# Thiagodcv/gaussian-process-mpc

Hardware: AMD Instinct MI355X
Metric: GP-MPC rollouts/sec (N train pts x H horizon x d dims) (higher is better)
Workload: dtype f64; 1 GPU; C3: N=2048, d(state_dim)=4, action_dim=1, H=20, B=256 trajectories per GPU, gamma=-1.0, objective+gradient; N=2048, state_dim=4, action_dim=1, H=20, batch_per_gpu=256, parallelism=single GPU

## Files before the change

gaussian_process_mpc_amd/_lib.py:

```python
import ctypes
import os

import torch

_HERE = os.path.dirname(os.path.abspath(__file__))
LIB_PATH = os.environ.get("GPMPC_LIB_PATH") or os.path.join(_HERE, "csrc", "libgpmpc_hip.so")

MAX_D = 8
MAX_DS = 8
MAX_CONS = 16
MPPI_MAX_SAMPLES = 4096
LBFGS_MAX_STARTS = 256
LBFGS_MAX_HISTORY = 16
WANT_GRAD = 1
COV_BUG_COMPAT = 2
USE_GRAPH = 4
FP32_ACCUM = 8
FP32_ALL = 16

_ERR = {-1: "bad argument", -2: "device allocation failed", -3: "HIP call / kernel launch failed",
        -4: "workspace too small", -5: "pack not built",
        -6: "current HIP device differs from the device the pack was created on"}


class LibraryMissing(RuntimeError):
    pass


class GpmpcError(RuntimeError):
    pass


class CostParamsC(ctypes.Structure):
    _fields_ = [("gamma", ctypes.c_double),
                ("Q", ctypes.c_double * (MAX_DS * MAX_DS)),
                ("R", ctypes.c_double * (MAX_D * MAX_D)),
                ("R_delta", ctypes.c_double * (MAX_D * MAX_D)),
                ("x_ref", ctypes.c_double * MAX_DS),
                ("u_ref", ctypes.c_double * MAX_D),
                ("last_u", ctypes.c_double * MAX_D),
                ("has_R_delta", ctypes.c_int),
                ("schedule_id", ctypes.c_int)]


class StateConstraintsC(ctypes.Structure):
    _fields_ = [("n_rows", ctypes.c_int),
                ("reserved", ctypes.c_int),
                ("A", ctypes.c_double * (MAX_CONS * MAX_DS)),
                ("b", ctypes.c_double * MAX_CONS),
                ("kappa", ctypes.c_double * MAX_CONS)]


class MppiParamsC(ctypes.Structure):
    _fields_ = [("n_samples", ctypes.c_int),
                ("iterations", ctypes.c_int),
                ("sigma", ctypes.c_double * MAX_D),
                ("sigma_decay", ctypes.c_double),
                ("beta", ctypes.c_double),
                ("seed", ctypes.c_ulonglong),
                ("call_index", ctypes.c_uint),
                ("reserved", ctypes.c_uint),
                ("lb", ctypes.c_double * MAX_D),
                ("ub", ctypes.c_double * MAX_D)]


class LbfgsParamsC(ctypes.Structure):
    _fields_ = [("n_starts", ctypes.c_int),
                ("history", ctypes.c_int),
                ("gtol", ctypes.c_double),
                ("ftol", ctypes.c_double),
                ("c1", ctypes.c_double),
                ("min_step", ctypes.c_double),
                ("lb", ctypes.c_double * MAX_D),
                ("ub", ctypes.c_double * MAX_D)]


class AuglagParamsC(ctypes.Structure):
    _fields_ = [("inner", LbfgsParamsC),
                ("rho0", ctypes.c_double),
                ("growth", ctypes.c_double),
                ("shrink", ctypes.c_double),
                ("rho_max", ctypes.c_double),
                ("lam_max", ctypes.c_double),
                ("feas_tol", ctypes.c_double),
                ("inner_ticks", ctypes.c_int),
                ("reserved", ctypes.c_int)]


_vp, _i, _d, _sz, _u = ctypes.c_void_p, ctypes.c_int, ctypes.c_double, ctypes.c_size_t, ctypes.c_uint
_dp = ctypes.POINTER(ctypes.c_double)

SIGNATURES = {
    "gpmpc_device_count": (_i, []),
    "gpmpc_version": (ctypes.c_char_p, []),
    "gpmpc_last_error": (ctypes.c_char_p, []),
    "gpmpc_pack_create": (_i, [ctypes.POINTER(_vp), _i, _i, _i]),
    "gpmpc_pack_destroy": (_i, [_vp]),
    "gpmpc_pack_resize": (_i, [_vp, _i]),
    "gpmpc_pack_reload_tuning": (_i, [_vp]),
    "gpmpc_pack_graph_captures": (ctypes.c_longlong, [_vp]),
    "gpmpc_pack_callback_captures": (ctypes.c_longlong, [_vp]),
    "gpmpc_store_host": (_i, [_vp, _vp, _sz, _vp]),
    "gpmpc_build_ky": (_i, [_i, _i, _vp, _dp, _d, _d, _vp, _vp, _vp]),
    "gpmpc_pack_build": (_i, [_vp, _vp, _vp, _vp, _dp, _dp, _vp]),
    "gpmpc_pack_build_strided": (_i, [_vp, _vp, _vp, _vp, _sz, _sz, _dp, _dp, _vp]),
    "gpmpc_pack_build_beta": (_i, [_vp, _vp, _vp, _vp, _dp, _dp, _vp]),
    "gpmpc_pack_set_nominal": (_i, [_vp, _dp, _dp, _vp]),
    "gpmpc_pack_get_nominal": (_i, [_vp, _dp, _dp]),
    "gpmpc_pack_set_noise": (_i, [_vp, _dp, _dp, _dp, _vp]),
    "gpmpc_pack_get_noise": (_i, [_vp, _dp, _dp, _dp]),
    "gpmpc_pack_enable_fullcov": (_i, [_vp, _vp]),
    "gpmpc_pack_dims": (_i, [_vp] + [ctypes.POINTER(_i)] * 4),
    "gpmpc_pack_shared_lambda": (_i, [_vp]),
    "gpmpc_pack_export": (_i, [_vp, _vp, _vp, _vp]),
    "gpmpc_moment_match_workspace_bytes": (_sz, [_vp, _i]),
    "gpmpc_moment_match": (_i, [_vp, _i, _vp, _vp, _u] + [_vp] * 10 + [_vp, _sz, _vp]),
    "gpmpc_cost": (_i, [_i, _i, _i, _i, ctypes.POINTER(CostParamsC), _vp, _vp, _vp, _vp, _vp]),
    "gpmpc_cost_grad": (_i, [_i, _i, _i, _i, ctypes.POINTER(CostParamsC)] + [_vp] * 8),
    "gpmpc_cost_schedule_create": (_i, [_i, _i, _i, ctypes.POINTER(_i)]),
    "gpmpc_cost_schedule_destroy": (_i, [_i]),
    "gpmpc_cost_schedule_set": (_i, [_i, _i, _dp, _dp, _dp, _vp]),
    "gpmpc_cost_schedule_set_dev": (_i, [_i, _i, _vp, _vp, _vp, _vp]),
    "gpmpc_cost_schedule_get": (_i, [_i] + [ctypes.POINTER(_i)] * 5 + [ctypes.POINTER(_vp)]),
    "gpmpc_rollout_jac_workspace_bytes": (_sz, [_vp, _i, _i]),
    "gpmpc_rollout_jac": (_i, [_vp, _i, _i, _vp, _vp, _vp, _vp, _vp, _vp, _sz, _vp]),
    "gpmpc_rollout_vjp": (_i, [_i, _i, _i, _i, _vp, _vp, _vp, _vp, _vp, _vp]),
    "gpmpc_rollout_constraints": (_i, [_i, _i, _i, _i, ctypes.POINTER(StateConstraintsC), _vp, _vp, _vp, _vp, _vp, _vp]),
    "gpmpc_rollout_constrained_workspace_bytes": (_sz, [_vp, _i, _i, _u]),
    "gpmpc_rollout_constrained": (_i, [_vp, _i, _i, _vp, _vp, ctypes.POINTER(CostParamsC), ctypes.POINTER(StateConstraintsC), _u,
                                       _vp, _vp, _vp, _vp, _vp, _vp, _vp, _sz, _vp]),
    "gpmpc_mppi_sample": (_i, [_i, _i, _i, ctypes.POINTER(MppiParamsC), _i, _vp, _vp, _vp, _vp, _vp]),
    "gpmpc_mppi_update": (_i, [_i, _i, _i, _i, _d, _vp, _vp, _vp, _vp, _vp, _vp, _vp, _vp]),
    "gpmpc_mppi_solve_workspace_bytes": (_sz, [_vp, _i, ctypes.POINTER(MppiParamsC), ctypes.POINTER(StateConstraintsC)]),
    "gpmpc_mppi_solve": (_i, [_vp, _i, _vp, _vp, ctypes.POINTER(CostParamsC), ctypes.POINTER(StateConstraintsC),
                              ctypes.POINTER(MppiParamsC), _vp, _vp, _vp, _vp, _sz, _vp]),
    "gpmpc_lbfgs_state_bytes": (_sz, [_i, _i, _i, _i]),
    "gpmpc_lbfgs_start": (_i, [_i, _i, _i, ctypes.POINTER(LbfgsParamsC), _vp, _vp, _vp, _vp, _vp, _vp, _sz, _vp]),
    "gpmpc_lbfgs_tick": (_i, [_i, _i, ctypes.POINTER(LbfgsParamsC), _vp, _vp, _vp, _sz, _vp]),
    "gpmpc_lbfgs_solve_workspace_bytes": (_sz, [_vp, _i, ctypes.POINTER(LbfgsParamsC)]),
    "gpmpc_lbfgs_solve": (_i, [_vp, _i, _vp, _vp, ctypes.POINTER(CostParamsC), ctypes.POINTER(LbfgsParamsC), _i, _i, _vp, _sz, _vp]),
    "gpmpc_auglag_state_bytes": (_sz, [_i, _i, _i, _i]),
    "gpmpc_auglag_merit": (_i, [_i, _i, _i, _i] + [_vp] * 9),
    "gpmpc_auglag_outer": (_i, [_i, _i, _i, ctypes.POINTER(AuglagParamsC), _i, _vp, _vp, _vp, _vp, _vp, _vp, _sz, _vp]),
    "gpmpc_auglag_solve_workspace_bytes": (_sz, [_vp, _i, ctypes.POINTER(StateConstraintsC), ctypes.POINTER(AuglagParamsC)]),
    "gpmpc_auglag_solve": (_i, [_vp, _i, _vp, _vp, ctypes.POINTER(CostParamsC), ctypes.POINTER(StateConstraintsC),
                                ctypes.POINTER(AuglagParamsC), _i, _i, _vp, _sz, _vp]),
    "gpmpc_rollout_workspace_bytes": (_sz, [_vp, _i, _i, _u]),
    "gpmpc_plan_describe": (_i, [_vp, _i, _i, _u, ctypes.c_char_p, _sz]),
    "gpmpc_pack_autotune": (_i, [_vp, _i, _i, _u, ctypes.c_char_p, _sz]),
    "gpmpc_pack_autotune_clear": (_i, [_vp]),
    "gpmpc_rollout": (_i, [_vp, _i, _i, _vp, _vp, ctypes.POINTER(CostParamsC), _u, _vp, _vp, _vp, _vp, _vp, _sz, _vp]),
    "gpmpc_objective_gradient": (_i, [_vp, _i, _dp, _dp, ctypes.POINTER(CostParamsC), _u, _dp, _vp]),
    "gpmpc_rollout_fullcov_workspace_bytes": (_sz, [_vp, _i, _i, _u]),
    "gpmpc_rollout_fullcov_describe": (_i, [_vp, _i, _i, _u, ctypes.c_char_p, _sz]),
    "gpmpc_rollout_fullcov": (_i, [_vp, _i, _i, _vp, _vp, ctypes.POINTER(CostParamsC), _u, _vp, _vp, _vp, _vp, _vp, _sz, _vp]),
    "gpmpc_timing_enable": (_i, [_i]),
    "gpmpc_debug_run_list": (_i, [_i, _i, _i, ctypes.POINTER(_i), _i, ctypes.POINTER(_i)]),
    "gpmpc_debug_xcd_order": (_i, [_i, _i, _i, _i, ctypes.POINTER(_i), ctypes.POINTER(_i)]),
    "gpmpc_pair_kernel_time": (_i, [_dp, ctypes.POINTER(ctypes.c_longlong), _i]),
    "gpmpc_pair_kernel_time_class": (_i, [_i, _dp, ctypes.POINTER(ctypes.c_longlong)]),
    "gpmpc_matvec": (_i, [_i, _i, _vp, _vp, _vp, _vp]),
    "gpmpc_kinv_append_workspace_bytes": (_sz, [_i]),
    "gpmpc_kinv_append": (_i, [_i, _vp, _vp, _d, _vp, _vp, _sz, _vp]),
    "gpmpc_gp_append_workspace_bytes": (_sz, [_i, _i]),
    "gpmpc_gp_append": (_i, [_i, _i, _vp, _vp, _dp, _d, _d, _vp, _vp, _sz, _vp, _sz, _vp, _vp, _vp, _sz, _vp, _sz, _vp]),
    "gpmpc_kinv_remove": (_i, [_i, _vp, _sz, _i, _vp, _sz, _vp]),
    "gpmpc_gp_replace_workspace_bytes": (_sz, [_i, _i]),
    "gpmpc_gp_replace": (_i, [_i, _i, _i, _vp, _vp, _dp, _d, _d, _vp, _vp, _sz, _vp, _sz, _vp, _vp, _vp, _sz, _vp, _sz, _vp]),
    "gpmpc_predict_workspace_bytes": (_sz, [_i, _i, _i]),
    "gpmpc_predict": (_i, [_i, _i, _vp, _dp, _d, _vp, _vp, _d, _i, _vp, _vp, _vp, _vp, _vp, _sz, _vp]),
    "gpmpc_ml_grad_workspace_bytes": (_sz, [_i, _i]),
    "gpmpc_ml_grad": (_i, [_i, _i, _vp, _vp, _vp, _vp, _dp, _d, _d, _vp, _vp, _sz, _vp]),
}

_lib = None


def lib():
    global _lib
    if _lib is None:
        if not os.path.exists(LIB_PATH):
            raise LibraryMissing(
                f"{LIB_PATH} not found: build it with `python -c 'import __graft_entry__ as g; g.build()'` "
                "or `make -C gaussian_process_mpc_amd/csrc`. There is no CPU fallback.")
        h = ctypes.CDLL(LIB_PATH)
        tolerant = bool(os.environ.get("GPMPC_LIB_PATH")) and os.environ.get("GPMPC_LIB_ALLOW_MISSING") == "1"
        for name, (res, args) in SIGNATURES.items():
            try:
                fn = getattr(h, name)
            except AttributeError:
                if tolerant:
                    continue
                raise
            fn.restype, fn.argtypes = res, args
        _lib = h
    return _lib


def check(rc, what):
    if rc != 0:
        detail = lib().gpmpc_last_error().decode() if rc == -3 else ""
        if rc == -1 and ("mppi" in what or "lbfgs" in what or "auglag" in what):
            detail = lib().gpmpc_last_error().decode()
        if rc == -1 and not detail:
            why = lib().gpmpc_last_error().decode()
            detail = why if "cost schedule" in why else ""
        if rc == -5:
            why = lib().gpmpc_last_error().decode()
            detail = why if "nominal model" in why else ""
        raise GpmpcError(f"{what} failed: {_ERR.get(rc, rc)} {detail}".strip())


def require_gpu():
    lib()
    if not torch.cuda.is_available():
        raise GpmpcError("no HIP device visible: the GP-MPC rollout runs on the MI355X only (no CPU fallback)")
    return torch.device("cuda", torch.cuda.current_device())


def stream_ptr(device=None):
    idx = device.index if isinstance(device, torch.device) and device.index is not None else torch.cuda.current_device()
    return ctypes.c_void_p(torch.cuda.current_stream(idx).cuda_stream)


def ptr(t):
    if t is None:
        return ctypes.c_void_p(0)
    assert t.is_cuda and t.dtype == torch.float64 and t.is_contiguous(), (t.device, t.dtype, t.is_contiguous())
    return ctypes.c_void_p(t.data_ptr())


def host_doubles(a):
    import numpy as np
    a = np.ascontiguousarray(np.asarray(a, dtype=np.float64))
    return a, a.ctypes.data_as(_dp)
```

gaussian_process_mpc_amd/csrc/api.hip:

```cpp
#include "gpmpc_internal.h"

int gpmpc_launch_pair(int D, bool diag, bool grad, int tb, int waves, const PairArgs& a, hipStream_t s) {
    if (waves < 1 || waves > 4) return GPMPC_E_ARG;
    switch (D) {
        case 1: return gpmpc_launch_pair_D<1>(diag, grad, tb, waves, a, s);
        case 2: return gpmpc_launch_pair_D<2>(diag, grad, tb, waves, a, s);
        case 3: return gpmpc_launch_pair_D<3>(diag, grad, tb, waves, a, s);
        case 4: return gpmpc_launch_pair_D<4>(diag, grad, tb, waves, a, s);
        case 5: return gpmpc_launch_pair_D<5>(diag, grad, tb, waves, a, s);
        case 6: return gpmpc_launch_pair_D<6>(diag, grad, tb, waves, a, s);
        case 7: return gpmpc_launch_pair_D<7>(diag, grad, tb, waves, a, s);
        case 8: return gpmpc_launch_pair_D<8>(diag, grad, tb, waves, a, s);
    }
    return GPMPC_E_ARG;
}

int gpmpc_launch_pair_sb(int D, bool grad, int tb, int ns2, int waves, const PairSbArgs& a, hipStream_t s) {
    if (waves < 1 || waves > 4) return GPMPC_E_ARG;
    switch (D) {
        case 1: return gpmpc_launch_pair_sb_D<1>(grad, tb, ns2, waves, a, s);
        case 2: return gpmpc_launch_pair_sb_D<2>(grad, tb, ns2, waves, a, s);
        case 3: return gpmpc_launch_pair_sb_D<3>(grad, tb, ns2, waves, a, s);
        case 4: return gpmpc_launch_pair_sb_D<4>(grad, tb, ns2, waves, a, s);
        case 5: return gpmpc_launch_pair_sb_D<5>(grad, tb, ns2, waves, a, s);
        case 6: return gpmpc_launch_pair_sb_D<6>(grad, tb, ns2, waves, a, s);
        case 7: return gpmpc_launch_pair_sb_D<7>(grad, tb, ns2, waves, a, s);
        case 8: return gpmpc_launch_pair_sb_D<8>(grad, tb, ns2, waves, a, s);
    }
    return GPMPC_E_ARG;
}

int gpmpc_launch_pair_sbs(int D, bool grad, int ng, int ns2, const PairSbsArgs& a, hipStream_t s) {
    switch (D) {
        case 2: return gpmpc_launch_pair_sbs_D<2>(grad, ng, ns2, a, s);
        case 3: return gpmpc_launch_pair_sbs_D<3>(grad, ng, ns2, a, s);
        case 4: return gpmpc_launch_pair_sbs_D<4>(grad, ng, ns2, a, s);
        case 5: return gpmpc_launch_pair_sbs_D<5>(grad, ng, ns2, a, s);
        case 6: return gpmpc_launch_pair_sbs_D<6>(grad, ng, ns2, a, s);
        case 7: return gpmpc_launch_pair_sbs_D<7>(grad, ng, ns2, a, s);
        case 8: return gpmpc_launch_pair_sbs_D<8>(grad, ng, ns2, a, s);
    }
    return GPMPC_E_ARG;
}

int gpmpc_launch_pair_sbf(int D, bool grad, int ns2, int waves, const PairSbfArgs& a, hipStream_t s) {
    if (waves < 1 || waves > 4) return GPMPC_E_ARG;
    switch (D) {
        case 1: return gpmpc_launch_pair_sbf_D<1>(grad, ns2, waves, a, s);
        case 2: return gpmpc_launch_pair_sbf_D<2>(grad, ns2, waves, a, s);
        case 3: return gpmpc_launch_pair_sbf_D<3>(grad, ns2, waves, a, s);
        case 4: return gpmpc_launch_pair_sbf_D<4>(grad, ns2, waves, a, s);
        case 5: return gpmpc_launch_pair_sbf_D<5>(grad, ns2, waves, a, s);
        case 6: return gpmpc_launch_pair_sbf_D<6>(grad, ns2, waves, a, s);
        case 7: return gpmpc_launch_pair_sbf_D<7>(grad, ns2, waves, a, s);
        case 8: return gpmpc_launch_pair_sbf_D<8>(grad, ns2, waves, a, s);
    }
    return GPMPC_E_ARG;
}

int gpmpc_launch_pair_sbfx(int D, bool grad, int ns2, const PairSbfxArgs& a, hipStream_t s) {
    switch (D) {
        case 3: return gpmpc_launch_pair_sbfx_D<3>(grad, ns2, a, s);
        case 4: return gpmpc_launch_pair_sbfx_D<4>(grad, ns2, a, s);
        case 5: return gpmpc_launch_pair_sbfx_D<5>(grad, ns2, a, s);
        case 6: return gpmpc_launch_pair_sbfx_D<6>(grad, ns2, a, s);
    }
    return GPMPC_E_ARG;
}

__global__ void k_cross_kernel(const double* __restrict__ Xp, int p, const double* __restrict__ X, int N, int D,
                               const double* __restrict__ lam, double sf2, double* __restrict__ K) {
    const int i = blockIdx.x * blockDim.x + threadIdx.x, r = blockIdx.y;
    if (i >= N) return;
    double d2 = 0.0;
    for (int k = 0; k < D; ++k) {
        const double d = Xp[(size_t)r * D + k] - X[(size_t)i * D + k];
        d2 = fma(d * d, 1.0 / lam[k], d2);
    }
    K[(size_t)r * N + i] = sf2 * exp(-0.5 * d2);
}

__global__ __launch_bounds__(256) void k_rows_dot(const double* __restrict__ A, const double* __restrict__ v, int N,
                                                   double* __restrict__ out) {
    __shared__ double s_scr[16], s_out[1];
    const int r = blockIdx.x;
    double acc[1] = {0.0};
    for (int i = threadIdx.x; i < N; i += blockDim.x) acc[0] = fma(A[(size_t)r * N + i], v[i], acc[0]);
    block_sum<1>(acc, s_scr, s_out);
    if (threadIdx.x == 0) out[r] = s_out[0];
}

#define GPMPC_PRED_RT 8
__global__ __launch_bounds__(1024) void k_pred_w(const double* __restrict__ K, const double* __restrict__ Kinv, int N, int p,
                                                 double* __restrict__ W) {
    __shared__ double s_part[16][GPMPC_PRED_RT][64];
    const int lane = threadIdx.x & 63, w = __builtin_amdgcn_readfirstlane(threadIdx.x >> 6), r0 = blockIdx.y * GPMPC_PRED_RT;
    const int c = blockIdx.x * 64 + lane;
    const int per = (N + 15) / 16, k0 = w * per, k1 = (k0 + per < N) ? k0 + per : N;
    double s[GPMPC_PRED_RT];
#pragma unroll
    for (int q = 0; q < GPMPC_PRED_RT; ++q) s[q] = 0.0;
    if (c < N)
        for (int k = k0; k < k1; ++k) {
            const double a = Kinv[(size_t)k * N + c];
#pragma unroll
            for (int q = 0; q < GPMPC_PRED_RT; ++q) {
                const int r = r0 + q < p ? r0 + q : p - 1;
                s[q] = fma(K[(size_t)r * N + k], a, s[q]);
            }
        }
#pragma unroll
    for (int q = 0; q < GPMPC_PRED_RT; ++q) s_part[w][q][lane] = s[q];
    __syncthreads();
    for (int q = w; q < GPMPC_PRED_RT; q += 16) {
        if (r0 + q < p && c < N) {
            double t = 0.0;
#pragma unroll
            for (int ww = 0; ww < 16; ++ww) t += s_part[ww][q][lane];
            W[(size_t)(r0 + q) * N + c] = t;
        }
    }
}

__global__ __launch_bounds__(256) void k_pred_cov(const double* __restrict__ Xp, int p, int D, const double* __restrict__ lam,
                                                   double sf2, const double* __restrict__ W, const double* __restrict__ K,
                                                   int N, double noise_var, double* __restrict__ cov) {
    __shared__ double s_scr[16], s_out[1];
    const int r = blockIdx.x, s = blockIdx.y;
    double v[1] = {0.0};
    for (int i = threadIdx.x; i < N; i += blockDim.x) v[0] = fma(W[(size_t)r * N + i], K[(size_t)s * N + i], v[0]);
    block_sum<1>(v, s_scr, s_out);
    if (threadIdx.x == 0) {
        double d2 = 0.0;
        for (int k = 0; k < D; ++k) {
            const double d = Xp[(size_t)r * D + k] - Xp[(size_t)s * D + k];
            d2 = fma(d * d, 1.0 / lam[k], d2);
        }
        cov[(size_t)r * p + s] = sf2 * exp(-0.5 * d2) - s_out[0] + (r == s ? noise_var : 0.0);
    }
}

extern "C" int gpmpc_matvec(int rows, int cols, const double* A_dev, const double* v_dev, double* out_dev, void* stream) {
    if (rows < 1 || cols < 1 || !A_dev || !v_dev || !out_dev) return GPMPC_E_ARG;
    hipLaunchKernelGGL(k_rows_dot, dim3(rows), dim3(256), 0, (hipStream_t)stream, A_dev, v_dev, cols, out_dev);
    GPMPC_HIP(hipGetLastError());
    return GPMPC_OK;
}

extern "C" size_t gpmpc_predict_workspace_bytes(int n, int D, int np) {
    if (n < 1 || np < 1 || D < 1) return 0;
    return 2 * ((sizeof(double) * (size_t)np * n + 255) & ~(size_t)255) + 256;
}

extern "C" int gpmpc_predict(int n, int D, const double* X, const double* lambdas_host, double sigma_f,
                             const double* beta, const double* Kinv, double noise_var, int np, const double* Xp,
                             double* out_K, double* out_mean, double* out_cov, void* workspace, size_t workspace_bytes,
                             void* stream) {
    if (n < 1 || D < 1 || D > GPMPC_MAX_D || np < 1 || !X || !lambdas_host || !Xp || !workspace) return GPMPC_E_ARG;
    if ((out_mean && !beta) || (out_cov && !Kinv)) return GPMPC_E_ARG;
    if (workspace_bytes < gpmpc_predict_workspace_bytes(n, D, np)) return GPMPC_E_WORKSPACE;
    hipStream_t s = (hipStream_t)stream;
    const size_t slab = (sizeof(double) * (size_t)np * n + 255) & ~(size_t)255;
    double* K = out_K ? out_K : (double*)workspace;
    double* W = (double*)((char*)workspace + slab);
    double* lam = (double*)((char*)workspace + 2 * slab);
    if (int rcu = gpmpc_upload_small(lam, lambdas_host, sizeof(double) * D, s)) return rcu;
    const double sf2 = sigma_f * sigma_f;
    hipLaunchKernelGGL(k_cross_kernel, dim3((n + 255) / 256, np), dim3(256), 0, s, Xp, np, X, n, D, lam, sf2, K);
    if (out_mean) hipLaunchKernelGGL(k_rows_dot, dim3(np), dim3(256), 0, s, K, beta, n, out_mean);
    if (out_cov) {
        hipLaunchKernelGGL(k_pred_w, dim3((n + 63) / 64, (np + GPMPC_PRED_RT - 1) / GPMPC_PRED_RT), dim3(1024), 0, s, K, Kinv, n, np, W);
        hipLaunchKernelGGL(k_pred_cov, dim3(np, np), dim3(256), 0, s, Xp, np, D, lam, sf2, W, K, n, noise_var, out_cov);
    }
    GPMPC_HIP(hipGetLastError());
    return GPMPC_OK;
}

__global__ __launch_bounds__(256) void k_append_vw(const double* __restrict__ Kinv, size_t ld, const double* __restrict__ k, int n,
                                                    double* __restrict__ v, double* __restrict__ wv) {
    __shared__ double s_scr[32], s_out[2];
    const int r = blockIdx.x;
    double acc[2] = {0.0, 0.0};
    for (int i = threadIdx.x; i < n; i += blockDim.x) {
        acc[0] = fma(Kinv[(size_t)r * ld + i], k[i], acc[0]);
        acc[1] = fma(Kinv[(size_t)i * ld + r], k[i], acc[1]);
    }
    block_sum<2>(acc, s_scr, s_out);
    if (threadIdx.x == 0) { v[r] = s_out[0]; wv[r] = s_out[1]; }
}

__global__ __launch_bounds__(256) void k_append_q(const double* __restrict__ k, const double* __restrict__ v, int n, double kappa,
                                                   double* __restrict__ q) {
    __shared__ double s_scr[16], s_out[1];
    double acc[1] = {0.0};
    for (int i = threadIdx.x; i < n; i += blockDim.x) acc[0] = fma(k[i], v[i], acc[0]);
    block_sum<1>(acc, s_scr, s_out);
    if (threadIdx.x == 0) q[0] = 1.0 / (kappa - s_out[0]);
}

__global__ void k_append_fill(const double* __restrict__ Kinv, size_t ld_in, const double* __restrict__ v, const double* __restrict__ wv,
                              const double* __restrict__ q, int n, double* __restrict__ out, size_t ld_out,
                              const double* __restrict__ k, const double* __restrict__ Kf_in, const double* __restrict__ Ky_in, size_t ld_k,
                              double* __restrict__ Kf_out, double* __restrict__ Ky_out, double kff, double noise_var) {
    const int j = blockIdx.x * blockDim.x + threadIdx.x, i = blockIdx.y, m = n + 1;
    if (j >= m) return;
    const double qq = q[0];
    double val;
    if (i < n && j < n) val = fma(qq * v[i], wv[j], Kinv[(size_t)i * ld_in + j]);
    else if (i < n) val = -qq * v[i];
    else if (j < n) val = -qq * wv[j];
    else val = qq;
    out[(size_t)i * ld_out + j] = val;
    if (Kf_out) {
        double kf, ky;
        if (i < n && j < n) { kf = Kf_in[(size_t)i * ld_k + j]; ky = Ky_in[(size_t)i * ld_k + j]; }
        else if (i < n) { kf = k[i]; ky = kf; }
        else if (j < n) { kf = k[j]; ky = kf; }
        else { kf = kff; ky = kff + noise_var; }
        Kf_out[(size_t)i * ld_out + j] = kf;
        Ky_out[(size_t)i * ld_out + j] = ky;
    }
}

__global__ void k_append_kvec(const double* __restrict__ X, int n, int D, const double* __restrict__ xnew, const double* __restrict__ lam,
                              double sf2, double* __restrict__ k) {
    const int i = blockIdx.x * blockDim.x + threadIdx.x;
    if (i >= n) return;
    double d2 = 0.0;
    for (int d = 0; d < D; ++d) { const double t = X[(size_t)i * D + d] - xnew[d]; d2 = fma(t * t, 1.0 / lam[d], d2); }
    k[i] = sf2 * exp(-0.5 * d2);
}

extern "C" size_t gpmpc_kinv_append_workspace_bytes(int n) { return n < 1 ? 0 : sizeof(double) * (2 * (size_t)n + 8); }

extern "C" int gpmpc_kinv_append(int n, const double* Kinv_dev, const double* k_dev, double kappa, double* out_dev,
                                 void* workspace, size_t workspace_bytes, void* stream) {
    if (n < 1 || !Kinv_dev || !k_dev || !out_dev || !workspace) return GPMPC_E_ARG;
    if (workspace_bytes < gpmpc_kinv_append_workspace_bytes(n)) return GPMPC_E_WORKSPACE;
    hipStream_t s = (hipStream_t)stream;
    double* v = (double*)workspace; double* wv = v + n; double* q = wv + n;
    hipLaunchKernelGGL(k_append_vw, dim3(n), dim3(256), 0, s, Kinv_dev, (size_t)n, k_dev, n, v, wv);
    hipLaunchKernelGGL(k_append_q, dim3(1), dim3(256), 0, s, k_dev, v, n, kappa, q);
    hipLaunchKernelGGL(k_append_fill, dim3((n + 1 + 255) / 256, n + 1), dim3(256), 0, s, Kinv_dev, (size_t)n, v, wv, q, n, out_dev,
                       (size_t)(n + 1), (const double*)nullptr, (const double*)nullptr, (const double*)nullptr, (size_t)0, (double*)nullptr,
                       (double*)nullptr, 0.0, 0.0);
    GPMPC_HIP(hipGetLastError());
    return GPMPC_OK;
}

struct AppendHyp { double lam[GPMPC_MAX_D]; double sf2; };

__global__ __launch_bounds__(256) void k_append_vw2(const double* __restrict__ X, int n, int D, const double* __restrict__ xnew, AppendHyp H,
                                                     const double* __restrict__ Kinv, size_t ld, double* __restrict__ kout,
                                                     double* __restrict__ v, double* __restrict__ wv) {
    __shared__ double s_scr[32], s_out[2];
    const int r = blockIdx.x;
    double acc[2] = {0.0, 0.0};
    for (int i = threadIdx.x; i < n; i += blockDim.x) {
        double d2 = 0.0;
        for (int d = 0; d < D; ++d) { const double t = X[(size_t)i * D + d] - xnew[d]; d2 = fma(t * t, 1.0 / H.lam[d], d2); }
        const double ki = H.sf2 * exp(-0.5 * d2);
        if (r == 0) kout[i] = ki;
        acc[0] = fma(Kinv[(size_t)r * ld + i], ki, acc[0]);
        acc[1] = fma(Kinv[(size_t)i * ld + r], ki, acc[1]);
    }
    block_sum<2>(acc, s_scr, s_out);
    if (threadIdx.x == 0) { v[r] = s_out[0]; wv[r] = s_out[1]; }
}

__global__ __launch_bounds__(256) void k_append_fill2(const double* __restrict__ Kinv, size_t ld_in, const double* __restrict__ v,
                                                       const double* __restrict__ wv, double kappa, int n, double* __restrict__ out, size_t ld_out,
                                                       const double* __restrict__ k, const double* __restrict__ Kf_in, const double* __restrict__ Ky_in,
                                                       size_t ld_k, double* __restrict__ Kf_out, double* __restrict__ Ky_out, double kff, double noise_var) {
    __shared__ double s_scr[16], s_out[1];
    double acc[1] = {0.0};
    for (int i = threadIdx.x; i < n; i += blockDim.x) acc[0] = fma(k[i], v[i], acc[0]);
    block_sum<1>(acc, s_scr, s_out);
    const double qq = 1.0 / (kappa - s_out[0]);
    const int j = blockIdx.x * blockDim.x + threadIdx.x, i = blockIdx.y, m = n + 1;
    if (j >= m) return;
    double val;
    if (i < n && j < n) val = fma(qq * v[i], wv[j], Kinv[(size_t)i * ld_in + j]);
    else if (i < n) val = -qq * v[i];
    else if (j < n) val = -qq * wv[j];
    else val = qq;
    out[(size_t)i * ld_out + j] = val;
    if (Kf_out) {
        double kf, ky;
        if (i < n && j < n) { kf = Kf_in[(size_t)i * ld_k + j]; ky = Ky_in[(size_t)i * ld_k + j]; }
        else if (i < n) { kf = k[i]; ky = kf; }
        else if (j < n) { kf = k[j]; ky = kf; }
        else { kf = kff; ky = kff + noise_var; }
        Kf_out[(size_t)i * ld_out + j] = kf;
        Ky_out[(size_t)i * ld_out + j] = ky;
    }
}

extern "C" size_t gpmpc_gp_append_workspace_bytes(int n, int D) { (void)D; return n < 1 ? 0 : sizeof(double) * (3 * (size_t)n + 8); }

extern "C" int gpmpc_gp_append(int n, int D, const double* X_dev, const double* xnew_dev, const double* lambdas_host, double sigma_f,
                               double noise_var, const double* Kf_in, const double* Ky_in, size_t ld_k_in, const double* Kinv_in, size_t ld_in,
                               double* Kf_out, double* Ky_out, double* Kinv_out, size_t ld_out, void* workspace, size_t workspace_bytes,
                               void* stream) {
    if (n < 1 || D < 1 || D > GPMPC_MAX_D || !X_dev || !xnew_dev || !lambdas_host || !Kf_in || !Ky_in || !Kinv_in || !Kf_out || !Ky_out ||
        !Kinv_out || !workspace || ld_in < (size_t)n || ld_k_in < (size_t)n || ld_out < (size_t)n + 1)
        return GPMPC_E_ARG;
    if (Kf_in == Kf_out || Ky_in == Ky_out || Kinv_in == Kinv_out) return GPMPC_E_ARG;
    if (workspace_bytes < gpmpc_gp_append_workspace_bytes(n, D)) return GPMPC_E_WORKSPACE;
    hipStream_t s = (hipStream_t)stream;
    double* v = (double*)workspace; double* wv = v + n; double* k = wv + n;
    AppendHyp hyp;
    memset(&hyp, 0, sizeof(hyp));
    for (int d = 0; d < D; ++d) hyp.lam[d] = lambdas_host[d];
    hyp.sf2 = sigma_f * sigma_f;
    hipLaunchKernelGGL(k_append_vw2, dim3(n), dim3(256), 0, s, X_dev, n, D, xnew_dev, hyp, Kinv_in, ld_in, k, v, wv);
    hipLaunchKernelGGL(k_append_fill2, dim3((n + 1 + 255) / 256, n + 1), dim3(256), 0, s, Kinv_in, ld_in, (const double*)v, (const double*)wv,
                       hyp.sf2 + noise_var, n, Kinv_out, ld_out, (const double*)k, Kf_in, Ky_in, ld_k_in, Kf_out, Ky_out, hyp.sf2, noise_var);
    GPMPC_HIP(hipGetLastError());
    return GPMPC_OK;
}

__global__ __launch_bounds__(256) void k_kinv_remove(const double* __restrict__ Kinv, size_t ld_in, int n, int p, double* __restrict__ out,
                                                      size_t ld_out) {
    const int jo = blockIdx.x * blockDim.x + threadIdx.x, io = blockIdx.y;
    if (jo >= n - 1) return;
    const int i = io + (io >= p), j = jo + (jo >= p);
    const double bd = Kinv[(size_t)i * ld_in + p] / Kinv[(size_t)p * ld_in + p];
    out[(size_t)io * ld_out + jo] = fma(-bd, Kinv[(size_t)p * ld_in + j], Kinv[(size_t)i * ld_in + j]);
}

extern "C" int gpmpc_kinv_remove(int n, const double* Kinv_dev, size_t ld_in, int index, double* out_dev, size_t ld_out, void* stream) {
    if (n < 2 || !Kinv_dev || !out_dev || index < 0 || index >= n || ld_in < (size_t)n || ld_out < (size_t)n - 1 || Kinv_dev == out_dev)
        return GPMPC_E_ARG;
    hipLaunchKernelGGL(k_kinv_remove, dim3((n - 1 + 255) / 256, n - 1), dim3(256), 0, (hipStream_t)stream, Kinv_dev, ld_in, n, index, out_dev,
                       ld_out);
    GPMPC_HIP(hipGetLastError());
    return GPMPC_OK;
}

__global__ __launch_bounds__(256) void k_replace_vw(const double* __restrict__ X, int n, int D, int p, const double* __restrict__ xnew, AppendHyp H,
                                                     const double* __restrict__ Kinv, size_t ld, double* __restrict__ kout,
                                                     double* __restrict__ v, double* __restrict__ wv) {
    __shared__ double s_scr[64], s_out[4];
    const int r = blockIdx.x;
    double acc[4] = {0.0, 0.0, 0.0, 0.0};
    for (int i = threadIdx.x; i < n; i += blockDim.x) {
        double ki = 0.0;
        if (i != p) {
            double d2 = 0.0;
            for (int d = 0; d < D; ++d) { const double t = X[(size_t)i * D + d] - xnew[d]; d2 = fma(t * t, 1.0 / H.lam[d], d2); }
            ki = H.sf2 * exp(-0.5 * d2);
        }
        if (r == 0) kout[i] = ki;
        acc[0] = fma(Kinv[(size_t)r * ld + i], ki, acc[0]);
        acc[1] = fma(Kinv[(size_t)i * ld + r], ki, acc[1]);
        acc[2] = fma(Kinv[(size_t)p * ld + i], ki, acc[2]);
        acc[3] = fma(Kinv[(size_t)i * ld + p], ki, acc[3]);
    }
    block_sum<4>(acc, s_scr, s_out);
    if (threadIdx.x == 0) {
        const double d = Kinv[(size_t)p * ld + p];
        v[r] = r == p ? 0.0 : fma(-Kinv[(size_t)r * ld + p], s_out[2] / d, s_out[0]);
        wv[r] = r == p ? 0.0 : fma(-Kinv[(size_t)p * ld + r], s_out[3] / d, s_out[1]);
    }
}

__global__ __launch_bounds__(256) void k_replace_fill(const double* __restrict__ Kinv, size_t ld_in, const double* __restrict__ v,
                                                       const double* __restrict__ wv, double kappa, int n, int p, double* __restrict__ out,
                                                       size_t ld_out, const double* __restrict__ k, const double* __restrict__ Kf_in,
                                                       const double* __restrict__ Ky_in, size_t ld_k, double* __restrict__ Kf_out,
                                                       double* __restrict__ Ky_out, double kff, double noise_var) {
    __shared__ double s_scr[16], s_out[1];
    double acc[1] = {0.0};
    for (int i = threadIdx.x; i < n; i += blockDim.x) acc[0] = fma(k[i], v[i], acc[0]);
    block_sum<1>(acc, s_scr, s_out);
    const double qq = 1.0 / (kappa - s_out[0]);
    const int j = blockIdx.x * blockDim.x + threadIdx.x, i = blockIdx.y;
    if (j >= n) return;
    double val, kf, ky;
    if (i != p && j != p) {
        const double bd = Kinv[(size_t)i * ld_in + p] / Kinv[(size_t)p * ld_in + p];
        val = fma(qq * v[i], wv[j], fma(-bd, Kinv[(size_t)p * ld_in + j], Kinv[(size_t)i * ld_in + j]));
        kf = Kf_in[(size_t)i * ld_k + j]; ky = Ky_in[(size_t)i * ld_k + j];
    } else if (i != p) { val = -qq * v[i]; kf = k[i]; ky = kf; }
    else if (j != p) { val = -qq * wv[j]; kf = k[j]; ky = kf; }
    else { val = qq; kf = kff; ky = kff + noise_var; }
    out[(size_t)i * ld_out + j] = val;
    Kf_out[(size_t)i * ld_out + j] = kf;
    Ky_out[(size_t)i * ld_out + j] = ky;
}

extern "C" size_t gpmpc_gp_replace_workspace_bytes(int n, int D) { (void)D; return n < 1 ? 0 : sizeof(double) * (3 * (size_t)n + 8); }

extern "C" int gpmpc_gp_replace(int n, int D, int slot, const double* X_dev, const double* xnew_dev, const double* lambdas_host, double sigma_f,
                                double noise_var, const double* Kf_in, const double* Ky_in, size_t ld_k_in, const double* Kinv_in, size_t ld_in,
                                double* Kf_out, double* Ky_out, double* Kinv_out, size_t ld_out, void* workspace, size_t workspace_bytes,
                                void* stream) {
    if (n < 1 || D < 1 || D > GPMPC_MAX_D || slot < 0 || slot >= n || !X_dev || !xnew_dev || !lambdas_host || !Kf_in || !Ky_in || !Kinv_in ||
        !Kf_out || !Ky_out || !Kinv_out || !workspace || ld_in < (size_t)n || ld_k_in < (size_t)n || ld_out < (size_t)n)
        return GPMPC_E_ARG;
    if (Kf_in == Kf_out || Ky_in == Ky_out || Kinv_in == Kinv_out) return GPMPC_E_ARG;
    if (workspace_bytes < gpmpc_gp_replace_workspace_bytes(n, D)) return GPMPC_E_WORKSPACE;
    hipStream_t s = (hipStream_t)stream;
    double* v = (double*)workspace; double* wv = v + n; double* k = wv + n;
    AppendHyp hyp;
    memset(&hyp, 0, sizeof(hyp));
    for (int d = 0; d < D; ++d) hyp.lam[d] = lambdas_host[d];
    hyp.sf2 = sigma_f * sigma_f;
    hipLaunchKernelGGL(k_replace_vw, dim3(n), dim3(256), 0, s, X_dev, n, D, slot, xnew_dev, hyp, Kinv_in, ld_in, k, v, wv);
    hipLaunchKernelGGL(k_replace_fill, dim3((n + 255) / 256, n), dim3(256), 0, s, Kinv_in, ld_in, (const double*)v, (const double*)wv,
                       hyp.sf2 + noise_var, n, slot, Kinv_out, ld_out, (const double*)k, Kf_in, Ky_in, ld_k_in, Kf_out, Ky_out, hyp.sf2, noise_var);
    GPMPC_HIP(hipGetLastError());
    return GPMPC_OK;
}
```

gaussian_process_mpc_amd/csrc/gpmpc_internal.h:

```cpp
#pragma once
#include <hip/hip_runtime.h>
#include <cstdio>
#include <cstring>
#include "../../include/gpmpc.h"

#define GPMPC_WAVE 64

#define GPMPC_INIT_VAR   1e-3
#define GPMPC_ACTION_VAR ((double)1e-3f)
#define GPMPC_NOISE_MAX (GPMPC_MAX_DS * GPMPC_MAX_DS + GPMPC_MAX_D + GPMPC_MAX_DS)
__host__ __device__ inline int gpmpc_noise_off_action(int ds) { return ds * ds; }
__host__ __device__ inline int gpmpc_noise_off_process(int ds, int da) { return ds * ds + da; }

#define GPMPC_MAX_PAIRS (GPMPC_MAX_DS * (GPMPC_MAX_DS - 1) / 2)

struct gpmpc_worklist {
    int it;
    int waves;
    int jt;
    int nunits, nwork;
    int contiguous;
    int* work_dev;
    int* perm_dev;
    int* ustart_dev;
    int ustart_host[GPMPC_MAX_DS + GPMPC_MAX_PAIRS + 1];
};

struct gpmpc_tuning {
    int pair_sb;
    int tiling;
    int tb;
    int rgroup;
    int no_first;
    int fused;
    int no_xcd_sort;
    int hchunks;
    int sbf_min;
    int colunroll;
    int fused_sb;
    int split;
    int shared;
    int fc_form;
    int fc_rsplit;
    int fc_cu;
    int fc_tiling;
    int fc_shared;
    int xcdmap;
    int persist;
};
void gpmpc_read_tuning(gpmpc_tuning* t);

struct gpmpc_pack {
    int N, Np, ds, da, D;
    int device;
    int num_cu;
    gpmpc_tuning tune;
    int built;
    int npairs;
    int fullcov;
    int pair_a[GPMPC_MAX_PAIRS > 0 ? GPMPC_MAX_PAIRS : 1], pair_b[GPMPC_MAX_PAIRS > 0 ? GPMPC_MAX_PAIRS : 1];
    int* pair_ab_dev;
    double* fcs_rows; int fcs_rw, fcs_tj;
    int fcs_ntile[3];
    int* fcs_ustart_dev[8][3]; int fcs_base[8], fcs_total[8][3];
    int* fcs_tiles256_dev;
    int ncol_host;
    int* ncol_dev;
    double* X;
    double* XT;
    double* beta;
    double* M;
    double* lam;
    double* sf;
    double lam_host[GPMPC_MAX_DS][GPMPC_MAX_D];
    double sf_host[GPMPC_MAX_DS];
    void* graph_cache;
    void* cb_cache;
    void* tuned;
    void* lock;
    gpmpc_worklist wl[2][8];
    int shared_lambda;
    int sh_ng;
    gpmpc_worklist wl_sh[4];
    int sh_tiles[3];
    int nominal;
    double* nom_dev;
    double* resid_dev;
    double nom_host[GPMPC_MAX_DS * (GPMPC_MAX_D + 1)];
    double* noise_dev;
    double noise_host[GPMPC_NOISE_MAX];
};

static inline int gpmpc_num_moments(int D, bool diag, bool grad) {
    if (!grad) return 1;
    return diag ? 1 + 2 * D : 1 + D + D * (D + 1) / 2;
}

struct PairArgs {
    const double* M;
    const double* XT;
    const double* pp;
    double* part;
    const int* work;
    int Np, B, nunits, nwork, pps, nm;
    int jside_off;
    int ntri;
    int ns2;
    int colsplit;
};

struct PairSbArgs {
    const double* M;
    const double* XT;
    const double* pp;
    const double* G;
    double* part;
    const int* work;
    int Np, B, ds, nwork, pps, nm;
    int rgroup;
    int first_step;
    int colunroll;
    const int* ncol;
};
static inline int gpmpc_sb_gw(int D, int ns2) { return (D + 1 + ns2 + 1) & ~1; }
int gpmpc_launch_pair_sb(int D, bool grad, int tb, int ns2, int waves, const PairSbArgs& a, hipStream_t s);
template <int D> int gpmpc_launch_pair_sb_D(bool grad, int tb, int ns2, int waves, const PairSbArgs& a, hipStream_t s);

struct PairSbfArgs {
    const double* M;
    const double* XT;
    const double* pp;
    const double* G;
    double* part;
    const int* work;
    int Np, B, nunits, nwork, pps, nm, ntri;
    int cu;
    double* part0;
    int pstride;
};
struct PairSbfxArgs {
    const double* XT; const double* lam; const double* beta; const double* sf;
    const double* pp; const double* G;
    const double* rows;
    double* part; double* part0;
    const int* pair_ab;
    int Np, N, B, nunits, unit0, pps, nm;
    int tj, ntile, jt;
    const int* tiles;
    int base, pstride;
};
template <int D> int gpmpc_launch_pair_sbfx_D(bool grad, int ns2, const PairSbfxArgs& a, hipStream_t s);
int gpmpc_launch_pair_sbfx(int D, bool grad, int ns2, const PairSbfxArgs& a, hipStream_t s);
static inline int gpmpc_sbf_gw(int D, int ns2) { return (D + 1 + ns2 * (ns2 + 1) / 2 + 1) & ~1; }
int gpmpc_launch_pair_sbf(int D, bool grad, int ns2, int waves, const PairSbfArgs& a, hipStream_t s);
template <int D> int gpmpc_launch_pair_sbf_D(bool grad, int ns2, int waves, const PairSbfArgs& a, hipStream_t s);

struct PairSbsArgs {
    const double* M;
    const double* XT;
    const double* pp;
    const double* G;
    double* part;
    const int* work;
    int Np, B, ds, nwork, tiles, jt, pps, nm;
    int rgroup, first_step;
    const int* ncol;
};
static inline int gpmpc_sbs_group(int ds, int D) {
    int cap = 48 / (1 + D + ds);
    if (cap > 4) cap = 4;
    if (cap < 2) cap = 2;
    const int groups = (ds + cap - 1) / cap;
    return (ds + groups - 1) / groups;
}
int gpmpc_launch_pair_sbs(int D, bool grad, int ng, int ns2, const PairSbsArgs& a, hipStream_t s);
template <int D> int gpmpc_launch_pair_sbs_D(bool grad, int ng, int ns2, const PairSbsArgs& a, hipStream_t s);

int gpmpc_launch_pair_lowprec(int D, int mode, const PairArgs& a, hipStream_t s);

struct FusedArgs {
    const double* XT; const double* beta; const double* lam; const double* sf; const double* M; const int* work;
    int Np, nwork;
    int tri64;
    int ustart[GPMPC_MAX_DS + 1];
    const double* x0; const double* U; int B, H;
    double* means; double* vars; double* jac;
    double* sp; double* part; double* partz;
    int sps, nm;
    double* gscr;
    int ntile;
    int tiles;
    const int* ncol;
    int xcdmap;
    const double* noise;
};
template <int D> int gpmpc_launch_step_fused_D(bool grad, int ns2, int q, int ng, const FusedArgs& a, int t, hipStream_t s);
__host__ __device__ inline void gpmpc_xcd_remap(int L, int gx, int nt, int nB, int* b, unsigned* bx) {
    const int nt8 = nt & ~7, full = nt8 * nB, allt = nt * nB;
    if (L < full) { const int grp = L / (8 * nB), r = L - grp * 8 * nB; *b = r >> 3; *bx = (unsigned)(grp * 8 + (r & 7)); }
    else if (L < allt) { const int rem = nt - nt8, L2 = L - full; *b = L2 / rem; *bx = (unsigned)(nt8 + L2 - *b * rem); }
    else { const int nr = gx - nt, L3 = L - allt; *b = L3 / nr; *bx = (unsigned)(nt + L3 - *b * nr); }
}

struct PersistArgs {
    const double* XT; const double* beta; const double* lam; const double* sf; const double* M;
    int Np;
    const double* x0; const double* U; int B, H;
    double* means; double* vars; double* jac;
    double* gscr;
    const int* ncol;
    int total;
    const double* noise;
};
template <int D> int gpmpc_launch_persist_D(bool grad, int ns2, int waves, int ng, const PersistArgs& a, hipStream_t s);


int gpmpc_launch_pair(int D, bool diag, bool grad, int tb, int waves, const PairArgs& a, hipStream_t s);
template <int D> int gpmpc_launch_pair_D(bool diag, bool grad, int tb, int waves, const PairArgs& a, hipStream_t s);

void gpmpc_set_error(const char* what, hipError_t e);
void gpmpc_set_error_text(const char* text);
int gpmpc_check_constraints(const gpmpc_state_constraints* cons, const char* who);
__host__ __device__ inline size_t gpmpc_sched_off_u(int H_max, int ds) { return (size_t)(H_max + 1) * ds; }
__host__ __device__ inline size_t gpmpc_sched_off_q(int H_max, int ds, int da) { return gpmpc_sched_off_u(H_max, ds) + (size_t)H_max * da; }
__host__ __device__ inline size_t gpmpc_sched_off_flags(int H_max, int ds, int da) { return gpmpc_sched_off_q(H_max, ds, da) + (size_t)ds * ds; }
struct gpmpc_sched_ref { const double* dev; int H_max; };
int gpmpc_schedule_resolve(const gpmpc_cost_params* cost, int ds, int da, int H, const char* who, gpmpc_sched_ref* out);
int gpmpc_upload_small(void* dst_dev, const void* src_host, size_t bytes, hipStream_t s);
static inline int gpmpc_check_device(const gpmpc_pack* p) {
    int dev = -1;
    if (hipGetDevice(&dev) != hipSuccess) return GPMPC_E_LAUNCH;
    return dev == p->device ? GPMPC_OK : GPMPC_E_DEVICE;
}
enum { GPMPC_TIME_FULL = 0, GPMPC_TIME_FIRST = 1, GPMPC_TIME_FUSED = 2, GPMPC_TIME_CLASSES = 3 };
void gpmpc_tuned_free(void* table);
void gpmpc_tuned_clear(void* table);
void* gpmpc_lock_create();
void gpmpc_lock_destroy(void* lock);
void gpmpc_graph_cache_free(void* cache);
void gpmpc_cb_cache_free(void* cache);
void gpmpc_graph_cache_invalidate(void* cache);
void gpmpc_cb_cache_invalidate(void* cache);
#define GPMPC_HIP(call)                                              \
    do {                                                             \
        hipError_t e_ = (call);                                      \
        if (e_ != hipSuccess) { gpmpc_set_error(#call, e_); return GPMPC_E_LAUNCH; } \
    } while (0)

template <int CTRL>
__device__ __forceinline__ double gpmpc_dpp_f64(double v) {
    const int lo = __builtin_amdgcn_update_dpp(0, __double2loint(v), CTRL, 0xf, 0xf, false);
    const int hi = __builtin_amdgcn_update_dpp(0, __double2hiint(v), CTRL, 0xf, 0xf, false);
    return __hiloint2double(hi, lo);
}
__device__ __forceinline__ double gpmpc_readlane_f64(double v, int lane) {
    return __hiloint2double(__builtin_amdgcn_readlane(__double2hiint(v), lane), __builtin_amdgcn_readlane(__double2loint(v), lane));
}
__device__ __forceinline__ double wave_sum(double v) {
    v += gpmpc_dpp_f64<0xB1>(v);
    v += gpmpc_dpp_f64<0x4E>(v);
    v += gpmpc_dpp_f64<0x141>(v);
    v += gpmpc_dpp_f64<0x140>(v);
    return (gpmpc_readlane_f64(v, 0) + gpmpc_readlane_f64(v, 16)) + (gpmpc_readlane_f64(v, 32) + gpmpc_readlane_f64(v, 48));
}

__device__ __forceinline__ double wave_row_sum(double v) {
    v += gpmpc_dpp_f64<0xB1>(v);
    v += gpmpc_dpp_f64<0x4E>(v);
    v += gpmpc_dpp_f64<0x141>(v);
    v += gpmpc_dpp_f64<0x140>(v);
    return v;
}

template <int NV>
__device__ __forceinline__ void block_sum4_rows(const double (&v)[NV], double* scratch, double* out) {
    const int lane = threadIdx.x & 63, w = threadIdx.x >> 6;
#pragma unroll
    for (int k = 0; k < NV; ++k) {
        const double s = wave_row_sum(v[k]);
        if ((lane & 15) == 0) scratch[(w * 4 + (lane >> 4)) * NV + k] = s;
    }
    __syncthreads();
    if (threadIdx.x < NV) {
        double s = 0;
        for (int ww = 0; ww < 4; ++ww) {
            const double* r4 = &scratch[ww * 4 * NV + threadIdx.x];
            s += (r4[0] + r4[NV]) + (r4[2 * NV] + r4[3 * NV]);
        }
        out[threadIdx.x] = s;
    }
    __syncthreads();
}

template <int NV>
__device__ __forceinline__ void block_sum(const double (&v)[NV], double* scratch, double* out) {
    const int lane = threadIdx.x & 63, w = threadIdx.x >> 6, nw = (blockDim.x + 63) >> 6;
#pragma unroll
    for (int k = 0; k < NV; ++k) {
        double s = wave_sum(v[k]);
        if (lane == 0) scratch[w * NV + k] = s;
    }
    __syncthreads();
    if (threadIdx.x < NV) {
        double s = 0;
        for (int ww = 0; ww < nw; ++ww) s += scratch[ww * NV + threadIdx.x];
        out[threadIdx.x] = s;
    }
    __syncthreads();
}
```

gaussian_process_mpc_amd/csrc/pack.hip:

```cpp
#include "gpmpc_internal.h"
#include <cstdlib>

__global__ void k_pack_points(const double* __restrict__ X, int N, int Np, int D,
                              double* __restrict__ Xp, double* __restrict__ XT) {
    const int i = blockIdx.x * blockDim.x + threadIdx.x;
    if (i >= Np) return;
    for (int k = 0; k < D; ++k) {
        const double v = i < N ? X[(size_t)i * D + k] : 0.0;
        Xp[(size_t)i * D + k] = v;
        XT[(size_t)k * Np + i] = v;
    }
}

__global__ __launch_bounds__(256) void k_pack_beta(const double* __restrict__ Kinv, size_t ld, size_t gstride, const double* __restrict__ Y,
                                                    int N, int Np, int ds, double* __restrict__ beta) {
    const int a = blockIdx.y;
    const int row = blockIdx.x * (blockDim.x >> 6) + (threadIdx.x >> 6);
    const int lane = threadIdx.x & 63;
    if (row >= Np) return;
    double s = 0.0;
    if (row < N) {
        const double* __restrict__ r = Kinv + (size_t)a * gstride + (size_t)row * ld;
        for (int j = lane; j < N; j += 64) s = fma(r[j], Y[(size_t)j * ds + a], s);
        s = wave_sum(s);
    }
    if (lane == 0) beta[(size_t)a * Np + row] = s;
}

__global__ __launch_bounds__(256) void k_pack_weights(const double* __restrict__ Kinv, size_t ld, size_t gstride, const double* __restrict__ beta,
                                                       const double* __restrict__ XT, const double* __restrict__ lam,
                                                       const double* __restrict__ sf, int N, int Np, int D,
                                                       double* __restrict__ M) {
    __shared__ double s_t[32][33];
    const int a = blockIdx.z;
    const int ti = blockIdx.x * 32, tj = blockIdx.y * 32;
    const int tx = threadIdx.x & 31, ty = threadIdx.x >> 5;
    const double* __restrict__ Ka = Kinv + (size_t)a * gstride;
    double* __restrict__ Ma = M + (size_t)a * Np * Np;
    if (tj + 31 < ti) {
        for (int r = ty; r < 32; r += 8) {
            const int j = tj + r, i = ti + tx;
            if (j < Np && i < Np) Ma[(size_t)j * Np + i] = 0.0;
        }
        return;
    }
    for (int r = ty; r < 32; r += 8) {
        const int i = ti + r, j = tj + tx;
        s_t[r][tx] = (i < N && j < N) ? Ka[(size_t)i * ld + j] : 0.0;
    }
    __syncthreads();
    const double sf2 = sf[a] * sf[a], sf4 = sf2 * sf2;
    for (int r = ty; r < 32; r += 8) {
        const int j = tj + r, i = ti + tx;
        if (j >= Np || i >= Np) continue;
        double out = 0.0;
        if (i <= j && j < N) {
            const double kji = Ka[(size_t)j * ld + i];
            const double kij = s_t[tx][r];
            double d2 = 0.0;
            for (int k = 0; k < D; ++k) {
                const double d = XT[(size_t)k * Np + i] - XT[(size_t)k * Np + j];
                d2 = fma(d * d, 1.0 / lam[a * D + k], d2);
            }
            const double wsym = 0.5 * (kij + kji) - beta[(size_t)a * Np + i] * beta[(size_t)a * Np + j];
            out = (i == j ? 1.0 : 2.0) * wsym * sf4 * exp(-0.25 * d2);
        }
        Ma[(size_t)j * Np + i] = out;
    }
}

__global__ void k_pack_residual(const double* __restrict__ X, const double* __restrict__ Y, const double* __restrict__ nom,
                                int N, int D, int ds, double* __restrict__ R) {
    const int i = blockIdx.x * blockDim.x + threadIdx.x, a = blockIdx.y;
    if (i >= N) return;
    double m = nom[ds * D + a];
    for (int k = 0; k < D; ++k) m = fma(X[(size_t)i * D + k], nom[a * D + k], m);
    R[(size_t)i * ds + a] = Y[(size_t)i * ds + a] - m;
}

struct gpmpc_small_payload { unsigned w[128]; };
__global__ void k_upload_small(gpmpc_small_payload p, unsigned* __restrict__ dst, int nwords) {
    const int i = threadIdx.x;
    if (i < nwords) dst[i] = p.w[i];
}
int gpmpc_upload_small(void* dst_dev, const void* src_host, size_t bytes, hipStream_t s) {
    if (!dst_dev || !src_host || bytes == 0 || bytes > sizeof(gpmpc_small_payload) || (bytes & 3)) return GPMPC_E_ARG;
    gpmpc_small_payload p;
    memset(&p, 0, sizeof(p));
    memcpy(&p, src_host, bytes);
    hipLaunchKernelGGL(k_upload_small, dim3(1), dim3(128), 0, s, p, (unsigned*)dst_dev, (int)(bytes / 4));
    GPMPC_HIP(hipGetLastError());
    return GPMPC_OK;
}

extern "C" int gpmpc_store_host(void* dst_dev, const void* src_host, size_t bytes, void* stream) {
    return gpmpc_upload_small(dst_dev, src_host, bytes, (hipStream_t)stream);
}

__global__ void k_build_ky(const double* __restrict__ X, int n, int D, const double* __restrict__ lam,
                           double sf2, double noise_var, double* __restrict__ Kf, double* __restrict__ Ky) {
    const int j = blockIdx.x * blockDim.x + threadIdx.x, i = blockIdx.y;
    if (j >= n) return;
    double d2 = 0.0;
    for (int k = 0; k < D; ++k) {
        const double d = X[(size_t)i * D + k] - X[(size_t)j * D + k];
        d2 = fma(d * d, 1.0 / lam[k], d2);
    }
    const double kf = sf2 * exp(-0.5 * d2);
    if (Kf) Kf[(size_t)i * n + j] = kf;
    Ky[(size_t)i * n + j] = kf + (i == j ? noise_var : 0.0);
}

__global__ void k_pack_fcs_rows(const double* __restrict__ beta, const double* __restrict__ XT, const double* __restrict__ lam,
                                int N, int Np, int D, int ds, int rw, double* __restrict__ rows) {
    const int j = blockIdx.x * blockDim.x + threadIdx.x;
    if (j >= Np) return;
    double* r = rows + (size_t)j * rw;
    double e = 0.0;
    for (int k = 0; k < D; ++k) { const double x = XT[(size_t)k * Np + j]; r[k] = x; e = fma(x * x, 1.0 / lam[k], e); }
    r[D] = (0.25 * 0x1.71547652b82fep+11) * e;
    for (int c = 0; c < ds; ++c) r[D + 1 + c] = j < N ? beta[(size_t)c * Np + j] : 0.0;
    for (int k = D + 1 + ds; k < rw; ++k) r[k] = 0.0;
}

static int fcs_refresh(gpmpc_pack* p, hipStream_t s) {
    if (!p->fullcov || p->npairs == 0 || !p->shared_lambda || p->ds < 2 || p->ds > 4 || p->D - p->ds < 1 || p->D - p->ds > 2) return GPMPC_OK;
    if (!p->fcs_rows) {
        p->fcs_rw = (p->D + 1 + p->ds + 1) & ~1;
        p->fcs_tj = p->Np / 64;
        p->fcs_ntile[0] = p->fcs_tj * (p->fcs_tj + 1) / 2; p->fcs_ntile[1] = 4 * p->fcs_ntile[0];
        {
            const int T = p->fcs_tj;
            int n2 = 0;
            for (int ti = 0; ti < T; ++ti) n2 += (p->Np - 64 * ti + 255) / 256;
            int* h = (int*)malloc(sizeof(int) * 3 * (size_t)n2);
            if (!h) return GPMPC_E_ALLOC;
            int k = 0;
            for (int ti = 0; ti < T; ++ti)
                for (int j0 = 64 * ti; j0 < p->Np; j0 += 256) { h[3 * k] = ti; h[3 * k + 1] = j0; h[3 * k + 2] = p->Np - j0 < 256 ? p->Np - j0 : 256; ++k; }
            p->fcs_ntile[2] = n2;
            hipError_t e = hipMalloc(&p->fcs_tiles256_dev, sizeof(int) * 3 * (size_t)n2);
            if (e == hipSuccess) e = hipMemcpy(p->fcs_tiles256_dev, h, sizeof(int) * 3 * (size_t)n2, hipMemcpyHostToDevice);
            free(h);
            if (e != hipSuccess) return GPMPC_E_ALLOC;
        }
        if (hipMalloc(&p->fcs_rows, sizeof(double) * (size_t)p->Np * p->fcs_rw) != hipSuccess) { p->fcs_rows = nullptr; return GPMPC_E_ALLOC; }
        for (int k : {0, 2, 4}) {
            const gpmpc_worklist& w = p->wl[1][k];
            if (!w.work_dev) continue;
            int ust[GPMPC_MAX_DS + GPMPC_MAX_PAIRS + 1];
            const int ntri = w.ustart_host[p->ds];
            for (int u = 0; u <= p->ds; ++u) ust[u] = w.ustart_host[u];
            p->fcs_base[k] = ntri;
            const size_t nb = sizeof(int) * (p->ds + p->npairs + 1);
            for (int q = 0; q < 3; ++q) {
                for (int pr = 1; pr <= p->npairs; ++pr) ust[p->ds + pr] = ntri + pr * p->fcs_ntile[q];
                p->fcs_total[k][q] = ntri + p->npairs * p->fcs_ntile[q];
                if (hipMalloc(&p->fcs_ustart_dev[k][q], nb) != hipSuccess) { p->fcs_ustart_dev[k][q] = nullptr; return GPMPC_E_ALLOC; }
                GPMPC_HIP(hipMemcpy(p->fcs_ustart_dev[k][q], ust, nb, hipMemcpyHostToDevice));
            }
        }
    }
    hipLaunchKernelGGL(k_pack_fcs_rows, dim3((p->Np + 255) / 256), dim3(256), 0, s, p->beta, p->XT, p->lam, p->N, p->Np, p->D, p->ds,
                       p->fcs_rw, p->fcs_rows);
    GPMPC_HIP(hipGetLastError());
    return GPMPC_OK;
}

__global__ void k_pack_cross(const double* __restrict__ beta, const double* __restrict__ XT, const double* __restrict__ lam,
                             const double* __restrict__ sf, const int* __restrict__ pair_ab, int N, int Np, int D, int ds,
                             double* __restrict__ Mx) {
    const int i = blockIdx.x * blockDim.x + threadIdx.x, j = blockIdx.y, pr = blockIdx.z;
    if (i >= Np) return;
    const int a = pair_ab[2 * pr], b = pair_ab[2 * pr + 1];
    double out = 0.0;
    if (i < N && j < N) {
        double d2 = 0.0;
        for (int k = 0; k < D; ++k) {
            const double d = XT[(size_t)k * Np + i] - XT[(size_t)k * Np + j];
            d2 = fma(d * d, 1.0 / (lam[a * D + k] + lam[b * D + k]), d2);
        }
        const double s2 = sf[a] * sf[a] * sf[b] * sf[b];
        out = beta[(size_t)a * Np + i] * beta[(size_t)b * Np + j] * s2 * exp(-0.5 * d2);
    }
    Mx[((size_t)pr * Np + j) * Np + i] = out;
}

static int build_worklist(int Np, int it, int jt, int ds, int npairs, bool xcd_sort, gpmpc_worklist* w,
                          bool tile_slot = false, int* tiles_out = nullptr) {
    const int ti = (Np + it - 1) / it, tj = (Np + jt - 1) / jt;
    const size_t cap = (size_t)ti * tj * (ds + npairs);
    int* h = (int*)malloc(sizeof(int) * 4 * cap);
    if (!h) return -1;
    int n = 0;
    for (int u = 0; u < ds + npairs; ++u) {
        w->ustart_host[u] = n;
        for (int i0 = 0; i0 < Np; i0 += it)
            for (int j0 = 0; j0 < Np; j0 += jt) {
                const int j1 = j0 + jt < Np ? j0 + jt : Np;
                if (u < ds && j1 <= i0) continue;
                h[4 * n] = u; h[4 * n + 1] = i0; h[4 * n + 2] = j0; h[4 * n + 3] = tile_slot ? n - w->ustart_host[u] : j1; ++n;
            }
        if (tiles_out) *tiles_out = n - w->ustart_host[u];
    }
    w->ustart_host[ds + npairs] = n;
    w->contiguous = 1;
    if (xcd_sort && n >= 16) {
        int* q[8]; int cnt[8] = {0}, pos[8] = {0};
        for (int x = 0; x < 8; ++x) q[x] = (int*)malloc(sizeof(int) * 4 * (size_t)n);
        for (int k = 0; k < n; ++k) {
            const int u = h[4 * k], tjx = h[4 * k + 2] / jt;
            const int x = ((u & 1) ? (tj - 1 - tjx) : tjx) & 7;
            memcpy(q[x] + 4 * cnt[x]++, h + 4 * k, sizeof(int) * 4);
        }
        for (int x = 0; x < 8; ++x)
            qsort(q[x], cnt[x], sizeof(int) * 4, [](const void* a, const void* b) {
                const int* u = (const int*)a; const int* v = (const int*)b;
                if (u[0] != v[0]) return u[0] - v[0];
                if (u[2] != v[2]) return u[2] - v[2];
                return u[1] - v[1];
            });
        for (int p = 0; p < n; ++p) {
            int x = p & 7;
            if (pos[x] >= cnt[x]) {
                int best = 0;
                for (int y = 1; y < 8; ++y) if (cnt[y] - pos[y] > cnt[best] - pos[best]) best = y;
                x = best;
            }
            memcpy(h + 4 * p, q[x] + 4 * pos[x]++, sizeof(int) * 4);
        }
        for (int x = 0; x < 8; ++x) free(q[x]);
        w->contiguous = 0;
    }
    w->it = it; w->waves = it / 64 > 0 ? it / 64 : 1; w->jt = jt; w->nunits = ds + npairs; w->nwork = n;
    hipError_t e = hipMalloc(&w->work_dev, sizeof(int) * 4 * (size_t)n);
    if (e == hipSuccess) e = hipMemcpy(w->work_dev, h, sizeof(int) * 4 * (size_t)n, hipMemcpyHostToDevice);
    w->perm_dev = nullptr;
    if (e == hipSuccess && !w->contiguous) {
        int* perm = (int*)malloc(sizeof(int) * (size_t)n);
        int fill[GPMPC_MAX_DS + GPMPC_MAX_PAIRS + 1];
        for (int u = 0; u <= ds + npairs; ++u) fill[u] = w->ustart_host[u];
        for (int k = 0; k < n; ++k) perm[fill[h[4 * k]]++] = k;
        e = hipMalloc(&w->perm_dev, sizeof(int) * (size_t)n);
        if (e == hipSuccess) e = hipMemcpy(w->perm_dev, perm, sizeof(int) * (size_t)n, hipMemcpyHostToDevice);
        free(perm);
    }
    if (e == hipSuccess) e = hipMalloc(&w->ustart_dev, sizeof(int) * (ds + npairs + 1));
    if (e == hipSuccess) e = hipMemcpy(w->ustart_dev, w->ustart_host, sizeof(int) * (ds + npairs + 1), hipMemcpyHostToDevice);
    free(h);
    return e == hipSuccess ? 0 : -1;
}

static int runs_host(int Np, int ds, int slots, int** items_out, int* ustart) {
    const int it = 256;
    int n64 = 0;
    for (int i0 = 0; i0 < Np; i0 += it) n64 += (Np - (i0 / 64) * 64 + 63) / 64;
    n64 *= ds;
    if (slots < 64 || n64 <= slots + slots / 10) return 0;
    auto count = [&](int L) { int c = 0; for (int i0 = 0; i0 < Np; i0 += it) { const int span = Np - i0; c += (span + L - 1) / L; } return c * ds; };
    int L = 8;
    while (L < 256 && count(L) > slots) L += 8;
    if (count(L) > slots) return 0;
    const int n = count(L);
    int* h = (int*)malloc(sizeof(int) * 4 * (size_t)n);
    if (!h) return -1;
    int k = 0;
    for (int u = 0; u < ds; ++u) {
        ustart[u] = k;
        for (int i0 = 0; i0 < Np; i0 += it) {
            const int span = Np - i0, runs = (span + L - 1) / L;
            int j = i0;
            for (int q = 0; q < runs; ++q) {
                int len = ((span / runs) / 8) * 8;
                const int extra = (span - len * runs) / 8;
                if (q < extra) len += 8;
                if (q == runs - 1) len = Np - j;
                h[4 * k] = u; h[4 * k + 1] = i0; h[4 * k + 2] = j; h[4 * k + 3] = j + len; ++k;
                j += len;
            }
        }
    }
    ustart[ds] = k;
    *items_out = h;
    return k;
}

static int build_worklist_runs(int Np, int ds, int slots, gpmpc_worklist* w) {
    int* h = nullptr;
    const int k = runs_host(Np, ds, slots, &h, w->ustart_host);
    if (k == 0) return 1;
    if (k < 0) return -1;
    w->contiguous = 1;
    w->it = 256; w->waves = 4; w->jt = 256; w->nunits = ds; w->nwork = k;
    w->perm_dev = nullptr;
    hipError_t e = hipMalloc(&w->work_dev, sizeof(int) * 4 * (size_t)k);
    if (e == hipSuccess) e = hipMemcpy(w->work_dev, h, sizeof(int) * 4 * (size_t)k, hipMemcpyHostToDevice);
    if (e == hipSuccess) e = hipMalloc(&w->ustart_dev, sizeof(int) * (ds + 1));
    if (e == hipSuccess) e = hipMemcpy(w->ustart_dev, w->ustart_host, sizeof(int) * (ds + 1), hipMemcpyHostToDevice);
    free(h);
    return e == hipSuccess ? 0 : -1;
}

extern "C" int gpmpc_debug_run_list(int n_padded, int state_dim, int slots, int* items_out, int capacity, int* n_items) {
    if (n_padded < 64 || n_padded % 64 || state_dim < 1 || state_dim > GPMPC_MAX_DS || !n_items || capacity < 0 || (capacity > 0 && !items_out)) return GPMPC_E_ARG;
    int* h = nullptr; int ust[GPMPC_MAX_DS + 1];
    const int k = runs_host(n_padded, state_dim, slots, &h, ust);
    if (k < 0) return GPMPC_E_ALLOC;
    *n_items = k;
    if (k > 0) { if (k <= capacity) memcpy(items_out, h, sizeof(int) * 4 * (size_t)k); free(h); }
    return (k > capacity && capacity > 0) ? GPMPC_E_ARG : GPMPC_OK;
}
extern "C" int gpmpc_debug_xcd_order(int linear_id, int grid_x, int n_tile, int n_traj, int* traj, int* column) {
    if (!traj || !column || grid_x < 1 || n_tile < 1 || n_tile > grid_x || n_traj < 1 || linear_id < 0 || (long)linear_id >= (long)grid_x * n_traj) return GPMPC_E_ARG;
    unsigned bx = 0;
    gpmpc_xcd_remap(linear_id, grid_x, n_tile, n_traj, traj, &bx);
    *column = (int)bx;
    return GPMPC_OK;
}

void gpmpc_read_tuning(gpmpc_tuning* t) {
    auto geti = [](const char* name, int unset) { const char* ev = getenv(name); return ev ? atoi(ev) : unset; };
    t->pair_sb = geti("GPMPC_PAIR_SB", -1);
    t->tiling = geti("GPMPC_TILING", -1);
    t->tb = geti("GPMPC_PAIR_TB", 0);
    t->rgroup = geti("GPMPC_RGROUP", 0);
    t->no_first = getenv("GPMPC_NO_FIRST") ? 1 : 0;
    t->fused = geti("GPMPC_FUSED", -1);
    t->no_xcd_sort = getenv("GPMPC_NO_XCD_SORT") ? 1 : 0;
    t->hchunks = geti("GPMPC_HEAD_CHUNKS", -1);
    t->sbf_min = geti("GPMPC_SBF_MIN", 0);
    t->shared = geti("GPMPC_SHARED", -1);
    t->colunroll = geti("GPMPC_SB_UNROLL", -1);
    t->split = geti("GPMPC_SPLIT", -1);
    t->fused_sb = geti("GPMPC_FUSED_SB", -1);
    t->persist = geti("GPMPC_PERSIST", -1);
    t->xcdmap = geti("GPMPC_XCDMAP", -1);
    t->fc_shared = geti("GPMPC_FC_SHARED", -1);
    t->fc_form = geti("GPMPC_FC_FORM", -1);
    t->fc_tiling = geti("GPMPC_FC_TILING", -1);
    t->fc_rsplit = geti("GPMPC_FC_RSPLIT", 0);
    t->fc_cu = geti("GPMPC_FC_CU", 0);
}

extern "C" int gpmpc_pack_reload_tuning(gpmpc_pack* p) {
    if (!p) return GPMPC_E_ARG;
    if (int rc_dev = gpmpc_check_device(p)) return rc_dev;
    const int keep = p->tune.no_xcd_sort;
    gpmpc_read_tuning(&p->tune);
    p->tune.no_xcd_sort = keep;
    if (p->graph_cache) { gpmpc_graph_cache_free(p->graph_cache); p->graph_cache = nullptr; }
    if (p->cb_cache) { gpmpc_cb_cache_free(p->cb_cache); p->cb_cache = nullptr; }
    gpmpc_tuned_clear(p->tuned);
    return GPMPC_OK;
}

static void noise_defaults(int ds, int da, double* img, bool init, bool action, bool process) {
    if (init) for (int k = 0; k < ds; ++k) for (int l = 0; l < ds; ++l) img[k * ds + l] = k == l ? GPMPC_INIT_VAR : 0.0;
    if (action) for (int j = 0; j < da; ++j) img[gpmpc_noise_off_action(ds) + j] = GPMPC_ACTION_VAR;
    if (process) for (int a = 0; a < ds; ++a) img[gpmpc_noise_off_process(ds, da) + a] = 0.0;
}

extern "C" int gpmpc_pack_create(gpmpc_pack** out, int n_train, int state_dim, int action_dim) {
    if (!out || n_train < 1 || state_dim < 1 || action_dim < 0) return GPMPC_E_ARG;
    const int D = state_dim + action_dim;
    if (D > GPMPC_MAX_D || state_dim > GPMPC_MAX_DS || D < 1) return GPMPC_E_ARG;
    gpmpc_pack* p = (gpmpc_pack*)calloc(1, sizeof(gpmpc_pack));
    if (!p) return GPMPC_E_ALLOC;
    p->N = n_train; p->Np = ((n_train + 63) / 64) * 64; p->ds = state_dim; p->da = action_dim; p->D = D;
    gpmpc_read_tuning(&p->tune);
    p->lock = gpmpc_lock_create();
    if (!p->lock) { free(p); return GPMPC_E_ALLOC; }
    if (hipError_t ed = hipGetDevice(&p->device); ed != hipSuccess) { gpmpc_set_error("gpmpc_pack_create: hipGetDevice", ed); gpmpc_lock_destroy(p->lock); free(p); return GPMPC_E_LAUNCH; }
    if (hipDeviceGetAttribute(&p->num_cu, hipDeviceAttributeMultiprocessorCount, p->device) != hipSuccess || p->num_cu < 1) p->num_cu = 256;
    for (int a = 0; a < state_dim; ++a)
        for (int b = a + 1; b < state_dim; ++b) { p->pair_a[p->npairs] = a; p->pair_b[p->npairs] = b; ++p->npairs; }
    const size_t Np = p->Np;
    hipError_t e = hipSuccess;
    if (e == hipSuccess) e = hipMalloc(&p->X, sizeof(double) * Np * D);
    if (e == hipSuccess) e = hipMalloc(&p->XT, sizeof(double) * Np * D);
    if (e == hipSuccess) e = hipMalloc(&p->beta, sizeof(double) * Np * state_dim);
    if (e == hipSuccess) e = hipMalloc(&p->M, sizeof(double) * Np * Np * state_dim);
    if (e == hipSuccess) e = hipMalloc(&p->lam, sizeof(double) * state_dim * D);
    if (e == hipSuccess) e = hipMalloc(&p->sf, sizeof(double) * state_dim);
    if (e == hipSuccess) e = hipMalloc(&p->ncol_dev, 64);
    if (e == hipSuccess) { const int nc0 = p->Np; e = hipMemcpy(p->ncol_dev, &nc0, sizeof(int), hipMemcpyHostToDevice); p->ncol_host = nc0; }
    if (e == hipSuccess && p->npairs > 0) {
        int hab[2 * GPMPC_MAX_PAIRS];
        for (int k = 0; k < p->npairs; ++k) { hab[2 * k] = p->pair_a[k]; hab[2 * k + 1] = p->pair_b[k]; }
        e = hipMalloc(&p->pair_ab_dev, sizeof(int) * 2 * p->npairs);
        if (e == hipSuccess) e = hipMemcpy(p->pair_ab_dev, hab, sizeof(int) * 2 * p->npairs, hipMemcpyHostToDevice);
    }
    if (e == hipSuccess) e = hipMalloc(&p->noise_dev, sizeof(double) * GPMPC_NOISE_MAX);
    if (e == hipSuccess) {
        noise_defaults(p->ds, p->da, p->noise_host, true, true, true);
        e = hipMemcpy(p->noise_dev, p->noise_host, sizeof(double) * GPMPC_NOISE_MAX, hipMemcpyHostToDevice);
    }
    bool ok = e == hipSuccess;
    int cfg[7][2] = {{256, 256}, {64, 64}, {256, 64}, {64, 128}, {256, 128}, {256, 32}, {256, 16}};
    if (const char* ev = getenv("GPMPC_JT0")) { const int v = atoi(ev); if (v >= 64 && v % 64 == 0) cfg[0][1] = v; }
    for (int mode = 0; mode < 2 && ok; ++mode)
        for (int k = 0; k < 7 && ok; ++k) {
            if (mode == 1 && k >= 2 && k != 2 && k != 4) continue;
            ok = build_worklist(p->Np, cfg[k][0], cfg[k][1], state_dim, mode ? p->npairs : 0,
                                mode == 0 && (k == 0 || k == 4) && !p->tune.no_xcd_sort, &p->wl[mode][k]) == 0;
        }
    if (ok && D >= 6 && !getenv("GPMPC_NO_RUNS")) {
        const int occ = 4;
        if (build_worklist_runs(p->Np, state_dim, p->num_cu * occ - 2 * state_dim, &p->wl[0][7]) < 0) ok = false;
    }
    if (ok && state_dim >= 2 && action_dim >= 1 && action_dim <= 2) {
        p->sh_ng = gpmpc_sbs_group(state_dim, D);
        if (const char* ev = getenv("GPMPC_SHARED_NG")) { const int v = atoi(ev); if (v >= 2 && v <= 4 && v <= state_dim) p->sh_ng = v; }
        const int groups = (state_dim + p->sh_ng - 1) / p->sh_ng;
        ok = build_worklist(p->Np, 256, cfg[0][1], groups, 0, !p->tune.no_xcd_sort, &p->wl_sh[0], true, &p->sh_tiles[0]) == 0 &&
             build_worklist(p->Np, 256, 64, groups, 0, false, &p->wl_sh[1], true, &p->sh_tiles[1]) == 0 &&
             build_worklist(p->Np, 256, 128, groups, 0, !p->tune.no_xcd_sort, &p->wl_sh[2], true, &p->sh_tiles[2]) == 0;
        if (ok && p->sh_ng > 2 && state_dim % 2 == 0) {
            int tiles2 = 0;
            ok = build_worklist(p->Np, 256, 64, state_dim / 2, 0, false, &p->wl_sh[3], true, &tiles2) == 0;
        }
    }
    if (!ok) { gpmpc_set_error("gpmpc_pack_create", e); gpmpc_pack_destroy(p); return GPMPC_E_ALLOC; }
    *out = p;
    return GPMPC_OK;
}

extern "C" int gpmpc_pack_resize(gpmpc_pack* p, int n_train) {
    if (!p || n_train < 1) return GPMPC_E_ARG;
    if (int rc_dev = gpmpc_check_device(p)) return rc_dev;
    if (((n_train + 63) / 64) * 64 != p->Np) return GPMPC_E_ARG;
    p->N = n_train;
    p->built = 0;
    return GPMPC_OK;
}

extern "C" int gpmpc_pack_set_nominal(gpmpc_pack* p, const double* weights_host, const double* bias_host, void* stream) {
    if (!p || ((weights_host == nullptr) != (bias_host == nullptr))) return GPMPC_E_ARG;
    if (int rc_dev = gpmpc_check_device(p)) return rc_dev;
    const int on = weights_host ? 1 : 0, nw = p->ds * p->D;
    if (on) {
        if (!p->nom_dev && hipMalloc(&p->nom_dev, sizeof(double) * (nw + p->ds)) != hipSuccess) { p->nom_dev = nullptr; return GPMPC_E_ALLOC; }
        if (!p->resid_dev && hipMalloc(&p->resid_dev, sizeof(double) * (size_t)p->Np * p->ds) != hipSuccess) { p->resid_dev = nullptr; return GPMPC_E_ALLOC; }
        if (int rcu = gpmpc_upload_small(p->nom_dev, weights_host, sizeof(double) * nw, (hipStream_t)stream)) return rcu;
        if (int rcu = gpmpc_upload_small(p->nom_dev + nw, bias_host, sizeof(double) * p->ds, (hipStream_t)stream)) return rcu;
        memcpy(p->nom_host, weights_host, sizeof(double) * nw);
        memcpy(p->nom_host + nw, bias_host, sizeof(double) * p->ds);
    }
    if (on != p->nominal) {
        gpmpc_graph_cache_invalidate(p->graph_cache);
        gpmpc_cb_cache_invalidate(p->cb_cache);
        gpmpc_tuned_clear(p->tuned);
    }
    p->nominal = on;
    p->built = 0;
    return GPMPC_OK;
}

extern "C" int gpmpc_pack_get_nominal(const gpmpc_pack* p, double* weights_host, double* bias_host) {
    if (!p) return GPMPC_E_ARG;
    if (!p->nominal) return 0;
    const int nw = p->ds * p->D;
    if (weights_host) memcpy(weights_host, p->nom_host, sizeof(double) * nw);
    if (bias_host) memcpy(bias_host, p->nom_host + nw, sizeof(double) * p->ds);
    return 1;
}

extern "C" int gpmpc_pack_set_noise(gpmpc_pack* p, const double* init_cov_host, const double* action_var_host, const double* process_var_host,
                                    void* stream) {
    if (!p) return GPMPC_E_ARG;
    const int ds = p->ds, da = p->da, oa = gpmpc_noise_off_action(ds), ow = gpmpc_noise_off_process(ds, da), n = ow + ds;
    double img[GPMPC_NOISE_MAX];
    memset(img, 0, sizeof(img));
    noise_defaults(ds, da, img, !init_cov_host, !action_var_host, !process_var_host);
    char msg[160];
    if (init_cov_host) {
        double pmax = 0.0;
        for (int e = 0; e < ds * ds; ++e) {
            const double v = init_cov_host[e];
            if (!(v - v == 0.0)) { snprintf(msg, sizeof(msg), "gpmpc_pack_set_noise: init_cov[%d][%d] is not finite", e / ds, e % ds); gpmpc_set_error_text(msg); return GPMPC_E_ARG; }
            if (fabs(v) > pmax) pmax = fabs(v);
        }
        for (int k = 0; k < ds; ++k) {
            if (init_cov_host[k * ds + k] < 0.0) { snprintf(msg, sizeof(msg), "gpmpc_pack_set_noise: init_cov[%d][%d] is negative", k, k); gpmpc_set_error_text(msg); return GPMPC_E_ARG; }
            for (int l = 0; l < ds; ++l) {
                const double a = init_cov_host[k * ds + l], b = init_cov_host[l * ds + k];
                if (fabs(a - b) > 1e-12 * pmax) { snprintf(msg, sizeof(msg), "gpmpc_pack_set_noise: init_cov is not symmetric at [%d][%d]", k, l); gpmpc_set_error_text(msg); return GPMPC_E_ARG; }
                img[k * ds + l] = k == l ? a : 0.5 * (a + b);
            }
        }
    }
    for (int part = 0; part < 2; ++part) {
        const double* src = part ? process_var_host : action_var_host;
        const int cnt = part ? ds : da, off = part ? ow : oa;
        if (!src) continue;
        for (int j = 0; j < cnt; ++j) {
            const double v = src[j];
            if (!(v - v == 0.0) || v < 0.0) {
                snprintf(msg, sizeof(msg), "gpmpc_pack_set_noise: %s[%d] is %s", part ? "process_var" : "action_var", j, v < 0.0 ? "negative" : "not finite");
                gpmpc_set_error_text(msg);
                return GPMPC_E_ARG;
            }
            img[off + j] = v;
        }
    }
    if (int rc_dev = gpmpc_check_device(p)) return rc_dev;
    for (int o = 0; o < n; o += 64) {
        const int m = n - o < 64 ? n - o : 64;
        if (int rcu = gpmpc_upload_small(p->noise_dev + o, img + o, sizeof(double) * m, (hipStream_t)stream)) return rcu;
        memcpy(p->noise_host + o, img + o, sizeof(double) * m);
    }
    return GPMPC_OK;
}

extern "C" int gpmpc_pack_get_noise(const gpmpc_pack* p, double* init_cov_host, double* action_var_host, double* process_var_host) {
    if (!p) return GPMPC_E_ARG;
    const int ds = p->ds, da = p->da, oa = gpmpc_noise_off_action(ds), ow = gpmpc_noise_off_process(ds, da);
    if (init_cov_host) memcpy(init_cov_host, p->noise_host, sizeof(double) * ds * ds);
    if (action_var_host) memcpy(action_var_host, p->noise_host + oa, sizeof(double) * da);
    if (process_var_host) memcpy(process_var_host, p->noise_host + ow, sizeof(double) * ds);
    double def[GPMPC_NOISE_MAX];
    noise_defaults(ds, da, def, true, true, true);
    for (int e = 0; e < ow + ds; ++e) if (p->noise_host[e] != def[e]) return 1;
    return 0;
}

extern "C" int gpmpc_pack_destroy(gpmpc_pack* p) {
    if (!p) return GPMPC_OK;
    if (p->X) (void)hipFree(p->X);
    if (p->XT) (void)hipFree(p->XT);
    if (p->beta) (void)hipFree(p->beta);
    if (p->M) (void)hipFree(p->M);
    if (p->lam) (void)hipFree(p->lam);
    if (p->sf) (void)hipFree(p->sf);
    if (p->ncol_dev) (void)hipFree(p->ncol_dev);
    gpmpc_graph_cache_free(p->graph_cache);
    gpmpc_cb_cache_free(p->cb_cache);
    gpmpc_tuned_free(p->tuned);
    gpmpc_lock_destroy(p->lock);
    if (p->pair_ab_dev) (void)hipFree(p->pair_ab_dev);
    if (p->fcs_rows) (void)hipFree(p->fcs_rows);
    for (int k = 0; k < 8; ++k) for (int q = 0; q < 3; ++q) if (p->fcs_ustart_dev[k][q]) (void)hipFree(p->fcs_ustart_dev[k][q]);
    if (p->fcs_tiles256_dev) (void)hipFree(p->fcs_tiles256_dev);
    if (p->nom_dev) (void)hipFree(p->nom_dev);
    if (p->noise_dev) (void)hipFree(p->noise_dev);
    if (p->resid_dev) (void)hipFree(p->resid_dev);
    for (int mode = 0; mode < 2; ++mode)
        for (int k = 0; k < 8; ++k) {
            if (p->wl[mode][k].work_dev) (void)hipFree(p->wl[mode][k].work_dev);
            if (p->wl[mode][k].perm_dev) (void)hipFree(p->wl[mode][k].perm_dev);
            if (p->wl[mode][k].ustart_dev) (void)hipFree(p->wl[mode][k].ustart_dev);
        }
    for (int k = 0; k < 4; ++k) {
        if (p->wl_sh[k].work_dev) (void)hipFree(p->wl_sh[k].work_dev);
        if (p->wl_sh[k].perm_dev) (void)hipFree(p->wl_sh[k].perm_dev);
        if (p->wl_sh[k].ustart_dev) (void)hipFree(p->wl_sh[k].ustart_dev);
    }
    free(p);
    return GPMPC_OK;
}

__global__ void k_pack_copy_beta(const double* __restrict__ Bsrc, int N, int Np, int ds, double* __restrict__ beta) {
    const int i = blockIdx.x * blockDim.x + threadIdx.x, a = blockIdx.y;
    if (i < Np) beta[(size_t)a * Np + i] = i < N ? Bsrc[(size_t)i * ds + a] : 0.0;
}

static int pack_build_impl(gpmpc_pack* p, const double* X_dev, const double* Y_dev, bool y_is_beta,
                           const double* Ky_inv_dev, const double* lambdas_host, const double* sigma_f_host,
                           void* stream, size_t ld = 0, size_t gstride = 0) {
    if (!p || !X_dev || !Y_dev || !lambdas_host || !sigma_f_host) return GPMPC_E_ARG;
    if (ld == 0) { ld = (size_t)p->N; gstride = (size_t)p->N * p->N; }
    if (ld < (size_t)p->N) return GPMPC_E_ARG;
    if (int rc_dev = gpmpc_check_device(p)) return rc_dev;
    if (!Ky_inv_dev && !y_is_beta) return GPMPC_E_ARG;
    hipStream_t s = (hipStream_t)stream;
    for (int a = 0; a < p->ds; ++a) {
        p->sf_host[a] = sigma_f_host[a];
        for (int k = 0; k < p->D; ++k) {
            p->lam_host[a][k] = lambdas_host[a * p->D + k];
            if (!(p->lam_host[a][k] > 0.0)) return GPMPC_E_ARG;
        }
    }
    const int shared_before = p->shared_lambda;
    p->shared_lambda = p->sh_ng > 0 ? 1 : 0;
    for (int a = 1; a < p->ds && p->shared_lambda; ++a)
        if (memcmp(p->lam_host[a], p->lam_host[0], sizeof(double) * p->D) != 0) p->shared_lambda = 0;
    if (p->shared_lambda != shared_before) {
        gpmpc_graph_cache_invalidate(p->graph_cache);
        gpmpc_cb_cache_invalidate(p->cb_cache);
        gpmpc_tuned_clear(p->tuned);
    }
    if (int rcu = gpmpc_upload_small(p->lam, lambdas_host, sizeof(double) * p->ds * p->D, s)) return rcu;
    if (int rcu = gpmpc_upload_small(p->sf, sigma_f_host, sizeof(double) * p->ds, s)) return rcu;
    hipLaunchKernelGGL(k_pack_points, dim3((p->Np + 255) / 256), dim3(256), 0, s, X_dev, p->N, p->Np, p->D, p->X, p->XT);
    if (p->nominal && !y_is_beta) {
        hipLaunchKernelGGL(k_pack_residual, dim3((p->N + 255) / 256, p->ds), dim3(256), 0, s, X_dev, Y_dev, p->nom_dev, p->N, p->D, p->ds, p->resid_dev);
        Y_dev = p->resid_dev;
    }
    if (y_is_beta)
        hipLaunchKernelGGL(k_pack_copy_beta, dim3((p->Np + 255) / 256, p->ds), dim3(256), 0, s, Y_dev, p->N, p->Np, p->ds, p->beta);
    else
        hipLaunchKernelGGL(k_pack_beta, dim3((p->Np + 3) / 4, p->ds), dim3(256), 0, s, Ky_inv_dev, ld, gstride, Y_dev, p->N, p->Np, p->ds, p->beta);
    if (Ky_inv_dev)
        hipLaunchKernelGGL(k_pack_weights, dim3(p->Np / 32, p->Np / 32, p->ds), dim3(256), 0, s,
                           Ky_inv_dev, ld, gstride, p->beta, p->XT, p->lam, p->sf, p->N, p->Np, p->D, p->M);
    else
        GPMPC_HIP(hipMemsetAsync(p->M, 0, sizeof(double) * (size_t)p->Np * p->Np * p->ds, s));
    if (p->fullcov && p->npairs > 0)
        hipLaunchKernelGGL(k_pack_cross, dim3((p->Np + 255) / 256, p->Np, p->npairs), dim3(256), 0, s, p->beta, p->XT, p->lam,
                           p->sf, p->pair_ab_dev, p->N, p->Np, p->D, p->ds, p->M + (size_t)p->ds * p->Np * p->Np);
    if (int rcf = fcs_refresh(p, s)) return rcf;
    {
        int nc = ((p->N + 7) / 8) * 8;
        if (nc > p->Np) nc = p->Np;
        if (nc != p->ncol_host) {
            if (int rcu = gpmpc_upload_small(p->ncol_dev, &nc, sizeof(int), s)) return rcu;
            p->ncol_host = nc;
        }
    }
    GPMPC_HIP(hipGetLastError());
    p->built = 1;
    return GPMPC_OK;
}

extern "C" int gpmpc_pack_enable_fullcov(gpmpc_pack* p, void* stream) {
    if (!p) return GPMPC_E_ARG;
    if (int rc_dev = gpmpc_check_device(p)) return rc_dev;
    if (!p) return GPMPC_E_ARG;
    if (p->fullcov || p->npairs == 0) { p->fullcov = 1; return GPMPC_OK; }
    hipStream_t s = (hipStream_t)stream;
    const size_t mat = sizeof(double) * (size_t)p->Np * p->Np;
    double* Mnew = nullptr;
    if (hipMalloc(&Mnew, mat * (p->ds + p->npairs)) != hipSuccess) return GPMPC_E_ALLOC;
    GPMPC_HIP(hipMemcpyAsync(Mnew, p->M, mat * p->ds, hipMemcpyDeviceToDevice, s));
    GPMPC_HIP(hipStreamSynchronize(s));
    (void)hipFree(p->M);
    p->M = Mnew;
    p->fullcov = 1;
    gpmpc_graph_cache_free(p->graph_cache); p->graph_cache = nullptr;
    gpmpc_cb_cache_free(p->cb_cache); p->cb_cache = nullptr;
    if (p->built) {
        hipLaunchKernelGGL(k_pack_cross, dim3((p->Np + 255) / 256, p->Np, p->npairs), dim3(256), 0, s, p->beta, p->XT, p->lam,
                           p->sf, p->pair_ab_dev, p->N, p->Np, p->D, p->ds, p->M + (size_t)p->ds * p->Np * p->Np);
        GPMPC_HIP(hipGetLastError());
        if (int rcf = fcs_refresh(p, s)) return rcf;
    }
    return GPMPC_OK;
}

extern "C" int gpmpc_pack_build(gpmpc_pack* p, const double* X_dev, const double* Y_dev, const double* Ky_inv_dev,
                                const double* lambdas_host, const double* sigma_f_host, void* stream) {
    return pack_build_impl(p, X_dev, Y_dev, false, Ky_inv_dev, lambdas_host, sigma_f_host, stream);
}

extern "C" int gpmpc_pack_build_strided(gpmpc_pack* p, const double* X_dev, const double* Y_dev, const double* Ky_inv_dev,
                                        size_t ld, size_t gp_stride, const double* lambdas_host, const double* sigma_f_host, void* stream) {
    if (!Ky_inv_dev || ld == 0) return GPMPC_E_ARG;
    return pack_build_impl(p, X_dev, Y_dev, false, Ky_inv_dev, lambdas_host, sigma_f_host, stream, ld, gp_stride);
}

extern "C" int gpmpc_pack_build_beta(gpmpc_pack* p, const double* X_dev, const double* beta_dev, const double* Ky_inv_dev,
                                     const double* lambdas_host, const double* sigma_f_host, void* stream) {
    return pack_build_impl(p, X_dev, beta_dev, true, Ky_inv_dev, lambdas_host, sigma_f_host, stream);
}

extern "C" int gpmpc_pack_dims(const gpmpc_pack* p, int* n, int* np, int* ds, int* da) {
    if (!p) return GPMPC_E_ARG;
    if (n) *n = p->N;
    if (np) *np = p->Np;
    if (ds) *ds = p->ds;
    if (da) *da = p->da;
    return GPMPC_OK;
}
extern "C" int gpmpc_pack_shared_lambda(const gpmpc_pack* p) {
    if (!p) return GPMPC_E_ARG;
    if (!p->built) return GPMPC_E_STATE;
    return p->shared_lambda;
}
extern "C" int gpmpc_pack_export(const gpmpc_pack* p, double* beta_out, double* weights_out, void* stream) {
    if (!p) return GPMPC_E_ARG;
    if (!p->built) return GPMPC_E_STATE;
    hipStream_t s = (hipStream_t)stream;
    const size_t Np = p->Np;
    if (beta_out) GPMPC_HIP(hipMemcpyAsync(beta_out, p->beta, sizeof(double) * Np * p->ds, hipMemcpyDeviceToDevice, s));
    if (weights_out) GPMPC_HIP(hipMemcpyAsync(weights_out, p->M, sizeof(double) * Np * Np * p->ds, hipMemcpyDeviceToDevice, s));
    return GPMPC_OK;
}

extern "C" int gpmpc_build_ky(int n, int D, const double* X_dev, const double* lambdas_host, double sigma_f,
                              double noise_var, double* Kf_dev, double* Ky_dev, void* stream) {
    if (n < 1 || D < 1 || D > GPMPC_MAX_D || !X_dev || !lambdas_host || !Ky_dev) return GPMPC_E_ARG;
    hipStream_t s = (hipStream_t)stream;
    double* lam = nullptr;
    GPMPC_HIP(hipMallocAsync((void**)&lam, sizeof(double) * D, s));
    if (int rcu = gpmpc_upload_small(lam, lambdas_host, sizeof(double) * D, s)) { (void)hipFreeAsync(lam, s); return rcu; }
    hipLaunchKernelGGL(k_build_ky, dim3((n + 255) / 256, n), dim3(256), 0, s, X_dev, n, D, lam, sigma_f * sigma_f,
                       noise_var, Kf_dev, Ky_dev);
    GPMPC_HIP(hipGetLastError());
    GPMPC_HIP(hipFreeAsync(lam, s));
    return GPMPC_OK;
}
```

gaussian_process_mpc_amd/csrc/pair_inst.hip:

```cpp
#include "pair_kernel.h"
#include "pair_kernel_sb.h"
#include "pair_kernel_sbf.h"
#include "pair_kernel_sbfx.h"
#include "pair_kernel_sbs.h"
#ifndef GPMPC_PAIR_D
#error "compile with -DGPMPC_PAIR_D=<D>"
#endif
template int gpmpc_launch_pair_D<GPMPC_PAIR_D>(bool, bool, int, int, const PairArgs&, hipStream_t);
template int gpmpc_launch_pair_sb_D<GPMPC_PAIR_D>(bool, int, int, int, const PairSbArgs&, hipStream_t);
template int gpmpc_launch_pair_sbf_D<GPMPC_PAIR_D>(bool, int, int, const PairSbfArgs&, hipStream_t);
template int gpmpc_launch_pair_sbfx_D<GPMPC_PAIR_D>(bool, int, const PairSbfxArgs&, hipStream_t);
template int gpmpc_launch_pair_sbs_D<GPMPC_PAIR_D>(bool, int, int, const PairSbsArgs&, hipStream_t);

#if defined(GPMPC_SB_STAMPS) && GPMPC_PAIR_D == 5
extern "C" int gpmpc_debug_sb_stamps(unsigned long long* host_out, int n) {
    return hipMemcpyFromSymbol(host_out, HIP_SYMBOL(g_sb_stamps), sizeof(unsigned long long) * (size_t)n) == hipSuccess ? 0 : -3;
}
#endif
```

gaussian_process_mpc_amd/csrc/plan.h:

```cpp
#pragma once
#include "gpmpc_internal.h"

__host__ __device__ static inline int sps_of(int D) { return 3 + 4 * D; }
__host__ __device__ static inline int sps_nominal(int D) { return sps_of(D) + 2 + 3 * D; }

struct RollShape {
    int tiling, tb, waves, nwork, sb, rgroup, fused, fq, shared, sh_list;
    int colunroll;
    int fng;
    int xcdmap;
    int pwaves;
    int png;
    int hchunks, hrows;
};
struct RollLayout {
    int nm, pps, sps, gw;
    size_t off_pp, off_sp, off_part, off_partz, off_mpart, off_jac, off_G, off_means, off_vars, total;
};

RollShape gpmpc_choose_shape(const gpmpc_pack* p, int B, int H, bool grad, bool lowprec, const gpmpc_tuning* tn_over = nullptr);
RollLayout gpmpc_layout_for(const gpmpc_pack* p, const RollShape& r, int B, int H, bool grad);
static inline const gpmpc_worklist& gpmpc_fused_shared_list(const gpmpc_pack* p, const RollShape& r) {
    return p->wl_sh[(r.fng == 2 && p->sh_ng != 2) ? 3 : 1];
}
bool gpmpc_same_shape(const RollShape& a, const RollShape& b);

#define GPMPC_MAX_SPLIT 4
int gpmpc_split_count(const gpmpc_pack* p, const RollShape& r, int B, bool lowprec, bool eager = false, int split_over = 0,
                      int H = 0, int grad = -1);
struct RollSlice { int b0, b1; RollLayout lay; size_t ws_off; };
size_t gpmpc_split_slices(const gpmpc_pack* p, const RollShape& r, int B, int H, bool grad, int S, RollSlice* out);

#define GPMPC_TUNED_SLOTS 16
struct gpmpc_tuned_entry { int B, H, grad, graph, S, valid; RollShape shape; double ms_default, ms_best; };
struct gpmpc_tuned_table { gpmpc_tuned_entry e[GPMPC_TUNED_SLOTS]; int next; };

struct GraphModeGuard {
    int prev;
    explicit GraphModeGuard(int m);
    ~GraphModeGuard();
};
```

gaussian_process_mpc_amd/csrc/plan.hip:

```cpp
#include "plan.h"
#include <cstdlib>

#define GPMPC_PERSIST_MAXNP_HOST 1024
static thread_local int tl_graph_mode = -1;
GraphModeGuard::GraphModeGuard(int m) : prev(tl_graph_mode) { tl_graph_mode = m; }
GraphModeGuard::~GraphModeGuard() { tl_graph_mode = prev; }
static const gpmpc_tuned_entry* tuned_lookup(const gpmpc_pack* p, int B, int H, bool grad) {
    const gpmpc_tuned_table* t = (const gpmpc_tuned_table*)p->tuned;
    if (!t) return nullptr;
    for (int k = 0; k < GPMPC_TUNED_SLOTS; ++k)
        if (t->e[k].valid && t->e[k].B == B && t->e[k].H == H && t->e[k].grad == (grad ? 1 : 0) &&
            (tl_graph_mode < 0 || t->e[k].graph == tl_graph_mode)) return &t->e[k];
    return nullptr;
}
void gpmpc_tuned_free(void* t) { free(t); }
void gpmpc_tuned_clear(void* t) { if (t) memset(t, 0, sizeof(gpmpc_tuned_table)); }

RollShape gpmpc_choose_shape(const gpmpc_pack* p, int B, int H, bool grad, bool lowprec, const gpmpc_tuning* tn_over) {
    const int D = p->D;
    if (!tn_over && !lowprec)
        if (const gpmpc_tuned_entry* te = tuned_lookup(p, B, H, grad)) return te->shape;
    RollShape shape;
    RollShape* const r = &shape;
    gpmpc_tuning tn_nom;
    if (p->nominal) { tn_nom = tn_over ? *tn_over : p->tune; tn_nom.fused = 0; tn_nom.fused_sb = 0; tn_nom.persist = 0; tn_nom.hchunks = 1; }
    const gpmpc_tuning& tn = p->nominal ? tn_nom : (tn_over ? *tn_over : p->tune);
    const bool sb_ok = p->da <= 2;
    const bool tb2 = D <= 5 && B >= 2;
    const long wg0 = (long)(tb2 ? (B + 1) / 2 : B) * p->wl[0][0].nwork;
    const long thr2 = p->Np <= 512 ? 1100 : 2800;
    const bool big = sb_ok ? wg0 >= (tb2 ? thr2 : 1500) : (long)((B + 1) / 2) * p->wl[0][0].nwork >= 1024;
    const long wg2 = (long)B * p->wl[0][2].nwork;
    const bool shared_on = p->shared_lambda && tn.shared != 0 && p->sh_ng >= 2;
    const bool fsb_can = sb_ok && !lowprec && p->da >= 1 && tn.fused_sb != 0 && (p->Np >= 256 || tn.fused_sb == 1) &&
                         p->wl[0][2].nwork <= 600 * p->ds;
    const bool narrow_ok = fsb_can && p->Np >= 512;
    const bool mid = !big && sb_ok && (wg2 >= (p->Np >= 1024 ? 1250 : 1700) || (fsb_can && wg2 >= (narrow_ok ? 150 : 400)));
    const long fsb_max = shared_on ? 7000 : (p->wl[0][2].nwork <= 200 ? 9000 : (D <= 5 ? 7000 : 4700));
    const bool fsb_take = fsb_can && wg2 <= fsb_max;
    const bool mid512 = p->Np == 512 && B < 768 && !fsb_take && sb_ok && tb2 && (long)((B + 1) / 2) * p->wl[0][4].nwork >= 1600;
    const bool big128 = (!big || mid512) && !fsb_take && sb_ok && tb2 && (p->Np > 512 || mid512) && (long)((B + 1) / 2) * p->wl[0][4].nwork >= 1600;
    r->sb = (sb_ok && (big || mid)) ? 1 : 0;
    const bool big_small_fused = big && p->Np <= 512 && fsb_take && sb_ok && tn.tiling < 0;
    const bool many = (long)p->wl[0][1].nwork > 256L * p->ds;
    r->tiling = big_small_fused ? 2 : ((big && !(mid512 && big128)) ? 0 : (big128 ? 4 : (mid ? 2 : (many ? 3 : 1))));
    if (r->tiling == 2 && narrow_ok && wg2 < 1000)
        r->tiling = (wg2 >= 300 || p->wl[0][6].nwork > 1300) ? 5 : 6;
    if (r->tiling == 2 && fsb_take && p->Np > 256 && p->Np <= 384 && wg2 >= 1000 && !shared_on && tn.xcdmap == 0) r->tiling = 5;
    if (tn.pair_sb >= 0) {
        r->sb = (tn.pair_sb != 0 && sb_ok) ? 1 : 0;
        r->tiling = r->sb ? (big ? 0 : (big128 ? 4 : 2)) : (big ? 0 : (many ? 3 : 1));
    }
    if (tn.tiling >= 0) { const int v = tn.tiling; if (v == 0 || ((v == 1 || v == 3) && !r->sb) || ((v == 2 || v == 4) && r->sb) || ((v == 5 || v == 6) && r->sb && fsb_can)) r->tiling = v; }
    const bool wide = r->tiling == 0 || r->tiling == 4;
    r->tb = r->sb ? ((wide && D <= 5 && B >= 2) ? 2 : 1) : (B >= 2 ? 2 : 1);
    if (tn.tb) { const int v = tn.tb; if (v == 1 || v == 2 || (v == 4 && !r->sb)) r->tb = v; }
    r->rgroup = 4;
    if (tn.rgroup >= 1 && tn.rgroup <= 16) r->rgroup = tn.rgroup;
    if (!wide) r->rgroup = 1;
    if (lowprec) { r->sb = 0; r->tiling = 0; r->tb = 1; }
    r->fused = (!r->sb && !lowprec && (r->tiling == 1 || r->tiling == 3) && p->da <= 2 && tn.fused != 0 &&
                p->wl[0][r->tiling].nwork <= 4096) ? 1 : 0;
    if (r->sb && r->tiling == 2 && r->tb == 1 && fsb_can && (tn.fused_sb == 1 || wg2 <= fsb_max))
        r->fused = 2;
    if (r->sb && (r->tiling == 5 || r->tiling == 6) && r->tb == 1 && fsb_can) r->fused = 2;
    if (r->fused) r->tb = 1;
    r->fq = (r->fused == 1 && r->tiling == 1 && (long)B * p->wl[0][1].nwork < 256) ? 4 : 1;
    r->waves = p->wl[0][r->tiling].waves;
    r->nwork = p->wl[0][r->tiling].nwork;
    r->shared = 0; r->sh_list = 0;
    r->fng = p->sh_ng;
    if (p->sh_ng > 2 && p->ds % 2 == 0 && p->wl_sh[3].work_dev && wg2 < 4200) r->fng = 2;
    if (r->sb && r->fused == 2 && r->tiling == 2 && shared_on && (wg2 >= (r->fng == 2 ? (p->ds == 2 ? 700 : 1000) : 2200) || tn.fused_sb == 1)) {
        r->shared = 1; r->sh_list = 1;
        r->tb = 1; r->waves = 4;
        r->nwork = p->ds * p->sh_tiles[1];
    } else
    if (r->sb && r->fused != 2 && !lowprec && p->shared_lambda && tn.shared != 0 && p->sh_ng >= 2) {
        r->shared = 1;
        r->sh_list = ((long)B * p->wl_sh[0].nwork >= 1700) ? 0 : 1;
        if (tn.tiling == 0 || tn.tiling == 2 || tn.tiling == 4) r->sh_list = tn.tiling == 0 ? 0 : (tn.tiling == 2 ? 1 : 2);
        r->tb = 1; r->waves = 4;
        r->nwork = p->ds * p->sh_tiles[r->sh_list];
        r->rgroup = r->sh_list != 1 ? ((tn.rgroup >= 1 && tn.rgroup <= 16) ? tn.rgroup : 4) : 1;
    }
    if (r->fused == 2 && r->tiling == 2 && !r->shared && tn.tiling < 0 && p->wl[0][7].work_dev) {
        r->tiling = 7;
        r->nwork = p->wl[0][7].nwork;
    }
    r->colunroll = (r->sb && !r->shared && !lowprec && r->tiling == 2 && r->tb == 1 && tn.colunroll != 1 &&
                  ((long)B * r->nwork <= 4096 || tn.colunroll == 4)) ? 4 : 1;
    r->xcdmap = tn.xcdmap;
    r->pwaves = 0;
    {
        const int cu = p->num_cu > 0 ? p->num_cu : 256;
        auto gens_cost = [](int Bn, int slots) {
            const int full = Bn / slots, rem = Bn - full * slots;
            return (double)full + (rem > 0 ? 0.64 + 0.36 * (double)rem / slots : 0.0);
        };
        const bool pshared = shared_on && p->ds >= 2 && D >= 3 && D <= 6;
        const bool all_in_one = pshared && ((p->ds == 4 && D == 5) || (p->ds == 3 && D <= 5));
        const double work = (double)p->ds * p->Np * p->Np;
        double r8 = 1.4 + 4.0e-12 * work * work;
        if (r8 > 2.2) r8 = 2.2;
        if (all_in_one) r8 *= 1.25;
        const double cost16 = gens_cost(B, cu), cost8 = r8 * gens_cost(B, 2 * cu);
        const int Npq = p->Np;
        double inv_e = Npq <= 256 ? (p->ds <= 2 ? 2.15 : 1.95) : (Npq <= 320 ? 1.50 : (Npq <= 384 ? 1.50 : (Npq <= 448 ? 1.45 : (Npq <= 512 ? 1.16 : (Npq <= 576 ? 1.10 : 1.14)))));
        if (pshared) inv_e *= p->ds <= 2 ? 1.0 : (Npq <= 448 ? 1.15 : 1.10);
        if (Npq >= 512 && B > 2 * cu && !pshared) inv_e = 0.9;
        const double cost_spl = (double)B / cu * inv_e;
        int pw = 0;
        if ((cost16 <= cost8 ? cost16 : cost8) < 0.97 * cost_spl) pw = cost8 < cost16 ? 8 : 16;
        if (tn.persist == 8 || tn.persist == 16) pw = tn.persist;
        const bool form_forced = tn.fused == 0 || tn.pair_sb >= 0 || tn.tiling >= 0 || tn.fused_sb >= 0;
        const bool shared_ahead = shared_on && !pshared && p->ds >= 3;
        r->png = 1;
        if (!lowprec && p->da >= 1 && p->da <= 2 && p->Np <= GPMPC_PERSIST_MAXNP_HOST && H * p->da <= 1024 && tn.persist != 0 &&
            pw && (tn.persist > 0 || (p->Np <= 640 && D <= 6 && !shared_ahead && !form_forced))) {
            r->fused = 3; r->sb = 0; r->shared = 0; r->tb = 1; r->rgroup = 1; r->colunroll = 1; r->fq = 1;
            r->pwaves = pw;
            r->png = pshared ? ((pw == 16 && all_in_one) ? p->ds : 2) : 1;
            r->nwork = 0;
        }
    }
    r->hchunks = 0; r->hrows = 0;
    if (!r->fused && !lowprec) {
        int c = 64 / (B * p->ds);
        if (c > p->Np / 512) c = p->Np / 512;
        if (c > 16) c = 16;
        if (tn.hchunks >= 0) c = tn.hchunks;
        if (c > 1) { r->hrows = ((p->Np + c - 1) / c + 255) & ~255; r->hchunks = (p->Np + r->hrows - 1) / r->hrows; if (r->hchunks <= 1) r->hchunks = 0; }
    }
    return shape;
}

RollLayout gpmpc_layout_for(const gpmpc_pack* p, const RollShape& r, int B, int H, bool grad) {
    const int D = p->D;
    RollLayout L;
    L.nm = gpmpc_num_moments(D, true, grad);
    L.pps = D + D * D;
    L.sps = p->nominal ? sps_nominal(D) : sps_of(D);
    size_t off = 0;
    auto take = [&](size_t n) { size_t o = off; off += (n * sizeof(double) + 255) & ~(size_t)255; return o; };
    L.off_pp = take((size_t)B * p->ds * L.pps);
    L.off_sp = take((size_t)2 * B * p->ds * L.sps);
    L.off_part = take((size_t)(r.fused ? 2 * r.fq : 1) * B * r.nwork * L.nm);
    L.off_partz = take(r.fused ? (size_t)2 * r.fq * B * r.nwork : 0);
    L.off_mpart = take(r.hchunks > 1 ? (size_t)2 * B * p->ds * r.hchunks * (1 + 2 * D) : 0);
    L.off_jac = take(grad ? (size_t)B * H * 2 * p->ds * (2 * p->ds + p->da) : 0);
    L.gw = gpmpc_sb_gw(D, p->ds);
    L.off_G = take(r.fused == 3 ? (size_t)B * p->ds * p->Np * L.gw : r.fused == 2 ? (size_t)B * (r.shared ? gpmpc_fused_shared_list(p, r).nwork : r.nwork) * p->wl[0][r.tiling].jt * L.gw
                                : (r.sb ? (size_t)B * (r.shared ? 1 : p->ds) * p->Np * L.gw : 0));
    L.off_means = take((size_t)B * (H + 1) * p->ds);
    L.off_vars = take((size_t)B * (H + 1) * p->ds);
    L.total = off;
    return L;
}

int gpmpc_split_count(const gpmpc_pack* p, const RollShape& r, int B, bool lowprec, bool eager, int split_over, int H, int grad) {
    if (lowprec || !r.sb) return 1;
    if (!split_over && H > 0 && grad >= 0)
        if (const gpmpc_tuned_entry* te = tuned_lookup(p, B, H, grad != 0)) { int S = te->S; if (eager && S > 2) S = 2; return S < 1 ? 1 : (S > B ? B : S); }
    const bool mid = r.shared ? r.sh_list == 1 : r.tiling == 2;
    int S = 1;
    if (r.fused == 2) {
        const long wgs = (long)B * (r.shared && r.fng > 1 ? r.nwork / r.fng : r.nwork);
        S = ((B >= 4 && wgs >= 800) || (B >= 2 && wgs >= 1000 && wgs <= 2500)) ? 2 : 1;
    } else if (mid && B >= 4) {
        S = B / 2 < GPMPC_MAX_SPLIT ? B / 2 : GPMPC_MAX_SPLIT;
        while (S > 1 && (long)(B / S) * r.nwork >= 4096 && B / S < 8) --S;
        while (S > 1 && (long)(B / S) * r.nwork < 900) --S;
        if (S == 3) S = 2;
    }
    if (!mid && !r.shared && (r.tiling == 0 || r.tiling == 4) && r.tb == 2 && B >= 16 && (long)((B + 1) / 2) * r.nwork <= 10000) S = 2;
    if (eager && S > 2) S = 2;
    if (p->tune.split >= 1) S = p->tune.split;
    if (split_over >= 1) S = split_over;
    if (S > GPMPC_MAX_SPLIT) S = GPMPC_MAX_SPLIT;
    if (S > B) S = B;
    return S;
}
size_t gpmpc_split_slices(const gpmpc_pack* p, const RollShape& r, int B, int H, bool grad, int S, RollSlice* out) {
    size_t off = 0;
    for (int k = 0; k < S; ++k) {
        RollSlice& s = out[k];
        s.b0 = (int)((long)B * k / S); s.b1 = (int)((long)B * (k + 1) / S);
        s.lay = gpmpc_layout_for(p, r, s.b1 - s.b0, H, grad);
        s.ws_off = off;
        off += s.lay.total;
    }
    return off;
}

extern "C" size_t gpmpc_rollout_workspace_bytes(const gpmpc_pack* p, int B, int H, unsigned flags) {
    if (!p || B < 1 || H < 1) return 0;
    const bool grad = (flags & GPMPC_WANT_GRAD) != 0, lowprec = (flags & (GPMPC_FP32_ACCUM | GPMPC_FP32_ALL)) != 0;
    GraphModeGuard mode((flags & GPMPC_USE_GRAPH) ? 1 : 0);
    const RollShape r = gpmpc_choose_shape(p, B, H, grad, lowprec);
    size_t need = gpmpc_layout_for(p, r, B, H, grad).total;
    const int S = gpmpc_split_count(p, r, B, lowprec, false, 0, H, grad ? 1 : 0);
    if (S > 1) { RollSlice sl[GPMPC_MAX_SPLIT]; const size_t sb = gpmpc_split_slices(p, r, B, H, grad, S, sl); if (sb > need) need = sb; }
    return need;
}

extern "C" int gpmpc_plan_describe(const gpmpc_pack* p, int B, int H, unsigned flags, char* out, size_t out_bytes) {
    if (!p || !out || out_bytes < 64 || B < 1 || H < 1) return GPMPC_E_ARG;
    const bool grad = (flags & GPMPC_WANT_GRAD) != 0, lowprec = (flags & (GPMPC_FP32_ACCUM | GPMPC_FP32_ALL)) != 0;
    GraphModeGuard mode((flags & GPMPC_USE_GRAPH) ? 1 : 0);
    const RollShape r = gpmpc_choose_shape(p, B, H, grad, lowprec);
    const int S = gpmpc_split_count(p, r, B, lowprec, (flags & GPMPC_USE_GRAPH) == 0, 0, H, grad ? 1 : 0);
    static const int cfg[8][2] = {{256, 256}, {64, 64}, {256, 64}, {64, 128}, {256, 128}, {256, 32}, {256, 16}, {256, 256}};
    const int D = p->D, ds = p->ds;
    char kern[160];
    const char* form;
    long wgs;
    if (r.fused == 3) {
        form = "persist";
        snprintf(kern, sizeof(kern), "k_traj_persist<%d,%d,%s,%d>x%dwaves", D, ds, grad ? "true" : "false", r.png, r.pwaves);
        wgs = B;
    } else if (r.fused == 2) {
        const int q = r.tiling == 2 ? 0 : cfg[r.tiling][1], ng = r.shared ? r.fng : 1;
        const gpmpc_worklist& wsh = gpmpc_fused_shared_list(p, r);
        form = r.shared ? "fused_sb_shared" : "fused_sb";
        snprintf(kern, sizeof(kern), "k_step_fused<%d,%d,%s,%d,%d>", D, ds, grad ? "true" : "false", q, ng);
        wgs = (long)B * ((r.shared ? wsh.nwork : r.nwork) + 2 * ds);
    } else if (r.fused == 1) {
        form = "fused_staged";
        snprintf(kern, sizeof(kern), "k_step_fused<%d,%d,%s,%d,1>", D, ds, grad ? "true" : "false", r.fq);
        wgs = (long)B * (r.nwork * r.fq + 2 * ds);
    } else if (lowprec) {
        form = "lowprec"; snprintf(kern, sizeof(kern), "k_pair_lowprec<%d>", D); wgs = (long)B * r.nwork;
    } else if (r.shared) {
        form = "head+pair_sbs";
        snprintf(kern, sizeof(kern), "gpmpc_pair_kernel_sbs<%d,%d,%d,%s,false>", D, p->sh_ng, ds, grad ? "true" : "false");
        wgs = (long)B * p->wl_sh[r.sh_list].nwork;
    } else if (r.sb) {
        form = "head+pair_sb";
        snprintf(kern, sizeof(kern), "gpmpc_pair_kernel_sb<%d,%d,%d,%s,false,%d>", D, r.tb, ds, grad ? "true" : "false", r.colunroll == 4 ? 4 : 1);
        wgs = (long)((B + r.tb - 1) / r.tb) * r.nwork;
    } else {
        form = "head+pair_staged";
        snprintf(kern, sizeof(kern), "gpmpc_pair_kernel<%d,true,%s,%d>", D, grad ? "true" : "false", r.tb);
        wgs = (long)((B + r.tb - 1) / r.tb) * r.nwork;
    }
    const int tl = r.shared && r.fused != 2 ? (r.sh_list == 0 ? 0 : (r.sh_list == 1 ? 2 : 4)) : r.tiling;
    snprintf(out, out_bytes, "form=%s kernel=%s tiling=%dx%d workgroups=%ld launches_per_step=%d split=%d tb=%d shared=%d hchunks=%d workspace=%zu%s",
             form, kern, cfg[tl][0], cfg[tl][1], wgs, r.fused == 3 ? 0 : (r.fused ? 1 : 2), S, r.tb, r.shared, r.hchunks, gpmpc_layout_for(p, r, B, H, grad).total,
             p->nominal ? " nominal=1" : "");
    return GPMPC_OK;
}

bool gpmpc_same_shape(const RollShape& a, const RollShape& b) {
    if (a.fused == 3 && b.fused == 3) return a.pwaves == b.pwaves && a.png == b.png;
    return a.tiling == b.tiling && a.tb == b.tb && a.sb == b.sb && a.fused == b.fused && a.fq == b.fq && a.shared == b.shared &&
           a.sh_list == b.sh_list && a.fng == b.fng && a.colunroll == b.colunroll && a.hchunks == b.hchunks && a.pwaves == b.pwaves &&
           a.rgroup == b.rgroup && a.nwork == b.nwork && a.xcdmap == b.xcdmap;
}
```

gaussian_process_mpc_amd/csrc/rollout.h:

```cpp
#pragma once
#include "gpmpc_internal.h"
#include "plan.h"
#include <mutex>
#include <type_traits>

struct RollCall {
    const gpmpc_pack* p; int B, H;
    const double* x0; const double* U; const gpmpc_cost_params* cost; unsigned flags;
    double* out_means; double* out_vars; double* out_cost; double* out_grad;
    void* workspace; size_t workspace_bytes; hipStream_t stream;
    double* ext_jac = nullptr;
    bool full_first = false;
    const RollShape* shape = nullptr;
};
int gpmpc_enqueue_rollout(const RollCall& c);

struct PackGuard {
    std::recursive_mutex* m;
    explicit PackGuard(const gpmpc_pack* p) : m((std::recursive_mutex*)p->lock) { if (m) m->lock(); }
    ~PackGuard() { if (m) m->unlock(); }
    PackGuard(const PackGuard&) = delete; PackGuard& operator=(const PackGuard&) = delete;
};

bool gpmpc_timing_on();
int gpmpc_timed_pair(int D, bool diag, bool grad, int tb, int waves, const PairArgs& a, hipStream_t s);
int gpmpc_timed_pair_sb(int D, bool grad, int tb, int ns2, int waves, const PairSbArgs& a, hipStream_t s);
int gpmpc_timed_pair_sbs(int D, bool grad, int ng, int ns2, const PairSbsArgs& a, hipStream_t s);
int gpmpc_timed_pair_sbf(int D, bool grad, int ns2, int waves, const PairSbfArgs& a, hipStream_t s);
int gpmpc_timed_persist(int D, bool grad, int ns2, int waves, int ng, const PersistArgs& a, hipStream_t s);
int gpmpc_timed_step_fused(int D, bool grad, int ns2, int q, int ng, const FusedArgs& a, int t, hipStream_t s);

struct gpmpc_graph_cache;
int gpmpc_ensure_graph_cache(gpmpc_pack* p, gpmpc_graph_cache** out);
size_t gpmpc_split_bytes(const gpmpc_pack* p, const RollShape& r, int B, int H, bool grad, int S);
int gpmpc_enqueue_split(gpmpc_graph_cache* g, int S, const RollShape& whole, const RollCall& c);

template <class Enqueue>
static int gpmpc_capture(hipStream_t s, Enqueue&& enqueue, hipGraphExec_t* out) {
    GPMPC_HIP(hipStreamBeginCapture(s, hipStreamCaptureModeThreadLocal));
    hipGraph_t graph = nullptr;
    const int rc = enqueue();
    hipError_t e = hipStreamEndCapture(s, &graph);
    if (rc == GPMPC_OK && e != hipSuccess) gpmpc_set_error("hipStreamEndCapture", e);
    if (rc == GPMPC_OK && e == hipSuccess) {
        e = hipGraphInstantiate(out, graph, nullptr, nullptr, 0);
        if (e != hipSuccess) gpmpc_set_error("hipGraphInstantiate", e);
    }
    if (graph) (void)hipGraphDestroy(graph);
    return rc != GPMPC_OK ? rc : (e == hipSuccess ? GPMPC_OK : GPMPC_E_LAUNCH);
}

template <int LO, class F>
static inline int gpmpc_dispatch_dim(int d, F&& f) {
    if constexpr (LO > 8) return GPMPC_E_ARG;
    else return d == LO ? f(std::integral_constant<int, LO>{}) : gpmpc_dispatch_dim<LO + 1>(d, f);
}
```

gaussian_process_mpc_amd/csrc/runtime.hip:

```cpp
#include "rollout.h"
#include <new>
#include <vector>

static thread_local char g_err[256] = "";
void gpmpc_set_error(const char* what, hipError_t e) {
    snprintf(g_err, sizeof(g_err), "%s: %s", what, hipGetErrorString(e));
}
void gpmpc_set_error_text(const char* text) { snprintf(g_err, sizeof(g_err), "%s", text); }
extern "C" const char* gpmpc_last_error(void) { return g_err; }
extern "C" const char* gpmpc_version(void) { return "gpmpc-hip 0.1 (gfx950)"; }
extern "C" int gpmpc_device_count(void) {
    int n = 0;
    if (hipGetDeviceCount(&n) != hipSuccess) return 0;
    return n;
}

struct EvPair { hipEvent_t a, b; int cls; };
static struct {
    std::mutex mu;
    int on = 0;
    double ms[GPMPC_TIME_CLASSES] = {0.0, 0.0, 0.0};
    long long n[GPMPC_TIME_CLASSES] = {0, 0, 0};
    std::vector<EvPair> pending;
} g_time;

static void drain_events_locked() {
    for (const EvPair& ev : g_time.pending) {
        float ms = 0.f;
        if (hipEventSynchronize(ev.b) == hipSuccess && hipEventElapsedTime(&ms, ev.a, ev.b) == hipSuccess) {
            g_time.ms[ev.cls] += ms; ++g_time.n[ev.cls];
        }
        (void)hipEventDestroy(ev.a); (void)hipEventDestroy(ev.b);
    }
    g_time.pending.clear();
}
bool gpmpc_timing_on() { std::lock_guard<std::mutex> lk(g_time.mu); return g_time.on != 0; }
extern "C" int gpmpc_timing_enable(int on) { std::lock_guard<std::mutex> lk(g_time.mu); g_time.on = on; return GPMPC_OK; }
extern "C" int gpmpc_pair_kernel_time(double* total_ms, long long* launches, int reset) {
    std::lock_guard<std::mutex> lk(g_time.mu);
    drain_events_locked();
    if (total_ms) *total_ms = g_time.ms[0] + g_time.ms[1] + g_time.ms[2];
    if (launches) *launches = g_time.n[0] + g_time.n[1] + g_time.n[2];
    if (reset) for (int c = 0; c < GPMPC_TIME_CLASSES; ++c) { g_time.ms[c] = 0.0; g_time.n[c] = 0; }
    return GPMPC_OK;
}
extern "C" int gpmpc_pair_kernel_time_class(int cls, double* total_ms, long long* launches) {
    if (cls < 0 || cls >= GPMPC_TIME_CLASSES) return GPMPC_E_ARG;
    std::lock_guard<std::mutex> lk(g_time.mu);
    drain_events_locked();
    if (total_ms) *total_ms = g_time.ms[cls];
    if (launches) *launches = g_time.n[cls];
    return GPMPC_OK;
}

template <class F>
static int timed_launch(int cls, hipStream_t s, F launch) {
    if (!gpmpc_timing_on()) return launch();
    EvPair ev; ev.cls = cls;
    GPMPC_HIP(hipEventCreate(&ev.a));
    GPMPC_HIP(hipEventCreate(&ev.b));
    GPMPC_HIP(hipEventRecord(ev.a, s));
    const int rc = launch();
    GPMPC_HIP(hipEventRecord(ev.b, s));
    std::lock_guard<std::mutex> lk(g_time.mu);
    if (g_time.pending.size() >= 4096) drain_events_locked();
    g_time.pending.push_back(ev);
    return rc;
}

int gpmpc_timed_pair(int D, bool diag, bool grad, int tb, int waves, const PairArgs& a, hipStream_t s) {
    return timed_launch(GPMPC_TIME_FULL, s, [&] { return gpmpc_launch_pair(D, diag, grad, tb, waves, a, s); });
}
int gpmpc_timed_pair_sb(int D, bool grad, int tb, int ns2, int waves, const PairSbArgs& a, hipStream_t s) {
    return timed_launch(a.first_step ? GPMPC_TIME_FIRST : GPMPC_TIME_FULL, s,
                        [&] { return gpmpc_launch_pair_sb(D, grad, tb, ns2, waves, a, s); });
}
int gpmpc_timed_pair_sbs(int D, bool grad, int ng, int ns2, const PairSbsArgs& a, hipStream_t s) {
    return timed_launch(a.first_step ? GPMPC_TIME_FIRST : GPMPC_TIME_FULL, s,
                        [&] { return gpmpc_launch_pair_sbs(D, grad, ng, ns2, a, s); });
}
int gpmpc_timed_pair_sbf(int D, bool grad, int ns2, int waves, const PairSbfArgs& a, hipStream_t s) {
    return timed_launch(GPMPC_TIME_FULL, s, [&] { return gpmpc_launch_pair_sbf(D, grad, ns2, waves, a, s); });
}

int gpmpc_timed_persist(int D, bool grad, int ns2, int waves, int ng, const PersistArgs& a, hipStream_t s) {
    return timed_launch(GPMPC_TIME_FUSED, s, [&] {
        return gpmpc_dispatch_dim<2>(D, [&](auto d) { return gpmpc_launch_persist_D<decltype(d)::value>(grad, ns2, waves, ng, a, s); });
    });
}
int gpmpc_timed_step_fused(int D, bool grad, int ns2, int q, int ng, const FusedArgs& a, int t, hipStream_t s) {
    return timed_launch(GPMPC_TIME_FUSED, s, [&] {
        return gpmpc_dispatch_dim<1>(D, [&](auto d) { return gpmpc_launch_step_fused_D<decltype(d)::value>(grad, ns2, q, ng, a, t, s); });
    });
}

void* gpmpc_lock_create() { return new (std::nothrow) std::recursive_mutex(); }
void gpmpc_lock_destroy(void* l) { delete (std::recursive_mutex*)l; }
```

gaussian_process_mpc_amd/csrc/step.hip:

```cpp
#include "rollout.h"
#include "roll_dev.h"
#include "fast_exp.h"

#ifdef GPMPC_SB_STAMPS
static __device__ unsigned long long g_head_stamps[16];
#define GPMPC_HST(slot)                                                                             \
    do {                                                                                            \
        if (t == 5 && blockIdx.x == 0 && blockIdx.y == 0 && blockIdx.z == 0 && threadIdx.x == 0)    \
            g_head_stamps[slot] = __builtin_amdgcn_s_memtime();                                     \
    } while (0)
extern "C" int gpmpc_debug_head_stamps(unsigned long long* host_out) {
    return hipMemcpyFromSymbol(host_out, HIP_SYMBOL(g_head_stamps), sizeof(unsigned long long) * 16) == hipSuccess ? 0 : -3;
}
#else
#define GPMPC_HST(slot) do { } while (0)
#endif

template <int D, int NOM>
__device__ static void prep_step(const RollArgs& A, int b, int t, int a, int chunk, const double* s_mu, const double* s_var,
                                 double* s_u, double* s_s, double* s_scr, double* s_out, double* s_g) {
    const int ds = A.ds;
    __shared__ double s_B[GPMPC_MAX_D], s_A[GPMPC_MAX_D], s_sc[GPMPC_MAX_D], s_r1[GPMPC_MAX_D], s_r2[GPMPC_MAX_D];
    __shared__ double s_n[NOM ? GPMPC_MAX_D : 1], s_wB[NOM ? GPMPC_MAX_D : 1];
    constexpr int NV = 1 + 2 * D + (NOM == 2 ? 2 * D : 0);
    if (threadIdx.x < D) {
        const int k = threadIdx.x;
        double uk, sk;
        if (k < ds) {
            uk = s_mu[k];
            sk = s_var[k];
        } else {
            uk = A.U[((size_t)b * A.H + (t - 1)) * A.da + (k - ds)];
            sk = A.noise[gpmpc_noise_off_action(ds) + (k - ds)];
        }
        const double lam = A.lam[a * D + k];
        s_u[k] = uk;
        s_s[k] = sk;
        s_B[k] = 1.0 / (sk + lam);
        s_A[k] = 1.0 / (0.5 * lam + sk);
        s_sc[k] = sqrt(0.125 / (0.5 * lam + sk));
        s_r1[k] = sk / lam + 1.0;
        s_r2[k] = 2.0 * sk / lam + 1.0;
        if (NOM) {
            const double nk = A.nom[a * D + k];
            s_n[k] = nk;
            s_wB[k] = (nk * sk) * s_B[k];
        }
    }
    __syncthreads();
    GPMPC_HST(2);
    double u[D], Bk[D], sck[D], wB[NOM == 2 ? D : 1];
#pragma unroll
    for (int k = 0; k < D; ++k) {
        u[k] = s_u[k];
        Bk[k] = s_B[k];
        sck[k] = s_sc[k];
        if (NOM == 2) wB[k] = s_wB[k];
    }
    double* __restrict__ Grow = A.G ? (A.shared ? (a == 0 ? A.G + (size_t)b * A.Np * A.gw : nullptr)
                                                : A.G + ((size_t)b * ds + a) * A.Np * A.gw) : nullptr;
    double v[NV];
#pragma unroll
    for (int m = 0; m < NV; ++m) v[m] = 0.0;
    const bool chunked = A.hchunks > 1;
    const int r0 = chunked ? chunk * A.hrows : 0, r1 = chunked ? (r0 + A.hrows < A.Np ? r0 + A.hrows : A.Np) : A.Np;
    constexpr int PF = 4;
    for (int ib = r0; ib < r1; ib += PF * (int)blockDim.x) {
        double xpf[PF][D], bpf[PF];
#pragma unroll
        for (int r = 0; r < PF; ++r) {
            const int i = ib + r * (int)blockDim.x + (int)threadIdx.x, ic = i < r1 ? i : r1 - 1;
#pragma unroll
            for (int k = 0; k < D; ++k) xpf[r][k] = A.XT[(size_t)k * A.Np + ic];
            bpf[r] = A.beta[(size_t)a * A.Np + ic];
        }
#pragma unroll
        for (int r = 0; r < PF; ++r) {
        const int i0 = ib + r * (int)blockDim.x;
        if (i0 >= r1) break;
        const int i = i0 + threadIdx.x;
        if (i < r1) {
            double d[D], xk[D], q = 0.0;
#pragma unroll
            for (int k = 0; k < D; ++k) { xk[k] = xpf[r][k]; d[k] = u[k] - xk[k]; q = fma(Bk[k] * d[k], d[k], q); }
            const double p = bpf[r] * exp(-0.5 * q);
            v[0] += p;
#pragma unroll
            for (int k = 0; k < D; ++k) { v[1 + k] = fma(p, d[k], v[1 + k]); v[1 + D + k] = fma(p * d[k], d[k], v[1 + D + k]); }
            if (NOM == 2) {
                double qn = 0.0;
#pragma unroll
                for (int k = 0; k < D; ++k) qn = fma(wB[k], d[k], qn);
                const double pq = p * qn;
#pragma unroll
                for (int k = 0; k < D; ++k) { v[1 + 2 * D + k] = fma(pq, d[k], v[1 + 2 * D + k]); v[1 + 3 * D + k] = fma(pq * d[k], d[k], v[1 + 3 * D + k]); }
            }
            if (Grow) {
                double* g = s_g + threadIdx.x * A.gw;
                double qh = 0.0;
#pragma unroll
                for (int k = 0; k < D; ++k) {
                    const double h = fma(-sck[k], xk[k], sck[k] * u[k]);
                    g[k] = h;
                    qh = fma(h, h, qh);
                    if (k < ds) g[D + 1 + k] = h * h;
                }
                g[D] = GPMPC_EXP_NEG_INV_C * qh;
                for (int k = D + 1 + ds; k < A.gw; ++k) g[k] = 0.0;
            }
        }
        if (Grow) {
            __syncthreads();
            const int rows = (r1 - i0 < (int)blockDim.x) ? r1 - i0 : (int)blockDim.x;
            double* dst = Grow + (size_t)i0 * A.gw;
            for (int e = threadIdx.x; e < rows * A.gw; e += blockDim.x) dst[e] = s_g[e];
            __syncthreads();
        }
        }
    }
    GPMPC_HST(3);
    block_sum<NV>(v, s_scr, s_out);
    GPMPC_HST(4);
    if (chunked) {
        if (threadIdx.x < 1 + 2 * D)
            A.mpart[((((size_t)(t & 1) * A.B + b) * ds + a) * A.hchunks + chunk) * (1 + 2 * D) + threadIdx.x] = s_out[threadIdx.x];
        if (chunk == 0 && threadIdx.x < D) {
            const int k = threadIdx.x;
            const double sf = A.sf[a], sf2 = sf * sf;
            double detm = 1.0, detv = 1.0;
            for (int l = 0; l < D; ++l) { detm *= s_r1[l]; detv *= s_r2[l]; }
            const double cm = sf2 / sqrt(detm), c = 1.0 / sqrt(detv);
            double* sp = A.sp + (((size_t)(t & 1) * A.B + b) * ds + a) * A.sps;
            double* pp = A.pp + ((size_t)b * ds + a) * A.pps;
            if (k == 0) { sp[0] = c; sp[1] = cm; sp[2] = sf2 + A.noise[gpmpc_noise_off_process(ds, A.da) + a]; }
            const double sc = s_sc[k];
            sp[3 + k] = s_A[k]; sp[3 + D + k] = sc;
            sp[3 + 2 * D + k] = s_B[k];
            pp[k] = sc * s_u[k];
            pp[D + k] = sc;
        }
        return;
    }
    if (threadIdx.x < D) {
        const int k = threadIdx.x;
        const double sf = A.sf[a], sf2 = sf * sf;
        double detm = 1.0, detv = 1.0;
        for (int l = 0; l < D; ++l) { detm *= s_r1[l]; detv *= s_r2[l]; }
        const double cm = sf2 / sqrt(detm), c = 1.0 / sqrt(detv);
        const double mu = cm * s_out[0];
        double* sp = A.sp + (((size_t)(t & 1) * A.B + b) * ds + a) * A.sps;
        double* pp = A.pp + ((size_t)b * ds + a) * A.pps;
        if (k == 0) { sp[0] = c; sp[1] = mu; sp[2] = sf2 + A.noise[gpmpc_noise_off_process(ds, A.da) + a]; }
        const double Bq = s_B[k], sc = s_sc[k];
        sp[3 + k] = s_A[k]; sp[3 + D + k] = sc;
        sp[3 + 2 * D + k] = -Bq * cm * s_out[1 + k];
        sp[3 + 3 * D + k] = -0.5 * mu * Bq + 0.5 * Bq * Bq * cm * s_out[1 + D + k];
        pp[k] = sc * s_u[k];
        pp[D + k] = sc;
        if (NOM) {
            double* ex = sp + sps_of(D);
            double lin = A.nom[A.ds * D + a], vlin = 0.0, cross = 0.0;
            for (int l = 0; l < D; ++l) {
                const double nl = s_n[l], wl = nl * s_s[l];
                lin = fma(nl, s_u[l], lin);
                vlin = fma(nl * nl, s_s[l], vlin);
                cross = fma(wl, -s_B[l] * cm * s_out[1 + l], cross);
            }
            if (k == 0) { ex[0] = lin; ex[1] = vlin + 2.0 * cross; }
            if (NOM == 2) {
                const double nk = s_n[k], wk = nk * s_s[k];
                ex[2 + k] = 2.0 * (cm * Bq * s_out[1 + 2 * D + k] - wk * Bq * mu);
                ex[2 + D + k] = nk * nk + 2.0 * nk * (-Bq * cm * s_out[1 + k]) - 0.5 * Bq * (2.0 * cross)
                                + Bq * Bq * cm * (2.0 * wk * s_out[1 + k] - s_out[1 + 3 * D + k]);
                ex[2 + 2 * D + k] = nk;
            }
        }
    }
}

template <int D, int NOM>
__global__ __launch_bounds__(256) void k_roll_head(RollArgs A, int t) {
    __shared__ double s_z[GPMPC_MAX_DS * (1 + 2 * GPMPC_MAX_D)];
    __shared__ double s_zred[GPMPC_MAX_DS * (1 + 2 * GPMPC_MAX_D) * GPMPC_RED_CH];
    __shared__ double s_mu[GPMPC_MAX_DS], s_var[GPMPC_MAX_DS];
    __shared__ double s_u[GPMPC_MAX_D], s_s[GPMPC_MAX_D];
    __shared__ double s_scr[16 * (1 + 2 * D + (NOM == 2 ? 2 * D : 0))], s_out[1 + 2 * D + (NOM == 2 ? 2 * D : 0)];
    __shared__ double s_g[256 * (2 * D + 2)];
    __shared__ double s_ms[GPMPC_MAX_DS * (1 + 2 * GPMPC_MAX_D) + 4 * GPMPC_MAX_DS];
    const int b = blockIdx.x, a = blockIdx.y, chunk = blockIdx.z;
    GPMPC_HST(0);
    if (t == 1) {
        if (threadIdx.x < A.ds) {
            const double x = A.x0[(size_t)b * A.ds + threadIdx.x];
            const double v0 = A.noise[threadIdx.x * (A.ds + 1)];
            s_mu[threadIdx.x] = x;
            s_var[threadIdx.x] = v0;
            if (a == 0 && chunk == 0) {
                A.means[((size_t)b * (A.H + 1)) * A.ds + threadIdx.x] = x;
                A.vars[((size_t)b * (A.H + 1)) * A.ds + threadIdx.x] = v0;
            }
        }
        __syncthreads();
    } else {
        finish_step<NOM != 0>(A, b, t - 1, chunk == 0 ? a : A.ds, s_z, s_zred, s_mu, s_var, s_ms);
    }
    GPMPC_HST(1);
    prep_step<D, NOM>(A, b, t, a, chunk, s_mu, s_var, s_u, s_s, s_scr, s_out, s_g);
    GPMPC_HST(5);
}

template <int D>
static void launch_head(const RollArgs& A, int t, hipStream_t s) {
    const dim3 grid(A.B, A.ds, A.hchunks > 1 ? A.hchunks : 1);
    if (!A.nom) hipLaunchKernelGGL((k_roll_head<D, 0>), grid, dim3(256), 0, s, A, t);
    else if (A.grad) hipLaunchKernelGGL((k_roll_head<D, 2>), grid, dim3(256), 0, s, A, t);
    else hipLaunchKernelGGL((k_roll_head<D, 1>), grid, dim3(256), 0, s, A, t);
}

int gpmpc_enqueue_rollout(const RollCall& c) {
    const gpmpc_pack* p = c.p;
    const int B = c.B, H = c.H;
    if (!p || !c.x0 || !c.U || !c.cost || !c.out_cost || !c.workspace || B < 1 || H < 1) return GPMPC_E_ARG;
    if (!p->built) return GPMPC_E_STATE;
    const bool grad = (c.flags & GPMPC_WANT_GRAD) != 0;
    if (grad && !c.out_grad) return GPMPC_E_ARG;
    gpmpc_sched_ref sched;
    if (int rcs = gpmpc_schedule_resolve(c.cost, p->ds, p->da, H, "gpmpc_rollout", &sched)) return rcs;
    const int lowprec = (c.flags & GPMPC_FP32_ALL) ? 2 : ((c.flags & GPMPC_FP32_ACCUM) ? 1 : 0);
    if (lowprec && grad) return GPMPC_E_ARG;
    if (lowprec && p->nominal) {
        gpmpc_set_error_text("gpmpc_rollout: the GPMPC_FP32_* modes do not know the linear nominal model of this pack");
        return GPMPC_E_STATE;
    }
    const RollShape r = c.shape ? *c.shape : gpmpc_choose_shape(p, B, H, grad, lowprec != 0);
    const RollLayout L = gpmpc_layout_for(p, r, B, H, grad);
    if (c.workspace_bytes < L.total) return GPMPC_E_WORKSPACE;
    hipStream_t s = c.stream;
    char* ws = (char*)c.workspace;
    RollArgs A;
    memset(&A, 0, sizeof(A));
    A.XT = p->XT; A.beta = p->beta; A.lam = p->lam; A.sf = p->sf;
    A.Np = p->Np; A.ds = p->ds; A.da = p->da; A.D = p->D;
    A.x0 = c.x0; A.U = c.U; A.B = B; A.H = H;
    A.means = c.out_means ? c.out_means : (double*)(ws + L.off_means);
    A.vars = c.out_vars ? c.out_vars : (double*)(ws + L.off_vars);
    A.pp = (double*)(ws + L.off_pp); A.sp = (double*)(ws + L.off_sp); A.part = (double*)(ws + L.off_part);
    A.jac = grad ? (c.ext_jac ? c.ext_jac : (double*)(ws + L.off_jac)) : nullptr;
    A.hchunks = r.hchunks; A.hrows = r.hrows; A.mpart = r.hchunks > 1 ? (double*)(ws + L.off_mpart) : nullptr;
    A.G = r.sb ? (double*)(ws + L.off_G) : nullptr; A.gw = L.gw;
    A.pps = L.pps; A.sps = L.sps; A.nwork = r.nwork; A.nm = L.nm; A.grad = grad ? 1 : 0;
    A.ustart = p->wl[0][r.tiling].ustart_dev;
    A.work = p->wl[0][r.tiling].contiguous ? nullptr : p->wl[0][r.tiling].work_dev;
    A.perm = p->wl[0][r.tiling].contiguous ? nullptr : p->wl[0][r.tiling].perm_dev;
    A.out_cost = c.out_cost; A.out_grad = c.out_grad; A.cost = *c.cost;
    A.nom = p->nominal ? p->nom_dev : nullptr;
    A.sched = sched.dev; A.sched_hmax = sched.H_max;
    A.noise = p->noise_dev;
    if (A.nom && (r.fused || r.hchunks > 1)) {
        gpmpc_set_error_text("gpmpc_rollout: plan without a nominal variant on a nominal pack");
        return GPMPC_E_STATE;
    }
    if (r.shared) {
        A.shared = 1; A.ust_inline = 1; A.work = nullptr; A.perm = nullptr;
        for (int a = 0; a <= p->ds; ++a) A.ust[a] = a * p->sh_tiles[r.sh_list];
    }

    PairArgs P;
    P.M = p->M; P.XT = p->XT; P.pp = A.pp; P.part = A.part; P.work = p->wl[0][r.tiling].work_dev;
    P.Np = p->Np; P.B = B; P.nunits = p->ds; P.nwork = r.nwork; P.pps = L.pps; P.nm = L.nm;
    P.jside_off = 0; P.ntri = p->ds; P.ns2 = p->ds; P.colsplit = (r.tiling == 1 || r.tiling == 3) ? 1 : 0;

    if (r.fused == 3) {
        PersistArgs Q;
        memset(&Q, 0, sizeof(Q));
        Q.XT = p->XT; Q.beta = p->beta; Q.lam = p->lam; Q.sf = p->sf; Q.M = p->M; Q.Np = p->Np;
        Q.x0 = c.x0; Q.U = c.U; Q.B = B; Q.H = H;
        Q.means = A.means; Q.vars = A.vars; Q.jac = A.jac;
        Q.gscr = (double*)(ws + L.off_G);
        const int T = p->Np / 64;
        Q.total = ((p->ds + r.png - 1) / r.png) * 32 * T * (T + 1);
        Q.ncol = p->ncol_dev;
        Q.noise = p->noise_dev;
        const int rc = gpmpc_timed_persist(p->D, grad, p->ds, r.pwaves, r.png, Q, s);
        if (rc != GPMPC_OK) return rc;
        A.finished = 1;
    } else
    if (r.fused) {
        FusedArgs F;
        memset(&F, 0, sizeof(F));
        const gpmpc_worklist& wl = p->wl[0][r.tiling];
        const bool fsh = r.fused == 2 && r.shared;
        const gpmpc_worklist& wsh = gpmpc_fused_shared_list(p, r);
        F.XT = p->XT; F.beta = p->beta; F.lam = p->lam; F.sf = p->sf; F.M = p->M; F.work = fsh ? wsh.work_dev : wl.work_dev;
        const int nwg = r.nwork * r.fq;
        F.Np = p->Np; F.nwork = nwg;
        F.ntile = fsh ? wsh.nwork : nwg; F.tiles = fsh ? p->sh_tiles[1] : 0;
        F.tri64 = (r.tiling == 1) ? 1 : 0;
        for (int a = 0; a <= p->ds; ++a) { F.ustart[a] = fsh ? a * p->sh_tiles[1] : wl.ustart_host[a] * r.fq; A.ust[a] = F.ustart[a]; }
        A.ust_inline = 1; A.nwork = nwg;
        F.x0 = c.x0; F.U = c.U; F.B = B; F.H = H;
        F.means = A.means; F.vars = A.vars; F.jac = A.jac;
        F.sp = A.sp; F.part = A.part; F.partz = (double*)(ws + L.off_partz);
        F.sps = L.sps; F.nm = L.nm;
        F.gscr = r.fused == 2 ? (double*)(ws + L.off_G) : nullptr;
        F.ncol = p->ncol_dev;
        F.noise = p->noise_dev;
        F.xcdmap = r.xcdmap >= 0 ? (r.xcdmap && B > 1) : B >= 2;
        const int fq = r.fused == 2 ? (r.tiling == 2 ? 0 : wl.jt) : r.fq;
        for (int t = 1; t <= H; ++t)
            if (int rc = gpmpc_timed_step_fused(p->D, grad, p->ds, fq, fsh ? r.fng : 1, F, t, s)) return rc;
        A.part += (size_t)(H & 1) * B * nwg * L.nm;
    }
    for (int t = 1; t <= H && !r.fused; ++t) {
        const int first_step = (t == 1 && !p->tune.no_first && !c.full_first) ? 1 : 0;
        int rc = gpmpc_dispatch_dim<1>(p->D, [&](auto d) { launch_head<decltype(d)::value>(A, t, s); return GPMPC_OK; });
        if (rc != GPMPC_OK) return rc;
        if (lowprec) {
            rc = gpmpc_launch_pair_lowprec(p->D, lowprec, P, s);
        } else if (r.shared) {
            const gpmpc_worklist& wl = p->wl_sh[r.sh_list];
            PairSbsArgs Q;
            Q.M = p->M; Q.XT = p->XT; Q.pp = A.pp; Q.G = A.G; Q.part = A.part; Q.work = wl.work_dev;
            Q.Np = p->Np; Q.B = B; Q.ds = p->ds; Q.nwork = wl.nwork; Q.tiles = p->sh_tiles[r.sh_list]; Q.jt = wl.jt;
            Q.pps = L.pps; Q.nm = L.nm; Q.rgroup = r.rgroup;
            Q.first_step = first_step;
            Q.ncol = p->ncol_dev;
            rc = gpmpc_timed_pair_sbs(p->D, grad, p->sh_ng, p->ds, Q, s);
        } else if (r.sb) {
            PairSbArgs Q;
            Q.M = p->M; Q.XT = p->XT; Q.pp = A.pp; Q.G = A.G; Q.part = A.part; Q.work = P.work;
            Q.Np = p->Np; Q.B = B; Q.ds = p->ds; Q.nwork = r.nwork; Q.pps = L.pps; Q.nm = L.nm; Q.rgroup = r.rgroup;
            Q.first_step = first_step;
            Q.colunroll = r.colunroll;
            Q.ncol = p->ncol_dev;
            rc = gpmpc_timed_pair_sb(p->D, grad, r.tb, p->ds, r.waves, Q, s);
        } else {
            rc = gpmpc_timed_pair(p->D, true, grad, r.tb, P.colsplit ? 4 : r.waves, P, s);
        }
        if (rc != GPMPC_OK) return rc;
    }
    return gpmpc_launch_roll_tail(A, grad, s);
}
```

include/gpmpc.h:

```cpp
#ifndef GPMPC_H
#define GPMPC_H

#include <stddef.h>

#ifdef __cplusplus
extern "C" {
#endif

#define GPMPC_MAX_D   8
#define GPMPC_MAX_DS  8

#define GPMPC_OK            0
#define GPMPC_E_ARG        -1
#define GPMPC_E_ALLOC      -2
#define GPMPC_E_LAUNCH     -3
#define GPMPC_E_WORKSPACE  -4
#define GPMPC_E_STATE      -5
#define GPMPC_E_DEVICE     -6

#define GPMPC_WANT_GRAD      1u
#define GPMPC_USE_GRAPH      4u
#define GPMPC_FP32_ACCUM     8u
#define GPMPC_FP32_ALL      16u
#define GPMPC_COV_BUG_COMPAT 2u

typedef struct gpmpc_pack gpmpc_pack;

int gpmpc_device_count(void);
const char* gpmpc_version(void);
const char* gpmpc_last_error(void);

int gpmpc_pack_create(gpmpc_pack** out, int n_train, int state_dim, int action_dim);
int gpmpc_pack_destroy(gpmpc_pack* pack);
int gpmpc_pack_resize(gpmpc_pack* pack, int n_train);
int gpmpc_pack_reload_tuning(gpmpc_pack* pack);
long long gpmpc_pack_graph_captures(const gpmpc_pack* pack);
long long gpmpc_pack_callback_captures(const gpmpc_pack* pack);

int gpmpc_store_host(void* dst_dev, const void* src_host, size_t bytes, void* stream);

int gpmpc_build_ky(int n, int D, const double* X_dev, const double* lambdas_host,
                   double sigma_f, double noise_var, double* Kf_dev, double* Ky_dev, void* stream);

int gpmpc_pack_build(gpmpc_pack* pack, const double* X_dev, const double* Y_dev,
                     const double* Ky_inv_dev, const double* lambdas_host,
                     const double* sigma_f_host, void* stream);

int gpmpc_pack_build_strided(gpmpc_pack* pack, const double* X_dev, const double* Y_dev, const double* Ky_inv_dev,
                             size_t ld, size_t gp_stride, const double* lambdas_host, const double* sigma_f_host, void* stream);

int gpmpc_pack_build_beta(gpmpc_pack* pack, const double* X_dev, const double* beta_dev,
                          const double* Ky_inv_dev, const double* lambdas_host,
                          const double* sigma_f_host, void* stream);

int gpmpc_pack_set_nominal(gpmpc_pack* pack, const double* weights_host, const double* bias_host, void* stream);
int gpmpc_pack_get_nominal(const gpmpc_pack* pack, double* weights_host, double* bias_host);

int gpmpc_pack_set_noise(gpmpc_pack* pack, const double* init_cov_host, const double* action_var_host, const double* process_var_host,
                         void* stream);
int gpmpc_pack_get_noise(const gpmpc_pack* pack, double* init_cov_host, double* action_var_host, double* process_var_host);

int gpmpc_pack_enable_fullcov(gpmpc_pack* pack, void* stream);

int gpmpc_pack_dims(const gpmpc_pack* pack, int* n_train, int* n_padded, int* state_dim, int* action_dim);
int gpmpc_pack_shared_lambda(const gpmpc_pack* pack);
int gpmpc_pack_export(const gpmpc_pack* pack, double* beta_out, double* weights_out, void* stream);

size_t gpmpc_moment_match_workspace_bytes(const gpmpc_pack* pack, int nq);
int gpmpc_moment_match(const gpmpc_pack* pack, int nq, const double* u_dev, const double* S_dev,
                       unsigned flags, double* out_mean, double* out_var, double* out_cov, double* out_l,
                       double* dmean_du, double* dmean_dS, double* dvar_du, double* dvar_dS,
                       double* dcov_du, double* dcov_dS,
                       void* workspace, size_t workspace_bytes, void* stream);

typedef struct gpmpc_cost_params {
    double gamma;
    double Q[GPMPC_MAX_DS * GPMPC_MAX_DS];
    double R[GPMPC_MAX_D * GPMPC_MAX_D];
    double R_delta[GPMPC_MAX_D * GPMPC_MAX_D];
    double x_ref[GPMPC_MAX_DS];
    double u_ref[GPMPC_MAX_D];
    double last_u[GPMPC_MAX_D];
    int has_R_delta;
    int schedule_id;
} gpmpc_cost_params;

int gpmpc_cost_schedule_create(int H_max, int state_dim, int action_dim, int* id_out);
int gpmpc_cost_schedule_destroy(int id);
int gpmpc_cost_schedule_set(int id, int H, const double* x_ref_host, const double* u_ref_host, const double* Q_terminal_host, void* stream);
int gpmpc_cost_schedule_set_dev(int id, int H, const double* x_ref_dev, const double* u_ref_dev, const double* Q_terminal_dev, void* stream);
int gpmpc_cost_schedule_get(int id, int* H_max, int* state_dim, int* action_dim, int* H, int* has_Q_terminal, const double** dev_out);

int gpmpc_cost(int B, int H, int state_dim, int action_dim, const gpmpc_cost_params* cost_host,
               const double* means_dev, const double* covs_dev, const double* U_dev,
               double* out_cost, void* stream);

int gpmpc_cost_grad(int B, int H, int state_dim, int action_dim, const gpmpc_cost_params* cost_host,
                    const double* means_dev, const double* covs_dev, const double* U_dev,
                    double* out_cost, double* d_means, double* d_covs, double* d_U, void* stream);

size_t gpmpc_rollout_workspace_bytes(const gpmpc_pack* pack, int B, int H, unsigned flags);
int gpmpc_plan_describe(const gpmpc_pack* pack, int B, int H, unsigned flags, char* out, size_t out_bytes);
int gpmpc_pack_autotune(gpmpc_pack* pack, int B, int H, unsigned flags, char* report, size_t report_bytes);
int gpmpc_pack_autotune_clear(gpmpc_pack* pack);
int gpmpc_rollout(const gpmpc_pack* pack, int B, int H, const double* x0_dev, const double* U_dev,
                  const gpmpc_cost_params* cost_host, unsigned flags,
                  double* out_means, double* out_vars, double* out_cost, double* out_grad,
                  void* workspace, size_t workspace_bytes, void* stream);

size_t gpmpc_rollout_jac_workspace_bytes(const gpmpc_pack* pack, int B, int H);
int gpmpc_rollout_jac(const gpmpc_pack* pack, int B, int H, const double* x0_dev, const double* U_dev,
                      double* out_means, double* out_vars, double* out_jac,
                      void* workspace, size_t workspace_bytes, void* stream);
int gpmpc_rollout_vjp(int B, int H, int state_dim, int action_dim, const double* jac_dev,
                      const double* g_means, const double* g_vars, double* out_gU, double* out_gx0, void* stream);

#define GPMPC_MAX_CONS 16
typedef struct gpmpc_state_constraints {
    int n_rows;
    int reserved;
    double A[GPMPC_MAX_CONS * GPMPC_MAX_DS];
    double b[GPMPC_MAX_CONS];
    double kappa[GPMPC_MAX_CONS];
} gpmpc_state_constraints;

int gpmpc_rollout_constraints(int B, int H, int state_dim, int action_dim, const gpmpc_state_constraints* cons_host,
                              const double* means_dev, const double* vars_dev, const double* jac_dev,
                              double* out_g, double* out_gjac, void* stream);

size_t gpmpc_rollout_constrained_workspace_bytes(const gpmpc_pack* pack, int B, int H, unsigned flags);
int gpmpc_rollout_constrained(const gpmpc_pack* pack, int B, int H, const double* x0_dev, const double* U_dev,
                              const gpmpc_cost_params* cost_host, const gpmpc_state_constraints* cons_host, unsigned flags,
                              double* out_means, double* out_vars, double* out_cost, double* out_grad,
                              double* out_g, double* out_gjac, void* workspace, size_t workspace_bytes, void* stream);

#define GPMPC_MPPI_MAX_SAMPLES 4096
typedef struct gpmpc_mppi_params {
    int n_samples;
    int iterations;
    double sigma[GPMPC_MAX_D];
    double sigma_decay;
    double beta;
    unsigned long long seed;
    unsigned int call_index;
    unsigned int reserved;
    double lb[GPMPC_MAX_D];
    double ub[GPMPC_MAX_D];
} gpmpc_mppi_params;

int gpmpc_mppi_sample(int H, int state_dim, int action_dim, const gpmpc_mppi_params* params_host, int iteration,
                      const double* mean_dev, const double* x0_dev, double* out_U, double* out_x0_batch, void* stream);

int gpmpc_mppi_update(int n_samples, int H, int action_dim, int n_rows, double beta, const double* U_dev, const double* cost_dev,
                      const double* g_dev, double* mean_dev, const double* best_in, double* best_out, double* out_trace, void* stream);

size_t gpmpc_mppi_solve_workspace_bytes(const gpmpc_pack* pack, int H, const gpmpc_mppi_params* params_host,
                                        const gpmpc_state_constraints* cons_host);
int gpmpc_mppi_solve(const gpmpc_pack* pack, int H, const double* x0_dev, const double* start_dev, const gpmpc_cost_params* cost_host,
                     const gpmpc_state_constraints* cons_host, const gpmpc_mppi_params* params_host, double* out_U, double* out_best,
                     double* out_trace, void* workspace, size_t workspace_bytes, void* stream);

#define GPMPC_LBFGS_MAX_STARTS 256
#define GPMPC_LBFGS_MAX_HISTORY 16
typedef struct gpmpc_lbfgs_params {
    int n_starts;
    int history;
    double gtol;
    double ftol;
    double c1;
    double min_step;
    double lb[GPMPC_MAX_D];
    double ub[GPMPC_MAX_D];
} gpmpc_lbfgs_params;

size_t gpmpc_lbfgs_state_bytes(int n_starts, int H, int action_dim, int history);

int gpmpc_lbfgs_start(int H, int state_dim, int action_dim, const gpmpc_lbfgs_params* params_host, const double* X0_dev,
                      const double* cost_dev, const double* grad_dev, const double* x0_dev, double* out_x0_batch,
                      void* state, size_t state_bytes, void* stream);

int gpmpc_lbfgs_tick(int H, int action_dim, const gpmpc_lbfgs_params* params_host, const double* cost_dev, const double* grad_dev,
                     void* state, size_t state_bytes, void* stream);

size_t gpmpc_lbfgs_solve_workspace_bytes(const gpmpc_pack* pack, int H, const gpmpc_lbfgs_params* params_host);
int gpmpc_lbfgs_solve(const gpmpc_pack* pack, int H, const double* x0_dev, const double* X0_dev, const gpmpc_cost_params* cost_host,
                      const gpmpc_lbfgs_params* params_host, int first_tick, int n_ticks, void* workspace, size_t workspace_bytes,
                      void* stream);

typedef struct gpmpc_auglag_params {
    gpmpc_lbfgs_params inner;
    double rho0;
    double growth;
    double shrink;
    double rho_max;
    double lam_max;
    double feas_tol;
    int inner_ticks;
    int reserved;
} gpmpc_auglag_params;

size_t gpmpc_auglag_state_bytes(int n_starts, int H, int action_dim, int n_rows);

int gpmpc_auglag_merit(int n_starts, int H, int action_dim, int n_rows, const double* f_dev, const double* grad_dev, const double* g_dev,
                       const double* gjac_dev, const double* lam_dev, const double* rho_dev, double* out_M, double* out_grad, void* stream);

int gpmpc_auglag_outer(int H, int action_dim, int n_rows, const gpmpc_auglag_params* params_host, int update, const double* f_dev,
                       const double* g_dev, const double* X_dev, const double* conv_dev, const double* alive_dev, void* state,
                       size_t state_bytes, void* stream);

size_t gpmpc_auglag_solve_workspace_bytes(const gpmpc_pack* pack, int H, const gpmpc_state_constraints* cons_host,
                                          const gpmpc_auglag_params* params_host);
int gpmpc_auglag_solve(const gpmpc_pack* pack, int H, const double* x0_dev, const double* X0_dev, const gpmpc_cost_params* cost_host,
                       const gpmpc_state_constraints* cons_host, const gpmpc_auglag_params* params_host, int first_outer, int n_outer,
                       void* workspace, size_t workspace_bytes, void* stream);

size_t gpmpc_rollout_fullcov_workspace_bytes(const gpmpc_pack* pack, int B, int H, unsigned flags);
int gpmpc_rollout_fullcov(const gpmpc_pack* pack, int B, int H, const double* x0_dev, const double* U_dev,
                          const gpmpc_cost_params* cost_host, unsigned flags,
                          double* out_means, double* out_covs, double* out_cost, double* out_grad,
                          void* workspace, size_t workspace_bytes, void* stream);
int gpmpc_rollout_fullcov_describe(const gpmpc_pack* pack, int B, int H, unsigned flags, char* out, size_t out_bytes);

int gpmpc_objective_gradient(gpmpc_pack* pack, int H, const double* x0_host, const double* U_host,
                             const gpmpc_cost_params* cost_host, unsigned flags, double* out_host, void* stream);

int gpmpc_timing_enable(int on);
int gpmpc_pair_kernel_time(double* total_ms, long long* launches, int reset);
int gpmpc_pair_kernel_time_class(int kernel_class, double* total_ms, long long* launches);

int gpmpc_debug_run_list(int n_padded, int state_dim, int slots, int* items_out, int capacity, int* n_items);
int gpmpc_debug_xcd_order(int linear_id, int grid_x, int n_tile, int n_traj, int* traj, int* column);

int gpmpc_matvec(int rows, int cols, const double* A_dev, const double* v_dev, double* out_dev, void* stream);
size_t gpmpc_predict_workspace_bytes(int n, int D, int p);
int gpmpc_predict(int n, int D, const double* X_dev, const double* lambdas_host, double sigma_f,
                  const double* beta_dev, const double* Ky_inv_dev, double noise_var,
                  int p, const double* X_pred_dev, double* out_K, double* out_mean, double* out_cov,
                  void* workspace, size_t workspace_bytes, void* stream);

size_t gpmpc_kinv_append_workspace_bytes(int n);
int gpmpc_kinv_append(int n, const double* Ky_inv_dev, const double* k_dev, double kappa, double* out_dev,
                      void* workspace, size_t workspace_bytes, void* stream);

size_t gpmpc_gp_append_workspace_bytes(int n, int D);
int gpmpc_gp_append(int n, int D, const double* X_dev, const double* x_new_dev, const double* lambdas_host, double sigma_f,
                    double noise_var, const double* Kf_in, const double* Ky_in, size_t ld_k_in, const double* Ky_inv_in, size_t ld_in,
                    double* Kf_out, double* Ky_out, double* Ky_inv_out, size_t ld_out, void* workspace, size_t workspace_bytes,
                    void* stream);

int gpmpc_kinv_remove(int n, const double* Ky_inv_dev, size_t ld_in, int index, double* out_dev, size_t ld_out, void* stream);

size_t gpmpc_gp_replace_workspace_bytes(int n, int D);
int gpmpc_gp_replace(int n, int D, int slot, const double* X_dev, const double* x_new_dev, const double* lambdas_host, double sigma_f,
                     double noise_var, const double* Kf_in, const double* Ky_in, size_t ld_k_in, const double* Ky_inv_in, size_t ld_in,
                     double* Kf_out, double* Ky_out, double* Ky_inv_out, size_t ld_out, void* workspace, size_t workspace_bytes,
                     void* stream);

size_t gpmpc_ml_grad_workspace_bytes(int n, int D);
int gpmpc_ml_grad(int n, int D, const double* X_dev, const double* Ky_inv_dev, const double* alpha_dev,
                  const double* resid_dev, const double* lambdas_host, double sigma_f, double noise_var,
                  double* out_dev, void* workspace, size_t workspace_bytes, void* stream);

#ifdef __cplusplus
}
#endif
#endif
```

Measured before the change: 6459 rollouts/s.

## Add shared-weight-column pair kernel where four trajectories share each M tile

```diff
diff --git a/gaussian_process_mpc_amd/_lib.py b/gaussian_process_mpc_amd/_lib.py
--- a/gaussian_process_mpc_amd/_lib.py
+++ b/gaussian_process_mpc_amd/_lib.py
@@ -156,6 +156,7 @@
     "gpmpc_rollout_fullcov": (_i, [_vp, _i, _i, _vp, _vp, ctypes.POINTER(CostParamsC), _u, _vp, _vp, _vp, _vp, _vp, _sz, _vp]),
     "gpmpc_timing_enable": (_i, [_i]),
     "gpmpc_debug_run_list": (_i, [_i, _i, _i, ctypes.POINTER(_i), _i, ctypes.POINTER(_i)]),
+    "gpmpc_debug_share_list": (_i, [_i, _i, ctypes.POINTER(_i), _i, ctypes.POINTER(_i)]),
     "gpmpc_debug_xcd_order": (_i, [_i, _i, _i, _i, ctypes.POINTER(_i), ctypes.POINTER(_i)]),
     "gpmpc_pair_kernel_time": (_i, [_dp, ctypes.POINTER(ctypes.c_longlong), _i]),
     "gpmpc_pair_kernel_time_class": (_i, [_i, _dp, ctypes.POINTER(ctypes.c_longlong)]),
diff --git a/gaussian_process_mpc_amd/csrc/api.hip b/gaussian_process_mpc_amd/csrc/api.hip
--- a/gaussian_process_mpc_amd/csrc/api.hip
+++ b/gaussian_process_mpc_amd/csrc/api.hip
@@ -39,6 +39,19 @@
         case 6: return gpmpc_launch_pair_sbs_D<6>(grad, ng, ns2, a, s);
         case 7: return gpmpc_launch_pair_sbs_D<7>(grad, ng, ns2, a, s);
         case 8: return gpmpc_launch_pair_sbs_D<8>(grad, ng, ns2, a, s);
+    }
+    return GPMPC_E_ARG;
+}
+
+int gpmpc_launch_pair_sbs4(int D, int ng, int ns2, const PairSbsArgs& a, hipStream_t s) {
+    switch (D) {
+        case 2: return gpmpc_launch_pair_sbs4_D<2>(ng, ns2, a, s);
+        case 3: return gpmpc_launch_pair_sbs4_D<3>(ng, ns2, a, s);
+        case 4: return gpmpc_launch_pair_sbs4_D<4>(ng, ns2, a, s);
+        case 5: return gpmpc_launch_pair_sbs4_D<5>(ng, ns2, a, s);
+        case 6: return gpmpc_launch_pair_sbs4_D<6>(ng, ns2, a, s);
+        case 7: return gpmpc_launch_pair_sbs4_D<7>(ng, ns2, a, s);
+        case 8: return gpmpc_launch_pair_sbs4_D<8>(ng, ns2, a, s);
     }
     return GPMPC_E_ARG;
 }
diff --git a/gaussian_process_mpc_amd/csrc/gpmpc_internal.h b/gaussian_process_mpc_amd/csrc/gpmpc_internal.h
--- a/gaussian_process_mpc_amd/csrc/gpmpc_internal.h
+++ b/gaussian_process_mpc_amd/csrc/gpmpc_internal.h
@@ -47,6 +47,7 @@
     int fc_shared;
     int xcdmap;
     int persist;
+    int sbs_share;
 };
 void gpmpc_read_tuning(gpmpc_tuning* t);
 
@@ -83,6 +84,8 @@
     int sh_ng;
     gpmpc_worklist wl_sh[4];
     int sh_tiles[3];
+    gpmpc_worklist wl_sh4;
+    int sh4_tiles;
     int nominal;
     double* nom_dev;
     double* resid_dev;
@@ -175,6 +178,23 @@
 }
 int gpmpc_launch_pair_sbs(int D, bool grad, int ng, int ns2, const PairSbsArgs& a, hipStream_t s);
 template <int D> int gpmpc_launch_pair_sbs_D(bool grad, int ng, int ns2, const PairSbsArgs& a, hipStream_t s);
+int gpmpc_launch_pair_sbs4(int D, int ng, int ns2, const PairSbsArgs& a, hipStream_t s);
+template <int D> int gpmpc_launch_pair_sbs4_D(int ng, int ns2, const PairSbsArgs& a, hipStream_t s);
+#define GPMPC_SBS4_RUN 256
+static inline int gpmpc_sbs4_items(int Np, int* items, int capacity) {
+    int k = 0;
+    for (int i0 = 0; i0 < Np; i0 += 64) {
+        const int span = Np - i0, runs = (span + GPMPC_SBS4_RUN - 1) / GPMPC_SBS4_RUN;
+        int j = i0;
+        for (int q = 0; q < runs; ++q) {
+            int len = ((span / runs) / 8) * 8;
+            if (q < (span - len * runs) / 8) len += 8;
+            if (items && k < capacity) { items[4 * k] = 0; items[4 * k + 1] = i0; items[4 * k + 2] = j; items[4 * k + 3] = len; }
+            ++k; j += len;
+        }
+    }
+    return k;
+}
 
 int gpmpc_launch_pair_lowprec(int D, int mode, const PairArgs& a, hipStream_t s);
 
diff --git a/gaussian_process_mpc_amd/csrc/pack.hip b/gaussian_process_mpc_amd/csrc/pack.hip
--- a/gaussian_process_mpc_amd/csrc/pack.hip
+++ b/gaussian_process_mpc_amd/csrc/pack.hip
@@ -301,6 +301,32 @@
     return e == hipSuccess ? 0 : -1;
 }
 
+static int sbs4_list_host(int Np, int groups, int** items_out) {
+    const int per = gpmpc_sbs4_items(Np, nullptr, 0);
+    int* h = (int*)malloc(sizeof(int) * 4 * (size_t)per * groups);
+    if (!h) return -1;
+    for (int g = 0; g < groups; ++g) {
+        gpmpc_sbs4_items(Np, h + 4 * (size_t)g * per, per);
+        for (int k = 0; k < per; ++k) h[4 * ((size_t)g * per + k)] = g;
+    }
+    *items_out = h;
+    return per;
+}
+static int build_worklist_sbs4(int Np, int groups, gpmpc_worklist* w, int* tiles_out) {
+    int* h = nullptr;
+    const int per = sbs4_list_host(Np, groups, &h), n = per * groups;
+    if (per < 0) return -1;
+    for (int g = 0; g <= groups; ++g) w->ustart_host[g] = g * per;
+    w->contiguous = 1;
+    w->it = 64; w->waves = 4; w->jt = GPMPC_SBS4_RUN; w->nunits = groups; w->nwork = n;
+    w->perm_dev = nullptr; w->ustart_dev = nullptr;
+    hipError_t e = hipMalloc(&w->work_dev, sizeof(int) * 4 * (size_t)n);
+    if (e == hipSuccess) e = hipMemcpy(w->work_dev, h, sizeof(int) * 4 * (size_t)n, hipMemcpyHostToDevice);
+    free(h);
+    *tiles_out = per;
+    return e == hipSuccess ? 0 : -1;
+}
+
 extern "C" int gpmpc_debug_run_list(int n_padded, int state_dim, int slots, int* items_out, int capacity, int* n_items) {
     if (n_padded < 64 || n_padded % 64 || state_dim < 1 || state_dim > GPMPC_MAX_DS || !n_items || capacity < 0 || (capacity > 0 && !items_out)) return GPMPC_E_ARG;
     int* h = nullptr; int ust[GPMPC_MAX_DS + 1];
@@ -308,6 +334,17 @@
     if (k < 0) return GPMPC_E_ALLOC;
     *n_items = k;
     if (k > 0) { if (k <= capacity) memcpy(items_out, h, sizeof(int) * 4 * (size_t)k); free(h); }
+    return (k > capacity && capacity > 0) ? GPMPC_E_ARG : GPMPC_OK;
+}
+extern "C" int gpmpc_debug_share_list(int n_padded, int groups, int* items_out, int capacity, int* n_items) {
+    if (n_padded < 64 || n_padded % 64 || groups < 1 || groups > GPMPC_MAX_DS || !n_items || capacity < 0 || (capacity > 0 && !items_out)) return GPMPC_E_ARG;
+    int* h = nullptr;
+    const int per = sbs4_list_host(n_padded, groups, &h);
+    if (per < 0) return GPMPC_E_ALLOC;
+    const int k = per * groups;
+    *n_items = k;
+    if (k <= capacity) memcpy(items_out, h, sizeof(int) * 4 * (size_t)k);
+    free(h);
     return (k > capacity && capacity > 0) ? GPMPC_E_ARG : GPMPC_OK;
 }
 extern "C" int gpmpc_debug_xcd_order(int linear_id, int grid_x, int n_tile, int n_traj, int* traj, int* column) {
@@ -334,6 +371,7 @@
     t->split = geti("GPMPC_SPLIT", -1);
     t->fused_sb = geti("GPMPC_FUSED_SB", -1);
     t->persist = geti("GPMPC_PERSIST", -1);
+    t->sbs_share = geti("GPMPC_SBS_SHARE", -1);
     t->xcdmap = geti("GPMPC_XCDMAP", -1);
     t->fc_shared = geti("GPMPC_FC_SHARED", -1);
     t->fc_form = geti("GPMPC_FC_FORM", -1);
@@ -419,6 +457,7 @@
             int tiles2 = 0;
             ok = build_worklist(p->Np, 256, 64, state_dim / 2, 0, false, &p->wl_sh[3], true, &tiles2) == 0;
         }
+        if (ok) ok = build_worklist_sbs4(p->Np, groups, &p->wl_sh4, &p->sh4_tiles) == 0;
     }
     if (!ok) { gpmpc_set_error("gpmpc_pack_create", e); gpmpc_pack_destroy(p); return GPMPC_E_ALLOC; }
     *out = p;
@@ -550,6 +589,7 @@
             if (p->wl[mode][k].perm_dev) (void)hipFree(p->wl[mode][k].perm_dev);
             if (p->wl[mode][k].ustart_dev) (void)hipFree(p->wl[mode][k].ustart_dev);
         }
+    if (p->wl_sh4.work_dev) (void)hipFree(p->wl_sh4.work_dev);
     for (int k = 0; k < 4; ++k) {
         if (p->wl_sh[k].work_dev) (void)hipFree(p->wl_sh[k].work_dev);
         if (p->wl_sh[k].perm_dev) (void)hipFree(p->wl_sh[k].perm_dev);
diff --git a/gaussian_process_mpc_amd/csrc/pair_inst.hip b/gaussian_process_mpc_amd/csrc/pair_inst.hip
--- a/gaussian_process_mpc_amd/csrc/pair_inst.hip
+++ b/gaussian_process_mpc_amd/csrc/pair_inst.hip
@@ -3,6 +3,7 @@
 #include "pair_kernel_sbf.h"
 #include "pair_kernel_sbfx.h"
 #include "pair_kernel_sbs.h"
+#include "pair_kernel_sbs4.h"
 #ifndef GPMPC_PAIR_D
 #error "compile with -DGPMPC_PAIR_D=<D>"
 #endif
@@ -11,6 +12,7 @@
 template int gpmpc_launch_pair_sbf_D<GPMPC_PAIR_D>(bool, int, int, const PairSbfArgs&, hipStream_t);
 template int gpmpc_launch_pair_sbfx_D<GPMPC_PAIR_D>(bool, int, const PairSbfxArgs&, hipStream_t);
 template int gpmpc_launch_pair_sbs_D<GPMPC_PAIR_D>(bool, int, int, const PairSbsArgs&, hipStream_t);
+template int gpmpc_launch_pair_sbs4_D<GPMPC_PAIR_D>(int, int, const PairSbsArgs&, hipStream_t);
 
 #if defined(GPMPC_SB_STAMPS) && GPMPC_PAIR_D == 5
 extern "C" int gpmpc_debug_sb_stamps(unsigned long long* host_out, int n) {
diff --git a/gaussian_process_mpc_amd/csrc/pair_kernel_sbs4.h b/gaussian_process_mpc_amd/csrc/pair_kernel_sbs4.h
--- /dev/null
+++ b/gaussian_process_mpc_amd/csrc/pair_kernel_sbs4.h
@@ -0,0 +1,201 @@
+#pragma once
+#include "pair_kernel_sbs.h"
+
+#ifndef GPMPC_SBS4_SYNC
+#define GPMPC_SBS4_SYNC 0
+#endif
+
+template <int D, int NG, int NS2, bool FIRST>
+__global__ __launch_bounds__(256, gpmpc_sbs_waves(NG, FIRST ? 1 + D - NS2 : 1 + D + NS2))
+void gpmpc_pair_kernel_sbs4(PairSbsArgs A) {
+    constexpr int GW = PairSbsTraits<D, NS2>::GW;
+    constexpr int NM = 1 + 2 * D, NA = 1 + D + NS2;
+    __shared__ double s_red[16 * NG * NM];
+    __shared__ double s_tab[GPMPC_EXP_N];
+    gpmpc_exp_table_to_lds(s_tab);
+
+    int bg, wi;
+    {
+        const int groups = (A.B + 3) >> 2, items = A.nwork, R = A.rgroup;
+        const int L = blockIdx.x, full = (items / (8 * R)) * (8 * R);
+        if (L < full * groups) {
+            const int q = L >> 3, ir = q % R, t = q / R;
+            bg = t % groups;
+            wi = ((t / groups) * R + ir) * 8 + (L & 7);
+        } else { const int Lt = L - full * groups; wi = full + Lt / groups; bg = Lt % groups; }
+    }
+    const int grp = A.work[wi * 4 + 0], i0 = A.work[wi * 4 + 1], j0 = A.work[wi * 4 + 2], nc = A.work[wi * 4 + 3];
+    const int tile = wi - grp * A.tiles;
+    const int Np = A.Np;
+    const int ncw = *(const int __attribute__((address_space(4)))*)A.ncol;
+    const int j1 = j0 + nc < ncw ? j0 + nc : ncw;
+    const int tid = threadIdx.x, lane = tid & 63;
+    const int w = __builtin_amdgcn_readfirstlane(tid >> 6);
+    const bool live = 4 * bg + w < A.B;
+    const int b = live ? 4 * bg + w : A.B - 1;
+
+    const double* __restrict__ prm = A.pp + (size_t)b * A.ds * A.pps;
+    const double* __restrict__ Gt = A.G + (size_t)b * Np * GW;
+    double hi2[D], qi;
+    {
+        const int i = i0 + lane;
+        double q = 0.0;
+#pragma unroll
+        for (int k = 0; k < D; ++k) {
+            const double x = A.XT[(size_t)k * Np + i];
+            const double h = fma(-prm[D + k], x, prm[k]);
+            hi2[k] = (2.0 * GPMPC_EXP_NEG_INV_C) * h;
+            q = fma(h, h, q);
+        }
+        qi = GPMPC_EXP_NEG_INV_C * q;
+    }
+
+    double acc[NG][NA];
+#pragma unroll
+    for (int g = 0; g < NG; ++g)
+#pragma unroll
+        for (int m = 0; m < NA; ++m) acc[g][m] = 0.0;
+
+    __syncthreads();
+
+    {
+        __amdgpu_buffer_rsrc_t Mrs[NG];
+#pragma unroll
+        for (int g = 0; g < NG; ++g) {
+            const int a = grp * NG + g < A.ds ? grp * NG + g : A.ds - 1;
+            Mrs[g] = __builtin_amdgcn_make_buffer_rsrc(const_cast<double*>(A.M + ((size_t)a * Np + j0) * Np + i0), 0, 0x7fffffff, 0x00020000);
+        }
+        const int lane8 = lane * 8;
+        constexpr int KC = 2;
+        typedef const double __attribute__((address_space(4))) gpmpc_cdouble;
+        auto batch = [&](int jc, const double (*mij)[NG]) {
+            double gr[KC][GW];
+#pragma unroll
+            for (int c = 0; c < KC; ++c) {
+                const gpmpc_cdouble* __restrict__ gp = (const gpmpc_cdouble*)(Gt + (size_t)(jc + c) * GW);
+#pragma unroll
+                for (int k = 0; k < D + 1 + NS2; ++k) gr[c][k] = gp[k];
+            }
+            __builtin_amdgcn_sched_barrier(0);
+            double fr[KC], Tv[KC];
+            int ni[KC];
+#pragma unroll
+            for (int c = 0; c < KC; ++c) {
+                double sx = qi + gr[c][D];
+#pragma unroll
+                for (int k = 0; k < D; ++k) sx = fma(hi2[k], gr[c][k], sx);
+                const double ax = __builtin_fabs(sx);
+                ni[c] = (int)(-ax);
+                fr[c] = __builtin_amdgcn_fract(ax);
+                Tv[c] = s_tab[ni[c] & (GPMPC_EXP_N - 1)];
+            }
+            __builtin_amdgcn_sched_barrier(0);
+#pragma unroll
+            for (int c = 0; c < KC; ++c) {
+                const double pq = fma(fr[c], fma(fr[c], GPMPC_EXP_A3, GPMPC_EXP_A2), GPMPC_EXP_A1);
+                const double e = ldexp(fma(Tv[c] * fr[c], pq, Tv[c]), ni[c] >> GPMPC_EXP_BITS);
+#pragma unroll
+                for (int q = 0; q < NG; ++q) {
+                    const double P = mij[c][q] * e;
+                    acc[q][0] += P;
+#pragma unroll
+                    for (int k = 0; k < D; ++k) if (!FIRST || k >= NS2) acc[q][1 + k] = fma(P, gr[c][k], acc[q][1 + k]);
+#pragma unroll
+                    for (int k = 0; k < NS2; ++k) if (!FIRST) acc[q][1 + D + k] = fma(P, gr[c][D + 1 + k], acc[q][1 + D + k]);
+                }
+            }
+            __builtin_amdgcn_sched_barrier(0);
+        };
+        auto wload = [&](double (*m)[NG], int jrel) {
+#pragma unroll
+            for (int c = 0; c < KC; ++c)
+#pragma unroll
+                for (int g = 0; g < NG; ++g) m[c][g] = __builtin_bit_cast(double, __builtin_amdgcn_raw_buffer_load_b64(Mrs[g], lane8, (jrel + c) * Np * 8, 0));
+        };
+        auto meet = [&](int jrel) {
+            if constexpr (GPMPC_SBS4_SYNC > 0) if ((jrel & (GPMPC_SBS4_SYNC - 1)) == 0) __builtin_amdgcn_s_barrier();
+        };
+        constexpr bool MPRE = NG >= 4;
+        if constexpr (MPRE) {
+            double ma[KC][NG], mb[KC][NG];
+            if (j0 < j1) wload(ma, 0);
+            for (int jc = j0; jc < j1; jc += 2 * KC) {
+                meet(jc - j0);
+                wload(mb, jc - j0 + KC);
+                __builtin_amdgcn_sched_barrier(0);
+                batch(jc, ma);
+                wload(ma, (jc + 2 * KC < j1 ? jc + 2 * KC : jc) - j0);
+                __builtin_amdgcn_sched_barrier(0);
+                batch(jc + KC, mb);
+            }
+        } else {
+            for (int jc = j0; jc < j1; jc += KC) {
+                meet(jc - j0);
+                double mij[KC][NG];
+                wload(mij, jc - j0);
+                batch(jc, mij);
+            }
+        }
+    }
+
+    double* const s_mine = s_red + w * 4 * NG * NM;
+#pragma unroll
+    for (int q = 0; q < NG; ++q) {
+        double z[NM];
+#pragma unroll
+        for (int m = 0; m < NM; ++m) z[m] = 0.0;
+        const double rs = acc[q][0];
+        z[0] += rs;
+#pragma unroll
+        for (int k = 0; k < D; ++k) {
+            const double h = (0.5 / GPMPC_EXP_NEG_INV_C) * hi2[k], v = acc[q][1 + k];
+            if (!FIRST || k >= NS2) z[1 + k] += fma(h, rs, v);
+            if (k < NS2 && !FIRST) z[1 + D + k] += fma(h * h, rs, fma(2.0 * h, v, acc[q][1 + D + (k < NS2 ? k : 0)]));
+        }
+#pragma unroll
+        for (int m = 0; m < NM; ++m) {
+            const double s = wave_row_sum(z[m]);
+            if ((lane & 15) == 0) s_mine[((lane >> 4) * NG + q) * NM + m] = s;
+        }
+    }
+    __builtin_amdgcn_fence(__ATOMIC_RELEASE, "wavefront");
+    __builtin_amdgcn_wave_barrier();
+    __builtin_amdgcn_fence(__ATOMIC_ACQUIRE, "wavefront");
+    for (int idx = lane; idx < NG * NM; idx += 64) {
+        const int q = idx / NM, m = idx - q * NM;
+        const int a = grp * NG + q;
+        if (a < A.ds && live) {
+            const double* r4 = &s_mine[q * NM + m];
+            const double s = (r4[0] + r4[NG * NM]) + (r4[2 * NG * NM] + r4[3 * NG * NM]);
+            A.part[((size_t)b * A.ds * A.tiles + (size_t)a * A.tiles + tile) * A.nm + m] = s;
+        }
+    }
+}
+
+template <int D, int NG, int NS2, bool FIRST>
+static int launch_pair_sbs4_one(const PairSbsArgs& a, hipStream_t s) {
+    dim3 grid((unsigned)((a.B + 3) / 4) * a.nwork), block(256);
+    hipLaunchKernelGGL((gpmpc_pair_kernel_sbs4<D, NG, NS2, FIRST>), grid, block, 0, s, a);
+    hipError_t e = hipGetLastError();
+    if (e != hipSuccess) { gpmpc_set_error("pair kernel (shared lambda, shared weight columns) launch", e); return GPMPC_E_LAUNCH; }
+    return GPMPC_OK;
+}
+
+template <int D>
+int gpmpc_launch_pair_sbs4_D(int ng, int ns2, const PairSbsArgs& a, hipStream_t s) {
+    if (a.nm != 1 + 2 * D || a.B < 1 || a.nwork < 1 || a.tiles < 1) return GPMPC_E_ARG;
+#define GPMPC_SBS4_NS(NGV, NSV)                                                                             \
+    if constexpr (NGV <= NSV) if (ng == NGV && ns2 == NSV) {                                                \
+        if (a.first_step) return launch_pair_sbs4_one<D, NGV, NSV, true>(a, s);                             \
+        return launch_pair_sbs4_one<D, NGV, NSV, false>(a, s);                                              \
+    }
+#define GPMPC_SBS4_NG(NGV)                                                                                  \
+    if constexpr (D >= 2) { GPMPC_SBS4_NS(NGV, (D >= 2 ? D - 1 : 1)) }                                      \
+    if constexpr (D >= 3) { GPMPC_SBS4_NS(NGV, (D >= 3 ? D - 2 : 1)) }
+    GPMPC_SBS4_NG(2)
+    GPMPC_SBS4_NG(3)
+    GPMPC_SBS4_NG(4)
+#undef GPMPC_SBS4_NG
+#undef GPMPC_SBS4_NS
+    return GPMPC_E_ARG;
+}
diff --git a/gaussian_process_mpc_amd/csrc/plan.h b/gaussian_process_mpc_amd/csrc/plan.h
--- a/gaussian_process_mpc_amd/csrc/plan.h
+++ b/gaussian_process_mpc_amd/csrc/plan.h
@@ -12,6 +12,7 @@
     int pwaves;
     int png;
     int hchunks, hrows;
+    int sbs4;
 };
 struct RollLayout {
     int nm, pps, sps, gw;
diff --git a/gaussian_process_mpc_amd/csrc/plan.hip b/gaussian_process_mpc_amd/csrc/plan.hip
--- a/gaussian_process_mpc_amd/csrc/plan.hip
+++ b/gaussian_process_mpc_amd/csrc/plan.hip
@@ -2,6 +2,8 @@
 #include <cstdlib>
 
 #define GPMPC_PERSIST_MAXNP_HOST 1024
+#define GPMPC_SBS4_MIN_B 16
+#define GPMPC_SBS4_MIN_NP 2048
 static thread_local int tl_graph_mode = -1;
 GraphModeGuard::GraphModeGuard(int m) : prev(tl_graph_mode) { tl_graph_mode = m; }
 GraphModeGuard::~GraphModeGuard() { tl_graph_mode = prev; }
@@ -68,7 +70,7 @@
     r->fq = (r->fused == 1 && r->tiling == 1 && (long)B * p->wl[0][1].nwork < 256) ? 4 : 1;
     r->waves = p->wl[0][r->tiling].waves;
     r->nwork = p->wl[0][r->tiling].nwork;
-    r->shared = 0; r->sh_list = 0;
+    r->shared = 0; r->sh_list = 0; r->sbs4 = 0;
     r->fng = p->sh_ng;
     if (p->sh_ng > 2 && p->ds % 2 == 0 && p->wl_sh[3].work_dev && wg2 < 4200) r->fng = 2;
     if (r->sb && r->fused == 2 && r->tiling == 2 && shared_on && (wg2 >= (r->fng == 2 ? (p->ds == 2 ? 700 : 1000) : 2200) || tn.fused_sb == 1)) {
@@ -83,6 +85,12 @@
         r->tb = 1; r->waves = 4;
         r->nwork = p->ds * p->sh_tiles[r->sh_list];
         r->rgroup = r->sh_list != 1 ? ((tn.rgroup >= 1 && tn.rgroup <= 16) ? tn.rgroup : 4) : 1;
+        if (grad && p->wl_sh4.work_dev && tn.sbs_share != 0 &&
+            (tn.sbs_share == 1 || (r->sh_list == 0 && B >= GPMPC_SBS4_MIN_B && p->Np >= GPMPC_SBS4_MIN_NP && D <= 5))) {
+            r->sbs4 = 1; r->sh_list = 0;
+            r->nwork = p->ds * p->sh4_tiles;
+            r->rgroup = (tn.rgroup >= 1 && tn.rgroup <= 16) ? tn.rgroup : 4;
+        }
     }
     if (r->fused == 2 && r->tiling == 2 && !r->shared && tn.tiling < 0 && p->wl[0][7].work_dev) {
         r->tiling = 7;
@@ -118,11 +126,17 @@
         r->png = 1;
         if (!lowprec && p->da >= 1 && p->da <= 2 && p->Np <= GPMPC_PERSIST_MAXNP_HOST && H * p->da <= 1024 && tn.persist != 0 &&
             pw && (tn.persist > 0 || (p->Np <= 640 && D <= 6 && !shared_ahead && !form_forced))) {
-            r->fused = 3; r->sb = 0; r->shared = 0; r->tb = 1; r->rgroup = 1; r->colunroll = 1; r->fq = 1;
+            r->fused = 3; r->sb = 0; r->shared = 0; r->sbs4 = 0; r->tb = 1; r->rgroup = 1; r->colunroll = 1; r->fq = 1;
             r->pwaves = pw;
             r->png = pshared ? ((pw == 16 && all_in_one) ? p->ds : 2) : 1;
             r->nwork = 0;
         }
+    }
+    if (tn.sbs_share == 1 && !r->sbs4 && shared_on && sb_ok && grad && !lowprec && p->wl_sh4.work_dev) {
+        r->sb = 1; r->fused = 0; r->fq = 1; r->shared = 1; r->sh_list = 0; r->sbs4 = 1; r->tiling = 0;
+        r->tb = 1; r->waves = 4; r->colunroll = 1; r->pwaves = 0; r->png = 1;
+        r->nwork = p->ds * p->sh4_tiles;
+        r->rgroup = (tn.rgroup >= 1 && tn.rgroup <= 16) ? tn.rgroup : 4;
     }
     r->hchunks = 0; r->hrows = 0;
     if (!r->fused && !lowprec) {
@@ -233,8 +247,9 @@
         form = "lowprec"; snprintf(kern, sizeof(kern), "k_pair_lowprec<%d>", D); wgs = (long)B * r.nwork;
     } else if (r.shared) {
         form = "head+pair_sbs";
-        snprintf(kern, sizeof(kern), "gpmpc_pair_kernel_sbs<%d,%d,%d,%s,false>", D, p->sh_ng, ds, grad ? "true" : "false");
-        wgs = (long)B * p->wl_sh[r.sh_list].nwork;
+        if (r.sbs4) snprintf(kern, sizeof(kern), "gpmpc_pair_kernel_sbs4<%d,%d,%d,false>", D, p->sh_ng, ds);
+        else snprintf(kern, sizeof(kern), "gpmpc_pair_kernel_sbs<%d,%d,%d,%s,false>", D, p->sh_ng, ds, grad ? "true" : "false");
+        wgs = r.sbs4 ? (long)((B + 3) / 4) * p->wl_sh4.nwork : (long)B * p->wl_sh[r.sh_list].nwork;
     } else if (r.sb) {
         form = "head+pair_sb";
         snprintf(kern, sizeof(kern), "gpmpc_pair_kernel_sb<%d,%d,%d,%s,false,%d>", D, r.tb, ds, grad ? "true" : "false", r.colunroll == 4 ? 4 : 1);
@@ -254,6 +269,6 @@
 bool gpmpc_same_shape(const RollShape& a, const RollShape& b) {
     if (a.fused == 3 && b.fused == 3) return a.pwaves == b.pwaves && a.png == b.png;
     return a.tiling == b.tiling && a.tb == b.tb && a.sb == b.sb && a.fused == b.fused && a.fq == b.fq && a.shared == b.shared &&
-           a.sh_list == b.sh_list && a.fng == b.fng && a.colunroll == b.colunroll && a.hchunks == b.hchunks && a.pwaves == b.pwaves &&
+           a.sh_list == b.sh_list && a.sbs4 == b.sbs4 && a.fng == b.fng && a.colunroll == b.colunroll && a.hchunks == b.hchunks && a.pwaves == b.pwaves &&
            a.rgroup == b.rgroup && a.nwork == b.nwork && a.xcdmap == b.xcdmap;
 }
diff --git a/gaussian_process_mpc_amd/csrc/rollout.h b/gaussian_process_mpc_amd/csrc/rollout.h
--- a/gaussian_process_mpc_amd/csrc/rollout.h
+++ b/gaussian_process_mpc_amd/csrc/rollout.h
@@ -26,6 +26,7 @@
 int gpmpc_timed_pair(int D, bool diag, bool grad, int tb, int waves, const PairArgs& a, hipStream_t s);
 int gpmpc_timed_pair_sb(int D, bool grad, int tb, int ns2, int waves, const PairSbArgs& a, hipStream_t s);
 int gpmpc_timed_pair_sbs(int D, bool grad, int ng, int ns2, const PairSbsArgs& a, hipStream_t s);
+int gpmpc_timed_pair_sbs4(int D, int ng, int ns2, const PairSbsArgs& a, hipStream_t s);
 int gpmpc_timed_pair_sbf(int D, bool grad, int ns2, int waves, const PairSbfArgs& a, hipStream_t s);
 int gpmpc_timed_persist(int D, bool grad, int ns2, int waves, int ng, const PersistArgs& a, hipStream_t s);
 int gpmpc_timed_step_fused(int D, bool grad, int ns2, int q, int ng, const FusedArgs& a, int t, hipStream_t s);
diff --git a/gaussian_process_mpc_amd/csrc/runtime.hip b/gaussian_process_mpc_amd/csrc/runtime.hip
--- a/gaussian_process_mpc_amd/csrc/runtime.hip
+++ b/gaussian_process_mpc_amd/csrc/runtime.hip
@@ -79,6 +79,10 @@
     return timed_launch(a.first_step ? GPMPC_TIME_FIRST : GPMPC_TIME_FULL, s,
                         [&] { return gpmpc_launch_pair_sbs(D, grad, ng, ns2, a, s); });
 }
+int gpmpc_timed_pair_sbs4(int D, int ng, int ns2, const PairSbsArgs& a, hipStream_t s) {
+    return timed_launch(a.first_step ? GPMPC_TIME_FIRST : GPMPC_TIME_FULL, s,
+                        [&] { return gpmpc_launch_pair_sbs4(D, ng, ns2, a, s); });
+}
 int gpmpc_timed_pair_sbf(int D, bool grad, int ns2, int waves, const PairSbfArgs& a, hipStream_t s) {
     return timed_launch(GPMPC_TIME_FULL, s, [&] { return gpmpc_launch_pair_sbf(D, grad, ns2, waves, a, s); });
 }
diff --git a/gaussian_process_mpc_amd/csrc/step.hip b/gaussian_process_mpc_amd/csrc/step.hip
--- a/gaussian_process_mpc_amd/csrc/step.hip
+++ b/gaussian_process_mpc_amd/csrc/step.hip
@@ -262,7 +262,7 @@
     }
     if (r.shared) {
         A.shared = 1; A.ust_inline = 1; A.work = nullptr; A.perm = nullptr;
-        for (int a = 0; a <= p->ds; ++a) A.ust[a] = a * p->sh_tiles[r.sh_list];
+        for (int a = 0; a <= p->ds; ++a) A.ust[a] = a * (r.sbs4 ? p->sh4_tiles : p->sh_tiles[r.sh_list]);
     }
 
     PairArgs P;
@@ -318,14 +318,14 @@
         if (lowprec) {
             rc = gpmpc_launch_pair_lowprec(p->D, lowprec, P, s);
         } else if (r.shared) {
-            const gpmpc_worklist& wl = p->wl_sh[r.sh_list];
+            const gpmpc_worklist& wl = r.sbs4 ? p->wl_sh4 : p->wl_sh[r.sh_list];
             PairSbsArgs Q;
             Q.M = p->M; Q.XT = p->XT; Q.pp = A.pp; Q.G = A.G; Q.part = A.part; Q.work = wl.work_dev;
-            Q.Np = p->Np; Q.B = B; Q.ds = p->ds; Q.nwork = wl.nwork; Q.tiles = p->sh_tiles[r.sh_list]; Q.jt = wl.jt;
+            Q.Np = p->Np; Q.B = B; Q.ds = p->ds; Q.nwork = wl.nwork; Q.tiles = r.sbs4 ? p->sh4_tiles : p->sh_tiles[r.sh_list]; Q.jt = wl.jt;
             Q.pps = L.pps; Q.nm = L.nm; Q.rgroup = r.rgroup;
             Q.first_step = first_step;
             Q.ncol = p->ncol_dev;
-            rc = gpmpc_timed_pair_sbs(p->D, grad, p->sh_ng, p->ds, Q, s);
+            rc = r.sbs4 ? gpmpc_timed_pair_sbs4(p->D, p->sh_ng, p->ds, Q, s) : gpmpc_timed_pair_sbs(p->D, grad, p->sh_ng, p->ds, Q, s);
         } else if (r.sb) {
             PairSbArgs Q;
             Q.M = p->M; Q.XT = p->XT; Q.pp = A.pp; Q.G = A.G; Q.part = A.part; Q.work = P.work;
diff --git a/include/gpmpc.h b/include/gpmpc.h
--- a/include/gpmpc.h
+++ b/include/gpmpc.h
@@ -228,6 +228,7 @@
 int gpmpc_pair_kernel_time(double* total_ms, long long* launches, int reset);
 int gpmpc_pair_kernel_time_class(int kernel_class, double* total_ms, long long* launches);
 
+int gpmpc_debug_share_list(int n_padded, int groups, int* items_out, int capacity, int* n_items);
 int gpmpc_debug_run_list(int n_padded, int state_dim, int slots, int* items_out, int capacity, int* n_items);
 int gpmpc_debug_xcd_order(int linear_id, int grid_x, int n_tile, int n_traj, int* traj, int* column);
 
```

Result: no change. 6477 rollouts/s, median of 6 (+0.3%).
